# forsaken628/katib

Measured on AMD Instinct MI355X. Metric: darts_cifar10_search_wall_clock_s, lower is better.
Workload: dtype fp32; 1 GPU; model=darts-cnn-cifar10 supernet (b5: C=4, L=2, N=3, stem x1, 6 primitives + none), global_batch=128, per_gpu_batch=128, parallelism=dp1, epochs=2, steps_per_epoch=196, ops=hip, hip_graph=True, sync_bn=False, hessian=concurrent

## Files before the change

katib_amd/csrc/hip/darts_bind.cpp:

```cpp
#include <torch/extension.h>
#include <c10/hip/HIPStream.h>

#include "darts_ops.h"
#include "darts_plane_layout.h"

using namespace katib_hip;
using at::Tensor;
using OptT = c10::optional<Tensor>;

namespace {

hipStream_t cur_stream() { return c10::hip::getCurrentHIPStream().stream(); }

void check_f32(const Tensor& t, const char* name) {
  TORCH_CHECK(t.is_cuda(), name, " must be a GPU tensor");
  TORCH_CHECK(t.scalar_type() == at::kFloat, name, " must be float32");
  TORCH_CHECK(t.is_contiguous(), name, " must be contiguous");
}

constexpr at::ScalarType kZType = kZbf16 ? at::kBFloat16 : at::kFloat;

void check_z(const Tensor& t, const char* name) {
  TORCH_CHECK(t.is_cuda(), name, " must be a GPU tensor");
  TORCH_CHECK(t.scalar_type() == kZType, name, " must be ", kZbf16 ? "bfloat16" : "float32",
              " (the per-op intermediates' storage type of this build)");
  TORCH_CHECK(t.is_contiguous(), name, " must be contiguous");
}

zt* zptr(const Tensor& t) { return reinterpret_cast<zt*>(t.data_ptr()); }

template <typename T>
T* ptr_or_null(const OptT& t) {
  return t.has_value() && t->defined() ? t->data_ptr<T>() : nullptr;
}

BNRef make_bn(const py::tuple& b, int C) {
  BNRef r{};
  TORCH_CHECK(b.size() == 8, "bn tuple has 8 fields");
  OptT sums = b[0].cast<OptT>(), rm = b[1].cast<OptT>(), rv = b[2].cast<OptT>();
  r.rep = b[6].cast<int>();
  r.rstride = b[7].cast<int>();
  TORCH_CHECK(r.rep >= 1 && r.rep <= kRep && r.rstride >= 2 * C, "bn replica layout");
  if (sums.has_value() && sums->defined()) {
    TORCH_CHECK(sums->scalar_type() == at::kDouble && sums->is_contiguous() &&
                    sums->numel() >= (int64_t)(r.rep - 1) * r.rstride + 2 * C,
                "bn sums must be f64 with rep x rstride doubles");
  }
  r.sums = ptr_or_null<double>(sums);
  r.rmean = ptr_or_null<float>(rm);
  r.rvar = ptr_or_null<float>(rv);
  r.inv_count = b[3].cast<float>();
  r.eval = b[4].cast<bool>() ? 1 : 0;
  r.eps = b[5].cast<float>();
  r.C = C;
  TORCH_CHECK(r.eval ? (r.rmean && r.rvar) : (r.sums != nullptr), "bn reference lacks its statistics");
  return r;
}

int64_t storage_doubles_after(const Tensor& t) {
  return (int64_t)(t.storage().nbytes() / sizeof(double)) - t.storage_offset();
}

GradSrc make_gs(const py::tuple& t, int C) {
  GradSrc g{};
  TORCH_CHECK(t.size() == 9, "grad-source tuple has 9 fields");
  Tensor gt = t[0].cast<Tensor>(), zt = t[1].cast<Tensor>();
  check_f32(gt, "g");
  check_z(zt, "z");
  g.g = gt.data_ptr<float>();
  g.z = zptr(zt);
  OptT s1 = t[2].cast<OptT>(), s2 = t[3].cast<OptT>();
  g.S1 = ptr_or_null<double>(s1);
  g.S2 = ptr_or_null<double>(s2);
  g.bn = make_bn(t[4].cast<py::tuple>(), C);
  g.eval = g.bn.eval;
  TORCH_CHECK(g.eval || (g.S1 && g.S2), "training-mode BN backward needs S1/S2 reductions");
  OptT w = t[5].cast<OptT>();
  g.w = ptr_or_null<float>(w);
  g.widx = t[6].cast<int>();
  g.rep = t[7].cast<int>();
  g.rstride = t[8].cast<int>();
  TORCH_CHECK(g.rep >= 1 && g.rep <= kRep, "replicas");
  if (!g.eval) {
    for (int k = 2; k <= 3; ++k) {
      Tensor sv = *t[k].cast<OptT>();
      TORCH_CHECK(sv.scalar_type() == at::kDouble &&
                      storage_doubles_after(sv) >= (int64_t)(g.rep - 1) * g.rstride + C,
                  "S1/S2 replicas exceed their buffer");
    }
  }
  return g;
}

int pick_chunk(int C, int per_channel_floats, int fixed_floats) {
  const int budget = 16384 - fixed_floats;
  int ch = C;
  while (ch > 1 && ch * per_channel_floats > budget) ch = (ch + 1) / 2;
  return std::max(ch, 1);
}

template <typename Bt>
void check_batch(const std::vector<py::tuple>& calls) {
  TORCH_CHECK(!calls.empty() && (int)calls.size() <= Bt::kCap, "batch of 1..", Bt::kCap, " edges");
}

#define SAME_SHAPE(b, fld) TORCH_CHECK(b.e[i].fld == b.e[0].fld, "edges in a batch must share " #fld)

static bool fill_dwpw(const py::tuple& t, DwPwFwdArgs& a, int64_t K, int64_t dil, int64_t S, int64_t pad, int nentries,
                      bool use_mfma) {
  Tensor x = t[0].cast<Tensor>(), dw = t[1].cast<Tensor>(), pw = t[2].cast<Tensor>();
  auto inbn = t[3].cast<c10::optional<py::tuple>>();
  OptT d = t[4].cast<OptT>();
  Tensor z = t[5].cast<Tensor>();
  OptT stats = t[6].cast<OptT>();
  const bool has_d = d.has_value() && d->defined();
  const bool has_inbn = t[3].cast<c10::optional<py::tuple>>().has_value();
  if (has_inbn) check_z(x, "x (previous stage z)");
  else check_f32(x, "x");
  check_f32(dw, "dw"); check_f32(pw, "pw"); check_z(z, "z");
  if (has_d) check_z(*d, "d");
  TORCH_CHECK(x.dim() == 4, "x must be NCHW");
  TORCH_CHECK((K == 3 || K == 5) && (dil == 1 || dil == 2) && (S == 1 || S == 2), "K in {3,5}, dil, S in {1,2}");
  const int N = x.size(0), C = x.size(1), H = x.size(2), W = x.size(3);
  const int Ho = z.size(2), Wo = z.size(3);
  TORCH_CHECK(dw.numel() == C * K * K && pw.numel() == C * C, "weight shapes");
  TORCH_CHECK(z.size(0) == N && z.size(1) == C && (!has_d || d->sizes() == z.sizes()), "output shapes");
  TORCH_CHECK(has_d || !dwpw_split_path(C), "dw-pw stages of 16..64 channels (depthwise + pointwise GEMM) need d");
  TORCH_CHECK(C == 4 || C == 8 || C == 16 || (64 % Wo == 0 && Ho % (64 / Wo) == 0),
              "tile constraint: 64 % Wo == 0 and Ho % (64/Wo) == 0");
  TORCH_CHECK(C <= kMaxC, "C too large");
  TORCH_CHECK(Ho == (H + 2 * pad - dil * (K - 1) - 1) / S + 1, "output height mismatch");
  a.x = x.data_ptr(); a.dw = dw.data_ptr<float>(); a.pw = pw.data_ptr<float>();
  a.d = has_d ? zptr(*d) : nullptr; a.z = zptr(z); a.stats = ptr_or_null<double>(stats);
  if (a.stats) TORCH_CHECK(stats->scalar_type() == at::kDouble && stats->numel() >= kRep * 2 * C, "stats f64 [kRep][2C]");
  a.N = N; a.C = C; a.H = H; a.W = W; a.Ho = Ho; a.Wo = Wo; a.pad = pad;
  const int TR = 64 / Wo;
  const int IR = (TR - 1) * S + (K - 1) * dil + 1, IW = (Wo - 1) * S + (K - 1) * dil + 1;
  a.chunk = pick_chunk(C, IR * IW, C * 64 + 4 * C);
  if (C == 4 || C == 8 || C == 16) {
    int nb = std::max(1, std::min(Ho / 4, 2048 / std::max(N * nentries, 1)));
    auto band_bytes = [&](int b) {
      const int BR = (Ho + b - 1) / b;
      return (size_t)C * ((BR - 1) * S + (K - 1) * dil + 1) * plane_pitch(W + 2 * pad, S) * sizeof(float);
    };
    while (band_bytes(nb) > 65536 && nb < Ho) ++nb;
    a.chunk = nb;
  }
  a.use_mfma = (use_mfma && C % 16 == 0) ? 1 : 0;
  const bool prebn = inbn.has_value();
  if (prebn) a.inbn = make_bn(*inbn, C);
  a.variant = (((K == 5) * 4 + (dil == 2) * 2 + (S == 2)) * 4) + (prebn ? 2 : 0);
  return prebn;
}

static void fill_dwpw_multi(const std::vector<py::tuple>& calls, DwPwMultiBatch& bt, int64_t* kk, int64_t* dd,
                            int64_t* ss, int64_t* pp, bool* pre) {
  TORCH_CHECK(!calls.empty() && (int)calls.size() <= DwPwMultiBatch::kCap, "1..", DwPwMultiBatch::kCap, " entries");
  bt.n = calls.size();
  for (int i = 0; i < bt.n; ++i) {
    const py::tuple& t = calls[i];
    TORCH_CHECK(t.size() == 11, "dwpw_fwd_multi entry: (x, dw, pw, inbn, d, z, stats, K, dil, S, pad)");
    kk[i] = t[7].cast<int64_t>(); dd[i] = t[8].cast<int64_t>(); ss[i] = t[9].cast<int64_t>(); pp[i] = t[10].cast<int64_t>();
    pre[i] = fill_dwpw(t, bt.e[i], kk[i], dd[i], ss[i], pp[i], bt.n, true);
    SAME_SHAPE(bt, N); SAME_SHAPE(bt, C); SAME_SHAPE(bt, Ho); SAME_SHAPE(bt, Wo);
  }
}

void dwpw_fwd_multi(std::vector<py::tuple> calls) {
  DwPwMultiBatch bt{};
  int64_t kk[DwPwMultiBatch::kCap], dd[DwPwMultiBatch::kCap], ss[DwPwMultiBatch::kCap], pp[DwPwMultiBatch::kCap];
  bool pre[DwPwMultiBatch::kCap];
  fill_dwpw_multi(calls, bt, kk, dd, ss, pp, pre);
  if (launch_dwpw_multi(bt, cur_stream())) return;
  for (int i = 0; i < bt.n; ++i) {
    DwPwFwdBatch one{};
    one.n = 1;
    fill_dwpw(calls[i], one.e[0], kk[i], dd[i], ss[i], pp[i], 1, true);
    launch_dwpw_fwd(one, kk[i], dd[i], ss[i], pre[i], cur_stream());
  }
}

void pw_fwd(std::vector<py::tuple> calls, int64_t S) {
  check_batch<PwFwdBatch>(calls);
  PwFwdBatch bt{};
  bt.n = calls.size();
  for (int i = 0; i < bt.n; ++i) {
    const py::tuple& t = calls[i];
    Tensor x = t[0].cast<Tensor>(), pw = t[1].cast<Tensor>(), z = t[2].cast<Tensor>();
    OptT stats = t[3].cast<OptT>();
    const int co_off = t[4].cast<int>(), off = t[5].cast<int>();
    check_f32(x, "x"); check_f32(pw, "pw"); check_z(z, "z");
    const bool nm = x.dim() == 5;
    const int xnodes = nm ? x.size(0) : 1;
    const int N = nm ? x.size(1) : x.size(0), Cin = nm ? x.size(0) * x.size(2) : x.size(1);
    const int H = x.size(nm ? 3 : 2), W = x.size(nm ? 4 : 3);
    const int Cout = pw.size(0), Ho = z.size(2), Wo = z.size(3);
    TORCH_CHECK(pw.size(1) == Cin && co_off + Cout <= z.size(1) && z.size(0) == N, "pw shapes");
    TORCH_CHECK((Ho * Wo) % 64 == 0, "Ho*Wo must be a multiple of 64");
    TORCH_CHECK(Cin <= kMaxC && Cout <= kMaxC, "channels");
    PwFwdArgs& a = bt.e[i];
    a.x = x.data_ptr<float>(); a.pw = pw.data_ptr<float>(); a.z = zptr(z);
    a.stats = ptr_or_null<double>(stats);
    if (a.stats)
      TORCH_CHECK(stats->scalar_type() == at::kDouble && stats->numel() >= kRep * 2 * z.size(1), "stats [kRep][2Ctot]");
    a.N = N; a.Cin = Cin; a.Cout = Cout; a.CoutTotal = z.size(1); a.co_off = co_off;
    a.H = H; a.W = W; a.Ho = Ho; a.Wo = Wo; a.S = S; a.off = off; a.relu = 1; a.xnodes = xnodes;
    SAME_SHAPE(bt, N); SAME_SHAPE(bt, Cin); SAME_SHAPE(bt, Cout); SAME_SHAPE(bt, Ho); SAME_SHAPE(bt, Wo);
  }
  launch_pw_fwd(bt, cur_stream());
}

void pool_fwd_multi(std::vector<py::tuple> calls) {
  check_batch<PoolFwdBatch>(calls);
  PoolFwdBatch bt{};
  bt.n = calls.size();
  for (int i = 0; i < bt.n; ++i) {
    const py::tuple& t = calls[i];
    const int64_t S = t[6].cast<int64_t>();
    TORCH_CHECK(S == 1 || S == 2, "pool stride must be 1 or 2");
    bt.e[i].S = (int)S;
    Tensor x = t[0].cast<Tensor>(), zavg = t[1].cast<Tensor>(), zmax = t[2].cast<Tensor>();
    OptT sa = t[3].cast<OptT>(), sm = t[4].cast<OptT>(), amax = t[5].cast<OptT>();
    check_f32(x, "x"); check_z(zavg, "zavg"); check_z(zmax, "zmax");
    PoolFwdArgs& a = bt.e[i];
    if (amax.has_value() && amax->defined()) {
      TORCH_CHECK(amax->scalar_type() == at::kByte && amax->numel() == zmax.numel(), "amax must be uint8 like zmax");
      a.amax = amax->data_ptr<uint8_t>();
    }
    a.x = x.data_ptr<float>(); a.zavg = zptr(zavg); a.zmax = zptr(zmax);
    a.stats_avg = ptr_or_null<double>(sa); a.stats_max = ptr_or_null<double>(sm);
    if (a.stats_avg) TORCH_CHECK(sa->scalar_type() == at::kDouble && sa->numel() >= kRep * 2 * x.size(1), "stats");
    if (a.stats_max) TORCH_CHECK(sm->scalar_type() == at::kDouble && sm->numel() >= kRep * 2 * x.size(1), "stats");
    a.N = x.size(0); a.C = x.size(1); a.H = x.size(2); a.W = x.size(3); a.Ho = zavg.size(2); a.Wo = zavg.size(3);
    TORCH_CHECK(a.Ho == (a.H - 1) / S + 1 && zmax.sizes() == zavg.sizes(), "pool shapes");
    SAME_SHAPE(bt, N); SAME_SHAPE(bt, C);
  }
  launch_pool_fwd_multi(bt, cur_stream());
}

void combine_fwd(std::vector<py::tuple> calls, OptT gamma, OptT beta, Tensor out, double momentum,
                 bool update_running, bool accumulate) {
  check_f32(out, "out");
  check_batch<CombineFwdBatch>(calls);
  CombineFwdBatch bt{};
  bt.n = calls.size();
  const int C = out.size(1);
  TORCH_CHECK(C <= kMaxC, "C too large");
  TORCH_CHECK((int64_t)2 * bt.n * kMaxOps * C * 4 <= 65536, "combine LDS budget exceeded");
  for (int e = 0; e < bt.n; ++e) {
    const py::tuple& t = calls[e];
    auto zs = t[0].cast<std::vector<Tensor>>();
    auto bns = t[1].cast<std::vector<py::tuple>>();
    auto widx = t[2].cast<std::vector<int64_t>>();
    OptT w = t[3].cast<OptT>();
    const int id_idx = t[4].cast<int>();
    OptT xid = t[5].cast<OptT>();
    auto upd = t[6].cast<std::vector<py::tuple>>();
    TORCH_CHECK(zs.size() == bns.size() && zs.size() == widx.size() && (int)zs.size() <= kMaxOps, "ops");
    CombineFwdArgs& a = bt.e[e];
    a.N = out.size(0); a.C = C; a.HW = out.size(2) * out.size(3);
    a.nops = zs.size();
    for (size_t k = 0; k < zs.size(); ++k) {
      check_z(zs[k], "z");
      TORCH_CHECK(zs[k].sizes() == out.sizes(), "combine input shape");
      a.z[k] = zptr(zs[k]);
      a.bn[k] = make_bn(bns[k], C);
      a.widx[k] = widx[k];
    }
    TORCH_CHECK((int)upd.size() <= kMaxUpd, "too many update-only BN layers");
    a.nupd = upd.size();
    for (size_t k = 0; k < upd.size(); ++k) a.upd[k] = make_bn(upd[k], C);
    a.w = ptr_or_null<float>(w); a.id_idx = id_idx; a.xid = ptr_or_null<float>(xid);
    if (a.xid) {
      check_f32(*xid, "xid");
      TORCH_CHECK(xid->sizes() == out.sizes(), "identity shape");
    }
    a.gamma = ptr_or_null<float>(gamma); a.beta = ptr_or_null<float>(beta);
    a.out = out.data_ptr<float>(); a.momentum = momentum; a.update_running = update_running;
    a.accumulate = accumulate;
  }
  launch_combine_fwd(bt, cur_stream());
}

void combine_bwd_reduce(std::vector<py::tuple> calls) {
  check_batch<CombineBwdBatch>(calls);
  CombineBwdBatch bt{};
  bt.n = calls.size();
  for (int i = 0; i < bt.n; ++i) {
    const py::tuple& t = calls[i];
    Tensor dout = t[0].cast<Tensor>();
    auto zs = t[1].cast<std::vector<Tensor>>();
    auto bns = t[2].cast<std::vector<py::tuple>>();
    OptT xid = t[3].cast<OptT>();
    Tensor red = t[4].cast<Tensor>();
    auto widx = t[5].cast<std::vector<int64_t>>();
    const int id_idx = t[6].cast<int>();
    OptT gw = t[7].cast<OptT>();
    check_f32(dout, "dout");
    TORCH_CHECK(red.scalar_type() == at::kDouble, "red must be f64");
    CombineBwdArgs& a = bt.e[i];
    a.N = dout.size(0); a.C = dout.size(1); a.HW = dout.size(2) * dout.size(3);
    a.nops = zs.size();
    a.rstride = (a.nops + 1) * a.C + 1;
    TORCH_CHECK(a.nops <= kMaxOps && red.numel() >= (int64_t)kRep * a.rstride, "red size [kRep][(nops+1)C+1]");
    for (int k = 0; k < a.nops; ++k) {
      TORCH_CHECK(zs[k].sizes() == dout.sizes(), "z shape");
      check_z(zs[k], "z");
      a.z[k] = zptr(zs[k]);
      a.bn[k] = make_bn(bns[k], a.C);
    }
    a.dout = dout.data_ptr<float>(); a.xid = ptr_or_null<float>(xid); a.red = red.data_ptr<double>();
    a.gw = ptr_or_null<double>(gw); a.id_idx = id_idx;
    if (a.gw) {
      TORCH_CHECK(gw->scalar_type() == at::kDouble && gw->numel() % kRep == 0, "gw must be f64 [kRep][nw]");
      a.gwstride = gw->numel() / kRep;
      TORCH_CHECK((int)widx.size() == a.nops, "widx per op");
      for (int k = 0; k < a.nops; ++k) {
        TORCH_CHECK(widx[k] >= 0 && widx[k] < a.gwstride, "widx out of range");
        a.widx[k] = widx[k];
      }
      TORCH_CHECK(id_idx < a.gwstride, "id_idx out of range");
    }
    SAME_SHAPE(bt, N); SAME_SHAPE(bt, C); SAME_SHAPE(bt, HW);
  }
  launch_combine_bwd_reduce(bt, cur_stream());
}

void check_grad_sink(const OptT& gW, int64_t numel, int64_t gstride) {
  if (!gW.has_value() || !gW->defined()) return;
  TORCH_CHECK(gW->scalar_type() == at::kFloat && gW->is_contiguous() && gW->numel() == numel, "gW shape");
  TORCH_CHECK(gstride == 0 || (gstride >= numel && (int64_t)(gW->storage().nbytes() / sizeof(float)) -
                                                           gW->storage_offset() >= (kRep - 1) * gstride + numel),
              "gW replicas exceed their buffer");
}

void pw_bwd(std::vector<py::tuple> calls, int64_t S, int64_t mode, bool need_dx) {
  check_batch<PwBwdBatch>(calls);
  PwBwdBatch bt{};
  bt.n = calls.size();
  for (int i = 0; i < bt.n; ++i) {
    const py::tuple& t = calls[i];
    py::tuple gs = t[0].cast<py::tuple>();
    Tensor pw = t[1].cast<Tensor>();
    OptT ain = t[2].cast<OptT>();
    Tensor x = t[3].cast<Tensor>();
    OptT dd = t[4].cast<OptT>(), gx = t[5].cast<OptT>(), gW = t[6].cast<OptT>();
    const int co_off = t[7].cast<int>(), off = t[8].cast<int>();
    const int64_t gstride = t[9].cast<int64_t>();
    const bool overwrite = t.size() > 10 && t[10].cast<bool>();
    check_f32(pw, "pw");
    if (mode != 0) check_f32(x, "x");
    PwBwdArgs& a = bt.e[i];
    a.overwrite = overwrite;
    TORCH_CHECK(!overwrite || (mode == 1 && S == 1 && off == 0), "gx overwrite needs the stride-1 full-coverage form");
    const int Cout = pw.size(0), Cin = pw.size(1);
    Tensor g = gs[0].cast<Tensor>();
    a.N = g.size(0); a.CoutTotal = g.size(1); a.Ho = g.size(2); a.Wo = g.size(3);
    a.gs = make_gs(gs, a.CoutTotal);
    a.Cin = Cin; a.Cout = Cout; a.co_off = co_off; a.S = S; a.off = off; a.mode = mode;
    a.need_dx = need_dx;
    const bool nm = mode != 0 && x.dim() == 5;
    a.xnodes = nm ? x.size(0) : 1;
    a.H = x.size(nm ? 3 : 2); a.W = x.size(nm ? 4 : 3);
    if (mode != 0) {
      TORCH_CHECK(x.numel() == (int64_t)a.N * Cin * a.H * a.W && (!nm || x.size(1) == a.N),
                  "pw_bwd: x must be [N][Cin][H][W] or node-major [nodes][N][Cin/nodes][H][W]");
      if (gx.has_value() && gx->defined()) TORCH_CHECK(gx->sizes() == x.sizes(), "pw_bwd: gx must have the shape of x");
    }
    TORCH_CHECK(Cin * Cout <= 8192, "pw_bwd supports Cin*Cout <= 8192");
    TORCH_CHECK((a.Ho * a.Wo) % 64 == 0, "Ho*Wo % 64");
    a.pw = pw.data_ptr<float>(); a.x = mode != 0 ? x.data_ptr<float>() : nullptr;
    if (ain.has_value() && ain->defined()) check_z(*ain, "ain (depthwise output d)");
    a.ain = ain.has_value() && ain->defined() ? zptr(*ain) : nullptr;
    a.dd = ptr_or_null<float>(dd); a.gx = ptr_or_null<float>(gx);
    a.gW = ptr_or_null<float>(gW);
    if (mode == 0) {
      TORCH_CHECK((a.ain || !a.gW) && (!need_dx || a.dd), "mode 0 needs ain for a weight gradient (and dd)");
    } else {
      TORCH_CHECK(!need_dx || a.gx, "mode 1 needs gx");
    }
    check_grad_sink(gW, (int64_t)Cin * Cout, gstride);
    a.gstride = gstride;
    SAME_SHAPE(bt, N); SAME_SHAPE(bt, Cin); SAME_SHAPE(bt, Cout); SAME_SHAPE(bt, Ho); SAME_SHAPE(bt, Wo);
  }
  launch_pw_bwd(bt, cur_stream());
}

void dw_bwd_fill(std::vector<py::tuple>& calls, DwBwdBatch& bt, const int64_t* Ks, const int64_t* dils,
                 const int64_t* Ss, bool& prebn);

void dw_bwd_multi(std::vector<py::tuple> calls) {
  check_batch<DwBwdBatch>(calls);
  DwBwdBatch bt{};
  int64_t Ks[DwBwdBatch::kCap], Ds[DwBwdBatch::kCap], Ss[DwBwdBatch::kCap];
  for (size_t i = 0; i < calls.size(); ++i) {
    TORCH_CHECK(calls[i].size() == 10 || calls[i].size() == 12,
                "dw_bwd_multi entry: (x, inbn, dw, dd, gout, gW, red, gstride, overwrite, K[, dil, S])");
    Ks[i] = calls[i][9].cast<int64_t>();
    Ds[i] = calls[i].size() == 12 ? calls[i][10].cast<int64_t>() : 1;
    Ss[i] = calls[i].size() == 12 ? calls[i][11].cast<int64_t>() : 1;
    TORCH_CHECK((Ks[i] == 3 || Ks[i] == 5) && (Ds[i] == 1 || Ds[i] == 2) && (Ss[i] == 1 || Ss[i] == 2),
                "K in {3, 5}, dil and S in {1, 2}");
  }
  bool prebn = false;
  dw_bwd_fill(calls, bt, Ks, Ds, Ss, prebn);
  for (int i = 0; i < bt.n; ++i) {
    TORCH_CHECK(prebn || bt.e[i].overwrite, "dw_bwd_multi: input-gradient entries must own (overwrite) their output");
    TORCH_CHECK(!prebn || (Ds[i] == 1 && Ss[i] == 1), "dw_bwd_multi: input-BN entries are stride-1 separable stages");
    bt.e[i].variant = dw_bwd_variant((int)Ks[i], (int)Ds[i], (int)Ss[i], prebn);
  }
  for (int i = 0; i < bt.n; ++i)
    for (int j = i + 1; j < bt.n; ++j) TORCH_CHECK(bt.e[i].gout != bt.e[j].gout, "dw_bwd_multi entries share an output");
  if (launch_dw_bwd_multi(bt, cur_stream())) return;
  for (int v = 0; v < 16; ++v) {
    DwBwdBatch one{};
    for (int i = 0; i < bt.n; ++i)
      if (bt.e[i].variant == v) one.e[one.n++] = bt.e[i];
    if (one.n) launch_dw_bwd(one, dw_variant_k(v), dw_variant_dil(v), dw_variant_s(v), prebn, cur_stream());
  }
}

void dw_bwd_fill(std::vector<py::tuple>& calls, DwBwdBatch& bt, const int64_t* Ks, const int64_t* dils,
                 const int64_t* Ss, bool& prebn) {
  bt.n = calls.size();
  bool has_gw = false;
  for (int i = 0; i < bt.n; ++i) {
    const py::tuple& t = calls[i];
    const int64_t K = Ks[i], dil = dils[i], S = Ss[i], pad = (K - 1) / 2 * dil;
    Tensor x = t[0].cast<Tensor>();
    auto inbn = t[1].cast<c10::optional<py::tuple>>();
    Tensor dw = t[2].cast<Tensor>(), dd = t[3].cast<Tensor>(), gout = t[4].cast<Tensor>();
    OptT gW = t[5].cast<OptT>(), red = t[6].cast<OptT>();
    const int64_t gstride = t[7].cast<int64_t>();
    const bool overwrite = t[8].cast<bool>();
    if (inbn.has_value()) check_z(x, "x (stage-1 z)");
    else check_f32(x, "x");
    check_f32(dw, "dw"); check_f32(dd, "dd"); check_f32(gout, "gout");
    DwBwdArgs& a = bt.e[i];
    a.N = x.size(0); a.C = x.size(1); a.H = x.size(2); a.W = x.size(3); a.Ho = dd.size(2); a.Wo = dd.size(3);
    TORCH_CHECK(a.H == a.Ho * S && a.W == a.Wo * S, "dw_bwd needs H == Ho*S");
    TORCH_CHECK(gout.sizes() == x.sizes(), "gout shape");
    TORCH_CHECK(dw.numel() == a.C * K * K && dd.size(1) == a.C, "dw_bwd weight / grad shapes");
    a.x = x.data_ptr(); a.dw = dw.data_ptr<float>(); a.dd = dd.data_ptr<float>();
    a.gout = gout.data_ptr<float>(); a.gW = ptr_or_null<float>(gW); a.red = ptr_or_null<double>(red);
    const bool plane = (a.C == 4 || a.C == 8 || (a.C % 16 == 0 && a.C <= kMaxC)) && a.Wo % 4 == 0 &&
                       (((uintptr_t)a.x | (uintptr_t)a.dd | (uintptr_t)a.gout) & 15) == 0;
    TORCH_CHECK(plane || (64 % a.Wo == 0 && a.Ho % (64 / a.Wo) == 0), "tile constraint");
    check_grad_sink(gW, (int64_t)a.C * K * K, gstride);
    a.gstride = gstride;
    a.overwrite = overwrite;
    if (a.red) TORCH_CHECK(red->scalar_type() == at::kDouble && red->numel() >= kRep * 2 * a.C, "red [kRep][2C]");
    a.pad = pad;
    if (i == 0) {
      prebn = inbn.has_value();
      has_gw = a.gW != nullptr;
    }
    TORCH_CHECK(inbn.has_value() == prebn, "edges in a batch must agree on the input BN");
    TORCH_CHECK((a.gW != nullptr) == has_gw, "edges in a batch must agree on weight-gradient sinks");
    TORCH_CHECK(!(prebn && overwrite), "overwrite applies to the input-gradient (non-BN) form");
    const int TR = 64 / a.Wo, r = (K - 1) / 2 * dil, h = (r + S - 1) / S, OR = TR + 2 * h;
    const int IR = (TR - 1) * S + (K - 1) * dil + 1, IW = (a.Wo - 1) * S + (K - 1) * dil + 1;
    a.chunk = pick_chunk(a.C, OR * a.Wo + IR * IW, 4 * a.C + (a.gW ? a.C * (int)(K * K) : 0));
    if (prebn) a.inbn = make_bn(*inbn, a.C);
    SAME_SHAPE(bt, N); SAME_SHAPE(bt, C); SAME_SHAPE(bt, Ho); SAME_SHAPE(bt, Wo);
  }
}

void pool_bwd_multi(std::vector<py::tuple> calls) {
  check_batch<PoolBwdBatch>(calls);
  PoolBwdBatch bt{};
  bt.n = calls.size();
  for (int i = 0; i < bt.n; ++i) {
    const py::tuple& t = calls[i];
    const int64_t S = t[9].cast<int64_t>();
    TORCH_CHECK(S == 1 || S == 2, "pool stride must be 1 or 2");
    bt.e[i].S = (int)S;
    auto ga = t[0].cast<c10::optional<py::tuple>>(), gm = t[1].cast<c10::optional<py::tuple>>();
    Tensor x = t[2].cast<Tensor>();
    OptT dout_id = t[3].cast<OptT>(), w = t[4].cast<OptT>();
    const int id_idx = t[5].cast<int>();
    Tensor gx = t[6].cast<Tensor>();
    OptT amax = t[7].cast<OptT>();
    check_f32(x, "x"); check_f32(gx, "gx");
    PoolBwdArgs& a = bt.e[i];
    a.N = x.size(0); a.C = x.size(1); a.H = x.size(2); a.W = x.size(3);
    a.Ho = (a.H - 1) / S + 1; a.Wo = (a.W - 1) / S + 1;
    TORCH_CHECK(a.Ho * a.Wo <= 8192, "pool_bwd stages one output plane in LDS (Ho*Wo <= 8192)");
    TORCH_CHECK(gx.sizes() == x.sizes(), "gx shape");
    TORCH_CHECK(!gm.has_value() || (amax.has_value() && amax->defined() && amax->scalar_type() == at::kByte &&
                                    amax->numel() == (int64_t)a.N * a.C * a.Ho * a.Wo),
                "max-pool backward needs the uint8 argmax from pool_fwd");
    if (amax.has_value() && amax->defined()) a.amax = amax->data_ptr<uint8_t>();
    if (ga.has_value()) a.ga = make_gs(*ga, a.C);
    if (gm.has_value()) a.gm = make_gs(*gm, a.C);
    a.x = x.data_ptr<float>(); a.dout_id = ptr_or_null<float>(dout_id); a.w = ptr_or_null<float>(w);
    if (a.dout_id) TORCH_CHECK(dout_id->sizes() == x.sizes(), "identity gradient shape");
    a.id_idx = id_idx; a.gx = gx.data_ptr<float>();
    a.overwrite = t[8].cast<bool>();
    if (t.size() > 10) {
      auto ex = t[10].cast<std::vector<Tensor>>();
      TORCH_CHECK(ex.size() <= 4, "pool_bwd: at most 4 extra gradient parts");
      a.nextra = ex.size();
      for (size_t j = 0; j < ex.size(); ++j) {
        check_f32(ex[j], "extra");
        TORCH_CHECK(ex[j].sizes() == gx.sizes(), "extra gradient part shape");
        TORCH_CHECK(ex[j].data_ptr() != gx.data_ptr(), "extra part aliases gx");
        a.extra[j] = ex[j].data_ptr<float>();
      }
    }
    SAME_SHAPE(bt, N); SAME_SHAPE(bt, C);
  }
  for (int i = 0; i < bt.n; ++i)
    for (int j = i + 1; j < bt.n; ++j) TORCH_CHECK(bt.e[i].gx != bt.e[j].gx, "pool_bwd entries share a gx buffer");
  launch_pool_bwd_multi(bt, cur_stream());
}

void fold_rows(Tensor buf) {
  check_f32(buf, "buf");
  TORCH_CHECK(buf.dim() == 2, "buf must be [rows][n]");
  FoldArgs a{};
  a.buf = buf.data_ptr<float>();
  a.rows = buf.size(0);
  a.n = buf.size(1);
  launch_fold_rows(a, cur_stream());
}

void fold_f64(std::vector<py::tuple> segs) {
  TORCH_CHECK(!segs.empty() && (int)segs.size() <= kMaxSeg, "1..kMaxSeg segments");
  FoldF64Args a{};
  a.nseg = segs.size();
  for (int k = 0; k < a.nseg; ++k) {
    Tensor t = segs[k][0].cast<Tensor>();
    int n = segs[k][1].cast<int>(), rs = segs[k][2].cast<int>();
    TORCH_CHECK(t.is_cuda() && t.scalar_type() == at::kDouble && t.is_contiguous(), "fold segment must be f64");
    TORCH_CHECK(n >= 1 && rs >= n && t.numel() >= (int64_t)(kRep - 1) * rs + n, "fold segment size");
    a.p[k] = t.data_ptr<double>();
    a.n[k] = n;
    a.rstride[k] = rs;
    a.total += n;
  }
  launch_fold_f64(a, cur_stream());
}

}

void register_xgmi(py::module& m);
void register_conv(py::module& m);
void register_transformer(py::module& m);
void register_batchnorm(py::module& m);
void register_mlp(py::module& m);
void register_stem(py::module& m);
void register_enas(py::module& m);
void register_dwconv(py::module& m);
void register_darts_optim(py::module& m);
void register_darts_head(py::module& m);
void register_resnet(py::module& m);
void register_augment(py::module& m);

PYBIND11_MODULE(TORCH_EXTENSION_NAME, m) {
  m.doc() = "katib_amd HIP kernels for gfx950 (DARTS edge ops, implicit-GEMM conv, transformer, xGMI all-reduce)";
  m.def("pw_fwd", &pw_fwd);
  m.def("combine_fwd", &combine_fwd);
  m.def("combine_bwd_reduce", &combine_bwd_reduce);
  m.def("pw_bwd", &pw_bwd);
  m.def("dw_bwd_multi", &dw_bwd_multi, "separable second-stage depthwise backward of mixed kernel size in one launch");
  m.def("dwpw_fwd_multi", &dwpw_fwd_multi, "mixed (K, dil, S) dw-pw entries of one node stage in one launch");
  m.def("pool_fwd_multi", &pool_fwd_multi, "stride-1 and stride-2 pools in one launch");
  m.def("pool_bwd_multi", &pool_bwd_multi, "stride-1 and stride-2 pool backward in one launch");
  m.def("set_max_blocks", &set_max_blocks);
  m.def("stamps_arm", [](int kind, int call, torch::Tensor buf) {
    TORCH_CHECK(!buf.defined() || kind == 0 || (buf.is_cuda() && buf.scalar_type() == torch::kInt64 &&
                                               buf.is_contiguous() && buf.numel() >= 65536 * 8),
                "stamps_arm: int64 CUDA buffer of >= 65536 * 8 entries");
    stamps_arm(kind, call, kind == 0 ? nullptr : reinterpret_cast<unsigned long long*>(buf.data_ptr<int64_t>()));
  }, "diagnostic build: phase-stamp the call-th launch of kind (StampKind) into buf[wg * 8 + phase]");
  m.def("stamps_compiled", &stamps_compiled);
  m.def("fold_rows", &fold_rows);
  m.def("fold_f64", &fold_f64);
  m.attr("REP") = kRep;
  m.attr("ZBF16") = kZbf16;
  m.def("max_blocks", &max_blocks);
  m.def("dwpw_split_path", [](int64_t C) { return dwpw_split_path((int)C); });
  register_xgmi(m);
  register_conv(m);
  register_transformer(m);
  register_batchnorm(m);
  register_enas(m);
  register_dwconv(m);
  register_mlp(m);
  register_stem(m);
  register_darts_optim(m);
  register_darts_head(m);
  register_resnet(m);
  register_augment(m);
}
```

katib_amd/csrc/hip/darts_ops.h:

```cpp
#pragma once
#include <hip/hip_runtime.h>
#include <hip/hip_bf16.h>

namespace katib_hip {

#ifdef KATIB_DARTS_ZBF16
typedef __hip_bfloat16 zt;
constexpr bool kZbf16 = true;
#else
typedef float zt;
constexpr bool kZbf16 = false;
#endif
typedef float zf4 __attribute__((ext_vector_type(4)));

__device__ __forceinline__ float z2f(float v) { return v; }
__device__ __forceinline__ float z2f(__hip_bfloat16 v) { return __bfloat162float(v); }
__device__ __forceinline__ void zput(float* p, float v) { *p = v; }
__device__ __forceinline__ void zput(__hip_bfloat16* p, float v) { *p = __float2bfloat16(v); }
__device__ __forceinline__ zf4 zld4(const float* p) { return *reinterpret_cast<const zf4*>(p); }
__device__ __forceinline__ zf4 zld4(const __hip_bfloat16* p) {
  const uint2 u = *reinterpret_cast<const uint2*>(p);
  return zf4{__uint_as_float(u.x << 16), __uint_as_float(u.x & 0xffff0000u), __uint_as_float(u.y << 16),
             __uint_as_float(u.y & 0xffff0000u)};
}
__device__ __forceinline__ void zst4(float* p, zf4 v) { *reinterpret_cast<zf4*>(p) = v; }
__device__ __forceinline__ void zst4(__hip_bfloat16* p, zf4 v) {
  __hip_bfloat16 b[4] = {__float2bfloat16(v.x), __float2bfloat16(v.y), __float2bfloat16(v.z), __float2bfloat16(v.w)};
  *reinterpret_cast<uint2*>(p) = *reinterpret_cast<const uint2*>(b);
}

__host__ __device__ __forceinline__ size_t plane_off(int n, int c, int N, int C, int nodes, size_t HW) {
  if (nodes <= 1) return ((size_t)n * C + c) * HW;
  const int Cn = C / nodes, k = c / Cn;
  return (((size_t)k * N + n) * Cn + (c - k * Cn)) * HW;
}

constexpr int kMaxOps = 8;
constexpr int kMaxUpd = 4;
constexpr int kMaxC = 256;
constexpr bool dwpw_split_path(int C) { return C % 16 == 0 && C <= 64; }
#ifndef KATIB_HIP_REP
#define KATIB_HIP_REP 32
#endif
constexpr int kRep = KATIB_HIP_REP;

struct BNRef {
  const double* sums;
  float* rmean;
  float* rvar;
  float inv_count;
  float eps;
  int eval;
  int C;
  int rep;
  int rstride;
};

struct GradSrc {
  const float* g;
  const zt* z;
  const double* S1;
  const double* S2;
  BNRef bn;
  const float* w;
  int widx;
  int eval;
  int rep;
  int rstride;
};

struct DwPwFwdArgs {
  const void* x;
  BNRef inbn; const float* dw; const float* pw;
  zt* d; zt* z; double* stats;
  int N, C, H, W, Ho, Wo, pad, chunk, use_mfma;
  int variant;
  int nblk;
  int vout = 0;
};

struct PwFwdArgs {
  const void* x;
  const float* pw; zt* z; double* stats;
  int N, Cin, Cout, CoutTotal, co_off, H, W, Ho, Wo, S, off;
  int relu;
  int xnodes;
};

struct PoolFwdArgs {
  const float* x; zt* zavg; zt* zmax; double* stats_avg; double* stats_max; unsigned char* amax;
  int N, C, H, W, Ho, Wo;
  int S, nblk;
};

struct CombineFwdArgs {
  const zt* z[kMaxOps]; BNRef bn[kMaxOps]; int widx[kMaxOps]; int nops;
  BNRef upd[kMaxUpd]; int nupd;
  const float* w; int id_idx; const float* xid; const float* gamma; const float* beta;
  float* out; int N, C, HW; float momentum; int update_running; int accumulate;
};

struct CombineBwdArgs {
  const float* dout; const zt* z[kMaxOps]; BNRef bn[kMaxOps]; int nops;
  const float* xid; double* red; int N, C, HW;
  double* gw; int widx[kMaxOps]; int id_idx;
  int rstride, gwstride;
};

struct PwBwdArgs {
  GradSrc gs; const float* pw; const zt* ain; const float* x; float* dd; float* gx; float* gW;
  int gstride;
  int N, Cin, Cout, CoutTotal, co_off, H, W, Ho, Wo, S, off, mode, need_dx;
  int overwrite;
  int xnodes;
};

struct DwBwdArgs {
  const void* x;
  BNRef inbn; const float* dw; const float* dd; float* gout; float* gW; double* red;
  int gstride;
  int N, C, H, W, Ho, Wo, pad, chunk;
  int overwrite;
  int variant, nbands, nblk;
  int vin = 0;
  int blk0 = 0;
};
constexpr int dw_bwd_variant(int K, int dil, int S, bool prebn) {
  return (((K == 5) * 4 + (dil == 2) * 2 + (S == 2)) << 1) | (prebn ? 1 : 0);
}
constexpr int dw_variant_k(int v) { return (v >> 3) & 1 ? 5 : 3; }
constexpr int dw_variant_dil(int v) { return (v >> 2) & 1 ? 2 : 1; }
constexpr int dw_variant_s(int v) { return (v >> 1) & 1 ? 2 : 1; }
constexpr bool dw_variant_prebn(int v) { return v & 1; }

struct FoldArgs {
  float* buf; int n; int rows;
};

constexpr int kMaxSeg = 128;
struct FoldF64Args {
  double* p[kMaxSeg]; int n[kMaxSeg]; int rstride[kMaxSeg]; int nseg; int total;
};

struct PoolBwdArgs {
  GradSrc ga; GradSrc gm; const float* x; const float* dout_id; const float* w; int id_idx; float* gx;
  const unsigned char* amax;
  const float* extra[4]; int nextra;
  int overwrite;
  int N, C, H, W, Ho, Wo;
  int S;
};

template <typename A, int M>
struct Batch {
  A e[M];
  int n;
  static constexpr int kCap = M;
};
using DwPwFwdBatch = Batch<DwPwFwdArgs, 16>;
using CombineFwdBatch = Batch<CombineFwdArgs, 4>;
using PwFwdBatch = Batch<PwFwdArgs, 32>;
using PoolFwdBatch = Batch<PoolFwdArgs, 16>;
using CombineBwdBatch = Batch<CombineBwdArgs, 8>;
using PwBwdBatch = Batch<PwBwdArgs, 32>;
using DwBwdBatch = Batch<DwBwdArgs, 40>;
using PoolBwdBatch = Batch<PoolBwdArgs, 16>;
using DwPwMultiBatch = Batch<DwPwFwdArgs, 40>;

constexpr size_t kKernargMax = 24576;
static_assert(sizeof(DwPwFwdBatch) <= kKernargMax && sizeof(CombineFwdBatch) <= kKernargMax &&
                  sizeof(PwFwdBatch) <= kKernargMax && sizeof(PoolFwdBatch) <= kKernargMax &&
                  sizeof(CombineBwdBatch) <= kKernargMax && sizeof(PwBwdBatch) <= kKernargMax &&
                  sizeof(DwBwdBatch) <= kKernargMax && sizeof(PoolBwdBatch) <= kKernargMax &&
                  sizeof(DwPwMultiBatch) <= kKernargMax,
              "kernel argument batches exceed the kernarg budget");

void launch_dwpw_fwd(const DwPwFwdBatch& b, int K, int dil, int S, bool prebn, hipStream_t st);
void launch_dw_bwd(const DwBwdBatch& b, int K, int dil, int S, bool prebn, hipStream_t st);
bool launch_dw_bwd_multi(DwBwdBatch b, hipStream_t st);
void launch_pw_fwd(const PwFwdBatch& b, hipStream_t st);
bool launch_dwpw_multi(DwPwMultiBatch b, hipStream_t st);
void launch_pool_fwd_multi(PoolFwdBatch b, hipStream_t st);
void launch_pool_bwd_multi(const PoolBwdBatch& b, hipStream_t st);
void launch_combine_fwd(const CombineFwdBatch& b, hipStream_t st);
void launch_combine_bwd_reduce(const CombineBwdBatch& b, hipStream_t st);
void launch_pw_bwd(const PwBwdBatch& b, hipStream_t st);
int max_blocks();
void launch_fold_rows(const FoldArgs& a, hipStream_t st);
void launch_fold_f64(const FoldF64Args& a, hipStream_t st);
void set_max_blocks(int n);
void stamps_arm(int kind, int call, unsigned long long* buf);
bool stamps_compiled();

}
```

katib_amd/csrc/hip/darts_ops_dwb.hip:

```cpp
#include "darts_ops_dev.h"

namespace katib_hip {

template <int K, int DIL, int S, bool PREBN>
__global__ void __launch_bounds__(256) dw_bwd_kernel(DwBwdBatch bt) {
  const DwBwdArgs& a = bt.e[blockIdx.y];
  constexpr int P = 64, KK = K * K;
  const int C = a.C, H = a.H, W = a.W, Ho = a.Ho, Wo = a.Wo;
  const int TR = P / Wo;
  const int tiles = Ho / TR;
  const int ntiles = a.N * tiles;
  const int pad = a.pad;
  const int r = (K - 1) / 2 * DIL;
  const int h = (r + S - 1) / S;
  const int OR = TR + 2 * h;
  const int IR = (TR - 1) * S + (K - 1) * DIL + 1;
  const int IW = (Wo - 1) * S + (K - 1) * DIL + 1;
  extern __shared__ __attribute__((aligned(16))) float smem[];
  float* sDD = smem;
  float* sIn = sDD + a.chunk * OR * Wo;
  float* sMean = sIn + a.chunk * IR * IW;
  float* sInv = sMean + C;
  float* sRed = sInv + C;
  float* sGW = sRed + 2 * C;
  const int tid = threadIdx.x, wave = tid >> 6, lane = tid & 63;
  for (int c = tid; c < C; c += 256) {
    if (PREBN) bn_coeffs(a.inbn, c, sMean[c], sInv[c]);
    sRed[c] = 0.f;
    sRed[C + c] = 0.f;
  }
  if (a.gW)
    for (int i = tid; i < C * KK; i += 256) sGW[i] = 0.f;
  __syncthreads();
  const int own_in = TR * S;
  const int nq = own_in * W;
  for (int t = blockIdx.x; t < ntiles; t += gridDim.x) {
    const int n = t / tiles, oy0 = (t % tiles) * TR;
    const int iy0 = oy0 * S - pad;
    const size_t xin = (size_t)n * C * H * W;
    const float* ddn = a.dd + (size_t)n * C * Ho * Wo;
    for (int c0 = 0; c0 < C; c0 += a.chunk) {
      const int cn = min(a.chunk, C - c0);
      #pragma unroll 4
      for (int i = tid; i < cn * OR * Wo; i += 256) {
        int cc = i / (OR * Wo), rr = (i / Wo) % OR, q = i % Wo;
        int oy = oy0 - h + rr;
        sDD[i] = (oy >= 0 && oy < Ho) ? ddn[((size_t)(c0 + cc) * Ho + oy) * Wo + q] : 0.f;
      }
      if (a.gW) {
        #pragma unroll 4
        for (int i = tid; i < cn * IR * IW; i += 256) {
          int cc = i / (IR * IW), rr = (i / IW) % IR, q = i % IW;
          int iy = iy0 + rr, ix = -pad + q, c = c0 + cc;
          float v = 0.f;
          if (iy >= 0 && iy < H && ix >= 0 && ix < W) {
            v = xval<PREBN>(a.x, xin + ((size_t)c * H + iy) * W + ix);
            if (PREBN) v = (v - sMean[c]) * sInv[c];
            v = fmaxf(v, 0.f);
          }
          sIn[i] = v;
        }
      }
      __syncthreads();
      if (a.gW) {
        for (int job = tid; job < cn * KK; job += 256) {
          const int cc = job / KK, tap = job % KK, ky = tap / K, kx = tap % K;
          const float* dd = sDD + (cc * OR + h) * Wo;
          const float* in = sIn + (cc * IR + ky * DIL) * IW + kx * DIL;
          float s = 0.f;
          for (int ty = 0; ty < TR; ++ty)
            for (int tx = 0; tx < Wo; ++tx) s += dd[ty * Wo + tx] * in[ty * S * IW + tx * S];
          sGW[(c0 + cc) * KK + tap] += s;
        }
      }
      const int qspan = (nq < 256 && 256 % nq == 0) ? nq : 256;
      const int G = 256 / qspan;
      for (int q0 = 0; q0 < nq; q0 += qspan) {
        const int q = q0 + tid % qspan;
        const int cg = __builtin_amdgcn_readfirstlane(tid / qspan);
        const int rr = q / W, ix = q - rr * W;
        const int iy = oy0 * S + rr;
        const bool ok = q < nq && iy < H;
        int srow[K], ocol[K];
        float mrow[K], mcol[K];
#pragma unroll
        for (int k = 0; k < K; ++k) {
          int ty = iy + pad - k * DIL;
          int oy = ty >= 0 ? ty / S : -1;
          bool v = ok && ty >= 0 && (ty % S) == 0 && oy < Ho;
          srow[k] = v ? oy - (oy0 - h) : 0;
          mrow[k] = v ? 1.f : 0.f;
          int tx = ix + pad - k * DIL;
          int ox = tx >= 0 ? tx / S : -1;
          bool u = ok && tx >= 0 && (tx % S) == 0 && ox < Wo;
          ocol[k] = u ? ox : 0;
          mcol[k] = u ? 1.f : 0.f;
        }
        for (int cc = cg; cc < cn; cc += G) {
          const int c = c0 + cc;
          const float* wk = a.dw + c * KK;
          const float* dd = sDD + cc * OR * Wo;
          float ga = 0.f;
#pragma unroll
          for (int ky = 0; ky < K; ++ky) {
            float rowacc = 0.f;
#pragma unroll
            for (int kx = 0; kx < K; ++kx) rowacc += mcol[kx] * wk[ky * K + kx] * dd[srow[ky] * Wo + ocol[kx]];
            ga += mrow[ky] * rowacc;
          }
          const size_t xi = ((size_t)(n * C + c) * H + iy) * W + ix;
          if (PREBN) {
            float g = 0.f, gy = 0.f;
            if (ok) {
              float y = (xval<true>(a.x, xi) - sMean[c]) * sInv[c];
              g = y > 0.f ? ga : 0.f;
              gy = g * y;
              a.gout[xi] = g;
            }
            if (a.red) {
              g = wave_sum(g);
              gy = wave_sum(gy);
              if (lane == 0) {
                atomicAdd(sRed + c, g);
                atomicAdd(sRed + C + c, gy);
              }
            }
          } else if (ok) {
            const float gm = xval<false>(a.x, xi) > 0.f ? ga : 0.f;
            if (a.overwrite) a.gout[xi] = gm;
            else if (gm != 0.f) a.gout[xi] += gm;
          }
        }
      }
      __syncthreads();
    }
  }
  if (PREBN && a.red)
    for (int i = tid; i < 2 * C; i += 256) atomicAdd(a.red + rep_slot() * 2 * C + i, (double)sRed[i]);
  if (a.gW)
    for (int i = tid; i < C * KK; i += 256) atomicAdd(a.gW + (size_t)rep_slot() * a.gstride + i, sGW[i]);
}

template <int S, bool V4 = false>
__device__ __forceinline__ void pool_bwd_body(const PoolBwdArgs& a, const int bx) {
  const int C = a.C, H = a.H, W = a.W, Ho = a.Ho, Wo = a.Wo, HWo = Ho * Wo;
  const int nc = bx, c = nc % C;
  const size_t ob = (size_t)nc * HWo;
  extern __shared__ __attribute__((aligned(16))) float smem[];
  float* sGa = smem;
  float* sGm = smem + HWo;
  unsigned char* sArg = (unsigned char*)(smem + 2 * HWo);
  __shared__ float sCo[8];
  KSTAMP(0);
  if (threadIdx.x < 64) {
    const int grp = threadIdx.x >> 4, j = threadIdx.x & 15;
    const GradSrc& gs = grp & 1 ? a.gm : a.ga;
    const bool on = gs.z != nullptr, stats = grp < 2;
    const BNRef& b = gs.bn;
    double s = 0.0, s2 = 0.0;
    if (on && stats && !b.eval) {
      for (int r = j; r < b.rep; r += 16) {
        s += b.sums[(size_t)r * b.rstride + c];
        s2 += b.sums[(size_t)r * b.rstride + b.C + c];
      }
    } else if (on && !stats && !gs.eval) {
      const int rep = gs.rep, rs = gs.rep == 1 ? 0 : gs.rstride;
      const size_t off2 = gs.S2 - gs.S1;
      for (int r = j; r < rep; r += 16) {
        s += gs.S1[(size_t)r * rs + c];
        s2 += gs.S1[(size_t)r * rs + off2 + c];
      }
    }
#pragma unroll
    for (int o = 8; o > 0; o >>= 1) {
      s += __shfl_xor(s, o, 64);
      s2 += __shfl_xor(s2, o, 64);
    }
    if (j == 0) {
      float* o = sCo + 4 * (grp & 1) + (stats ? 0 : 2);
      if (!on) {
        o[0] = 0.f;
        o[1] = stats ? 1.f : 0.f;
      } else if (stats) {
        if (b.eval) {
          o[0] = b.rmean[c];
          o[1] = rsqrtf(b.rvar[c] + b.eps);
        } else {
          const double m = s * (double)b.inv_count;
          double v = s2 * (double)b.inv_count - m * m;
          if (v < 0) v = 0;
          o[0] = (float)m;
          o[1] = rsqrtf((float)v + b.eps);
        }
      } else {
        o[0] = gs.eval ? 0.f : (float)(s * (double)gs.bn.inv_count);
        o[1] = gs.eval ? 0.f : (float)(s2 * (double)gs.bn.inv_count);
      }
    }
  }
  __syncthreads();
  KSTAMP(1);
  const float ma = sCo[0], ia = sCo[1], a1 = a.ga.z ? sCo[2] : 0.f, a2 = a.ga.z ? sCo[3] : 0.f;
  const float mm = sCo[4], im = sCo[5], m1 = a.gm.z ? sCo[6] : 0.f, m2 = a.gm.z ? sCo[7] : 0.f;
  const float wa = a.ga.w ? a.ga.w[a.ga.widx] : 0.f;
  const float wm = a.gm.w ? a.gm.w[a.gm.widx] : 0.f;
  const float wid = (a.w && a.id_idx >= 0) ? a.w[a.id_idx] : 0.f;
  if constexpr (V4) {
    typedef float f4 __attribute__((ext_vector_type(4)));
    const float* gsrc = a.ga.z ? a.ga.g : a.gm.g;
    for (int o4 = threadIdx.x * 4; o4 < HWo; o4 += 1024) {
      const f4 g = *reinterpret_cast<const f4*>(gsrc + ob + o4);
      if (a.ga.z) {
        const f4 z = zld4(a.ga.z + ob + o4);
        const f4 d = wa * ia * (g - a1 - ((z - ma) * ia) * a2);
#pragma unroll
        for (int t = 0; t < 4; ++t) {
          const int o = o4 + t, oy = o / Wo, ox = o - oy * Wo;
          const int y0 = max(oy * S - 1, 0), y1 = min(oy * S + 1, H - 1);
          const int x0 = max(ox * S - 1, 0), x1 = min(ox * S + 1, W - 1);
          sGa[o] = d[t] / (float)((y1 - y0 + 1) * (x1 - x0 + 1));
        }
      } else {
        *reinterpret_cast<f4*>(sGa + o4) = f4{0.f, 0.f, 0.f, 0.f};
      }
      if (a.gm.z) {
        const f4 z = zld4(a.gm.z + ob + o4);
        *reinterpret_cast<f4*>(sGm + o4) = wm * im * (g - m1 - ((z - mm) * im) * m2);
        *reinterpret_cast<unsigned*>(sArg + o4) = *reinterpret_cast<const unsigned*>(a.amax + ob + o4);
      } else {
        *reinterpret_cast<f4*>(sGm + o4) = f4{0.f, 0.f, 0.f, 0.f};
        *reinterpret_cast<unsigned*>(sArg + o4) = 0xffffffffu;
      }
    }
    __syncthreads();
    KSTAMP(2);
    const size_t pb = (size_t)nc * H * W;
    for (int q4 = threadIdx.x * 4; q4 < H * W; q4 += 1024) {
      f4 g = {0.f, 0.f, 0.f, 0.f};
      if (a.dout_id) g = wid * *reinterpret_cast<const f4*>(a.dout_id + pb + q4);
#pragma unroll
      for (int j = 0; j < 4; ++j)
        if (j < a.nextra) g += *reinterpret_cast<const f4*>(a.extra[j] + pb + q4);
      const int iy = q4 / W, ix0 = q4 - iy * W;
      if constexpr (S == 1) {
        float wa[3][6], wm[3][6];
        unsigned char wt[3][6];
#pragma unroll
        for (int r = 0; r < 3; ++r) {
          const int oy = iy - 1 + r;
          const bool rok = oy >= 0 && oy < Ho;
          const int o = (rok ? oy : 0) * Wo + ix0;
          const f4 ga4 = *reinterpret_cast<const f4*>(sGa + o), gm4 = *reinterpret_cast<const f4*>(sGm + o);
          const unsigned t4 = *reinterpret_cast<const unsigned*>(sArg + o);
#pragma unroll
          for (int k = 0; k < 4; ++k) {
            wa[r][k + 1] = rok ? ga4[k] : 0.f;
            wm[r][k + 1] = rok ? gm4[k] : 0.f;
            wt[r][k + 1] = rok ? (unsigned char)(t4 >> (8 * k)) : 255;
          }
          const bool lok = rok && ix0 > 0, hok = rok && ix0 + 4 < Wo;
          wa[r][0] = lok ? sGa[o - 1] : 0.f;
          wm[r][0] = lok ? sGm[o - 1] : 0.f;
          wt[r][0] = lok ? sArg[o - 1] : 255;
          wa[r][5] = hok ? sGa[o + 4] : 0.f;
          wm[r][5] = hok ? sGm[o + 4] : 0.f;
          wt[r][5] = hok ? sArg[o + 4] : 255;
        }
#pragma unroll
        for (int t = 0; t < 4; ++t) {
          float v = 0.f;
#pragma unroll
          for (int r = 0; r < 3; ++r)
#pragma unroll
            for (int cx = 0; cx < 3; ++cx) {
              v += wa[r][t + cx];
              if (wt[r][t + cx] == (2 - r) * 3 + (2 - cx)) v += wm[r][t + cx];
            }
          g[t] += v;
        }
        f4* dst = reinterpret_cast<f4*>(a.gx + pb + q4);
        *dst = a.overwrite ? g : *dst + g;
        continue;
      }
      if constexpr (S == 2) {
        float wa[2][3], wm[2][3];
        unsigned char wt[2][3];
        const int m = iy >> 1, k2 = ix0 >> 1;
#pragma unroll
        for (int r = 0; r < 2; ++r) {
          const int oy = m + r;
          const bool rok = oy < Ho && (r == 0 || (iy & 1));
          const int o = (rok ? oy : m) * Wo + k2;
          typedef float f2 __attribute__((ext_vector_type(2)));
          const f2 ga2 = *reinterpret_cast<const f2*>(sGa + o), gm2 = *reinterpret_cast<const f2*>(sGm + o);
          const unsigned short t2 = *reinterpret_cast<const unsigned short*>(sArg + o);
#pragma unroll
          for (int c = 0; c < 2; ++c) {
            wa[r][c] = rok ? ga2[c] : 0.f;
            wm[r][c] = rok ? gm2[c] : 0.f;
            wt[r][c] = rok ? (unsigned char)(t2 >> (8 * c)) : 255;
          }
          const bool hok = rok && k2 + 2 < Wo;
          wa[r][2] = hok ? sGa[o + 2] : 0.f;
          wm[r][2] = hok ? sGm[o + 2] : 0.f;
          wt[r][2] = hok ? sArg[o + 2] : 255;
        }
#pragma unroll
        for (int t = 0; t < 4; ++t) {
          float v = 0.f;
#pragma unroll
          for (int r = 0; r < 2; ++r)
#pragma unroll
            for (int c = t / 2; c <= (t + 1) / 2; ++c) {
              v += wa[r][c];
              if (wt[r][c] == (iy - 2 * (m + r) + 1) * 3 + (t - 2 * c + 1)) v += wm[r][c];
            }
          g[t] += v;
        }
        f4* dst = reinterpret_cast<f4*>(a.gx + pb + q4);
        *dst = a.overwrite ? g : *dst + g;
        continue;
      }
      const int oy_lo = iy - 1 < 0 ? 0 : (iy - 1 + S - 1) / S, oy_hi = min((iy + 1) / S, Ho - 1);
#pragma unroll
      for (int t = 0; t < 4; ++t) {
        const int ix = ix0 + t;
        const int ox_lo = ix - 1 < 0 ? 0 : (ix - 1 + S - 1) / S, ox_hi = min((ix + 1) / S, Wo - 1);
        float v = 0.f;
        for (int oy = oy_lo; oy <= oy_hi; ++oy)
          for (int ox = ox_lo; ox <= ox_hi; ++ox) {
            const int o = oy * Wo + ox;
            v += sGa[o];
            if (sArg[o] == (iy - oy * S + 1) * 3 + (ix - ox * S + 1)) v += sGm[o];
          }
        g[t] += v;
      }
      f4* dst = reinterpret_cast<f4*>(a.gx + pb + q4);
      *dst = a.overwrite ? g : *dst + g;
    }
    KSTAMP(3);
    return;
  }
  for (int o = threadIdx.x; o < HWo; o += 256) {
    int oy = o / Wo, ox = o % Wo;
    if (a.ga.z) {
      int y0 = max(oy * S - 1, 0), y1 = min(oy * S + 1, H - 1);
      int x0 = max(ox * S - 1, 0), x1 = min(ox * S + 1, W - 1);
      sGa[o] = bn_bwd_val(a.ga, ob + o, ma, ia, wa, a1, a2) / (float)((y1 - y0 + 1) * (x1 - x0 + 1));
    } else {
      sGa[o] = 0.f;
    }
    if (a.gm.z) {
      sGm[o] = bn_bwd_val(a.gm, ob + o, mm, im, wm, m1, m2);
      sArg[o] = a.amax[ob + o];
    } else {
      sGm[o] = 0.f;
      sArg[o] = 255;
    }
  }
  __syncthreads();
  for (int q = threadIdx.x; q < H * W; q += 256) {
    int iy = q / W, ix = q % W;
    float g = 0.f;
    int oy_lo = iy - 1 < 0 ? 0 : (iy - 1 + S - 1) / S, oy_hi = min((iy + 1) / S, Ho - 1);
    int ox_lo = ix - 1 < 0 ? 0 : (ix - 1 + S - 1) / S, ox_hi = min((ix + 1) / S, Wo - 1);
    for (int oy = oy_lo; oy <= oy_hi; ++oy) {
      for (int ox = ox_lo; ox <= ox_hi; ++ox) {
        int o = oy * Wo + ox;
        g += sGa[o];
        int tap = (iy - oy * S + 1) * 3 + (ix - ox * S + 1);
        if (sArg[o] == tap) g += sGm[o];
      }
    }
    if (a.dout_id) g += wid * a.dout_id[(size_t)nc * H * W + q];
#pragma unroll
    for (int j = 0; j < 4; ++j)
      if (j < a.nextra) g += a.extra[j][(size_t)nc * H * W + q];
    if (a.overwrite) a.gx[(size_t)nc * H * W + q] = g;
    else a.gx[(size_t)nc * H * W + q] += g;
  }
}

template <bool V4>
__global__ void __launch_bounds__(256) pool_bwd_multi_kernel(PoolBwdBatch bt) {
  const PoolBwdArgs a = bt.e[blockIdx.y];
  if ((int)blockIdx.x >= a.N * a.C) return;
  if (a.S == 1) pool_bwd_body<1, V4>(a, blockIdx.x);
  else pool_bwd_body<2, V4>(a, blockIdx.x);
}


template <int K, int DIL, int S, bool PREBN, int C>
__device__ __forceinline__ void dw_bwd_plane_body(const DwBwdArgs& a, const int bx, const int nb, const int dbg) {
  constexpr int KK = K * K, PAD = (K - 1) / 2 * DIL, PO = (PAD + S - 1) / S, SH = S == 2 ? 1 : 0;
  const int H = a.H, W = a.W, Ho = a.Ho, Wo = a.Wo;
  const int G = a.C / C, grp = bx % G, nbx = bx / G, c0 = grp * C;
  const int n = nbx / nb, band = nbx - n * nb;
  const int BRi = H / nb, iy0 = band * BRi, nrow = BRi;
  const int oyA = (iy0 - PAD) >> SH;
  const int oyB = (iy0 + nrow - 1 + PAD) >> SH;
  const int ODR = oyB - oyA + 1, ODW = plane_pitch(Wo + 2 * PO, S), PIN = plane_pitch(W, S), NP = nrow * W;
  const bool accum = !PREBN && !a.overwrite;
  extern __shared__ __attribute__((aligned(16))) float smem[];
  float* sWt = smem;
  float* sGW = smem + C * 25;
  float* sDD = smem + dwb_head_floats(C);
  float* sIn = sDD + C * ODR * ODW;
  float* sOld = sIn + C * nrow * PIN;
  __shared__ float sMean[C], sInv[C], sRed[2 * C];
  const int tid = threadIdx.x, lane = tid & 63, wave = tid >> 6;
  KSTAMP(0);
  for (int i = tid; i < C * KK; i += 256) {
    sGW[i] = 0.f;
    sWt[i] = a.dw[c0 * KK + i];
  }
  if (tid < C) {
    if (PREBN) bn_coeffs(a.inbn, c0 + tid, sMean[tid], sInv[tid]);
    sRed[tid] = 0.f;
    sRed[C + tid] = 0.f;
  }
  if (PREBN) __syncthreads();
  KSTAMP(1);
  const float* ddn = a.dd + ((size_t)n * a.C + c0) * Ho * Wo;
  const size_t xn = ((size_t)n * a.C + c0) * H * W;
  const int va = max(oyA, 0), vb = min(oyB, Ho - 1), vrows = vb - va + 1;
  {
    const int q4 = vrows * Wo / 4;
#pragma unroll 4
    for (int i = tid; i < C * q4; i += 256) {
      const int c = i / q4, o = (i - c * q4) * 4, r = o / Wo, ox = o - r * Wo;
      const float4 v = *reinterpret_cast<const float4*>(ddn + ((size_t)c * Ho + va) * Wo + o);
      float* d = sDD + (c * ODR + va - oyA + r) * ODW + PO + ox;
      d[0] = v.x;
      d[1] = v.y;
      d[2] = v.z;
      d[3] = v.w;
    }
    for (int i = tid; i < C * ODR; i += 256) {
      const int c = i / ODR, oy = oyA + i - c * ODR;
      float* d = sDD + i * ODW;
      if (oy < 0 || oy >= Ho) {
        for (int q = 0; q < ODW; ++q) d[q] = 0.f;
      } else {
        for (int q = 0; q < PO; ++q) d[q] = d[PO + Wo + q] = 0.f;
      }
    }
  }
  {
    const int q4 = NP / 4, w4 = W / 4;
#pragma unroll 4
    for (int i = tid; i < C * q4; i += 256) {
      const int c = i / q4, oq = i - c * q4, o = oq * 4, r = oq / w4, lo = (c * nrow + r) * PIN + (oq - r * w4) * 4;
      float4 v = xval4<PREBN>(a.x, xn + ((size_t)c * H + iy0) * W + o);
      if (PREBN) {
        const float m = sMean[c], iv = sInv[c];
        v.x = (v.x - m) * iv;
        v.y = (v.y - m) * iv;
        v.z = (v.z - m) * iv;
        v.w = (v.w - m) * iv;
      }
      v.x = fmaxf(v.x, 0.f);
      v.y = fmaxf(v.y, 0.f);
      v.z = fmaxf(v.z, 0.f);
      v.w = fmaxf(v.w, 0.f);
      *reinterpret_cast<float4*>(sIn + lo) = v;
    }
    if (accum) {
      const float* gsrc = a.gout + ((size_t)n * a.C + c0) * H * W;
#pragma unroll 4
      for (int i = tid; i < C * q4; i += 256) {
        const int c = i / q4, oq = i - c * q4, o = oq * 4, r = oq / w4;
        *reinterpret_cast<float4*>(sOld + (c * nrow + r) * PIN + (oq - r * w4) * 4) =
            *reinterpret_cast<const float4*>(gsrc + ((size_t)c * H + iy0) * W + o);
      }
    }
  }
  __syncthreads();
  KSTAMP(2);
  float st1[C], st2[C];
#pragma unroll
  for (int c = 0; c < C; ++c) st1[c] = st2[c] = 0.f;
  float* gn = a.gout + ((size_t)n * a.C + c0) * H * W;
  const bool tiled = S == 1 && (W & 7) == 0;
  const bool vin = a.vin && (S == 2 || tiled);
  if (S == 1 && vin) {
    typedef float f4 __attribute__((ext_vector_type(4)));
    constexpr int NQ = (4 + 2 * PAD + 3) / 4;
    const int npair = W >> 3, nrb = (nrow + kCellRows - 1) / kCellRows;
    for (int j = 4 * wave + tile_cell(lane); j < ((dbg & 1) ? 0 : C * nrb * npair); j += kBlockCells) {
      const TileItem it = tile_item(j, lane, nrb, npair);
      if (it.row >= nrow) continue;
      const int c = it.c, r = it.row, ix = 4 * it.quad, iy = iy0 + r;
      int srow[K];
#pragma unroll
      for (int k = 0; k < K; ++k) srow[k] = (iy + PAD - k * DIL - oyA) * ODW + ix;
      KEEP_WEIGHT_READS_LOCAL();
      const float* wk = sWt + c * KK;
      const float* dd = sDD + c * ODR * ODW;
      f4 ga = {0.f, 0.f, 0.f, 0.f};
#pragma unroll
      for (int ky = 0; ky < K; ++ky) {
        float v[4 * NQ];
#pragma unroll
        for (int q = 0; q < NQ; ++q) {
          const float4 t = *reinterpret_cast<const float4*>(dd + srow[ky] + 4 * q);
          v[4 * q] = t.x;
          v[4 * q + 1] = t.y;
          v[4 * q + 2] = t.z;
          v[4 * q + 3] = t.w;
        }
#pragma unroll
        for (int kx = 0; kx < K; ++kx) {
          const float w = wk[ky * K + kx];
          const int o = 2 * PAD - kx * DIL;
          ga.x += w * v[o];
          ga.y += w * v[o + 1];
          ga.z += w * v[o + 2];
          ga.w += w * v[o + 3];
        }
      }
      const int li = (c * nrow + r) * PIN + ix;
      const f4 act = *reinterpret_cast<const f4*>(sIn + li);
      const f4 g = {act.x > 0.f ? ga.x : 0.f, act.y > 0.f ? ga.y : 0.f, act.z > 0.f ? ga.z : 0.f,
                    act.w > 0.f ? ga.w : 0.f};
      f4* dst = reinterpret_cast<f4*>(gn + ((size_t)c * H + iy) * W + ix);
      if (PREBN) {
        *dst = g;
        const float t1 = (g.x + g.y) + (g.z + g.w);
        const float t2 = (g.x * act.x + g.y * act.y) + (g.z * act.z + g.w * act.w);
#pragma unroll
        for (int cc = 0; cc < C; ++cc)
          if (cc == c) {
            st1[cc] += t1;
            st2[cc] += t2;
          }
      } else {
        *dst = accum ? *reinterpret_cast<const f4*>(sOld + li) + g : g;
      }
    }
  }
  if constexpr (S == 2) {
    const int hw2 = W / 2, NPc = (nrow / 2) * hw2;
    for (int q = tid; q < ((dbg & 1) || !vin ? 0 : NP); q += 256) {
      const int cls = NPc % 64 == 0 ? __builtin_amdgcn_readfirstlane(q / NPc) : q / NPc;
      const int qq = q - cls * NPc, rr = qq / hw2, xx = qq - rr * hw2;
      const int r = 2 * rr + (cls >> 1), ix = 2 * xx + (cls & 1), iy = iy0 + r;
      const int iyc = iy0 + (cls >> 1), ixc = cls & 1;
      int srow[K], scol[K];
#pragma unroll
      for (int k = 0; k < K; ++k) {
        srow[k] = (((iy + PAD - k * DIL) >> 1) - oyA) * ODW;
        scol[k] = ((ix + PAD - k * DIL) >> 1) + PO;
      }
#pragma unroll
      for (int c = 0; c < C; ++c) {
        KEEP_WEIGHT_READS_LOCAL();
        const float* wk = sWt + c * KK;
        const float* dd = sDD + c * ODR * ODW;
        float ga = 0.f;
#pragma unroll
        for (int ky = 0; ky < K; ++ky) {
          if ((iyc + PAD - ky * DIL) & 1) continue;
#pragma unroll
          for (int kx = 0; kx < K; ++kx) {
            if ((ixc + PAD - kx * DIL) & 1) continue;
            ga += wk[ky * K + kx] * dd[srow[ky] + scol[kx]];
          }
        }
        const int li = (c * nrow + r) * PIN + ix;
        const float act = sIn[li];
        const size_t gi = ((size_t)c * H + iy) * W + ix;
        const float g = act > 0.f ? ga : 0.f;
        if (PREBN) {
          gn[gi] = g;
          st1[c] += g;
          st2[c] += g * act;
        } else {
          gn[gi] = accum ? sOld[li] + g : g;
        }
      }
    }
  }
  for (int p = tid; p < ((dbg & 1) || vin ? 0 : NP); p += 256) {
    const int r = p / W, ix = p - r * W, iy = iy0 + r;
    int srow[K], scol[K];
    float mrow[K], mcol[K];
#pragma unroll
    for (int k = 0; k < K; ++k) {
      const int t = iy + PAD - k * DIL, u = ix + PAD - k * DIL;
      srow[k] = ((t >> SH) - oyA) * ODW;
      scol[k] = (u >> SH) + PO;
      mrow[k] = (S == 1 || (t & 1) == 0) ? 1.f : 0.f;
      mcol[k] = (S == 1 || (u & 1) == 0) ? 1.f : 0.f;
    }
#pragma unroll
    for (int c = 0; c < C; ++c) {
      KEEP_WEIGHT_READS_LOCAL();
        const float* wk = sWt + c * KK;
      const float* dd = sDD + c * ODR * ODW;
      float ga = 0.f;
#pragma unroll
      for (int ky = 0; ky < K; ++ky) {
        float rowacc = 0.f;
#pragma unroll
        for (int kx = 0; kx < K; ++kx) {
          const float v = wk[ky * K + kx] * dd[srow[ky] + scol[kx]];
          rowacc += S == 1 ? v : mcol[kx] * v;
        }
        ga += S == 1 ? rowacc : mrow[ky] * rowacc;
      }
      const int li = (c * nrow + r) * PIN + ix;
      const float act = sIn[li];
      const size_t gi = ((size_t)c * H + iy) * W + ix;
      const float g = act > 0.f ? ga : 0.f;
      if (PREBN) {
        gn[gi] = g;
        st1[c] += g;
        st2[c] += g * act;
      } else {
        gn[gi] = accum ? sOld[li] + g : g;
      }
    }
  }
  if (PREBN && a.red) {
    float st[2 * C];
#pragma unroll
    for (int c = 0; c < C; ++c) st[c] = st1[c], st[C + c] = st2[c];
    const float v = wave_reduce_scatter<2 * C>(st);
    if ((lane & (32 / C - 1)) == 0) atomicAdd(sRed + wave_scatter_index<2 * C>(lane), v);
  }
  KSTAMP(3);
  if (a.gW && !(dbg & 2) && tiled) {
    constexpr int KP = K == 3 ? 4 : 8;
    const int npair = W >> 3, nrb = (nrow + kCellRows - 1) / kCellRows;
    const int xp = wgrad_parts(C * K * nrb, npair), ncell = C * K * nrb * xp;
    const bool wave_job = ((nrb * xp) & 3) == 0;
    for (int u0 = 4 * wave; u0 < ncell; u0 += kBlockCells) {
      const int u = u0 + tile_cell(lane);
      const WgradJob jb = wgrad_job(u, lane, K, nrb, xp);
      float acc[KP];
#pragma unroll
      for (int kx = 0; kx < KP; ++kx) acc[kx] = 0.f;
      if (u < ncell && jb.row < nrow) {
        const float* ddr = sDD + (jb.c * ODR + iy0 + jb.row + PAD - jb.ky * DIL - oyA) * ODW;
        const float* inr = sIn + (jb.c * nrow + jb.row) * PIN;
        for (int ix = 4 * jb.q0; ix < W; ix += 8 * xp) {
          const float4 v = *reinterpret_cast<const float4*>(inr + ix);
          constexpr int NQ = (4 + 2 * PAD + 3) / 4;
          float dseg[4 * NQ];
#pragma unroll
          for (int q = 0; q < NQ; ++q) {
            const float4 t = *reinterpret_cast<const float4*>(ddr + ix + 4 * q);
            dseg[4 * q] = t.x;
            dseg[4 * q + 1] = t.y;
            dseg[4 * q + 2] = t.z;
            dseg[4 * q + 3] = t.w;
          }
#pragma unroll
          for (int kx = 0; kx < K; ++kx) {
            const int o = 2 * PAD - kx * DIL;
            acc[kx] += v.x * dseg[o] + v.y * dseg[o + 1] + v.z * dseg[o + 2] + v.w * dseg[o + 3];
          }
        }
      }
      float* gw = sGW + jb.c * KK + jb.ky * K;
      if (wave_job) {
        const float sum = wave_reduce_scatter<KP>(acc);
        const int kx = wave_scatter_index<KP>(lane);
        if ((lane & (64 / KP - 1)) == 0 && kx < K) atomicAdd(gw + kx, sum);
      } else {
#pragma unroll
        for (int kx = 0; kx < K; ++kx) {
          float v = acc[kx];
          v += __shfl_xor(v, 1, 64);
          v += __shfl_xor(v, 2, 64);
          v += __shfl_xor(v, 12, 64);
          v += __shfl_xor(v, 20, 64);
          if ((lane & 27) == 0 && u < ncell) atomicAdd(gw + kx, v);
        }
      }
    }
  } else if (a.gW && !(dbg & 2)) {
    constexpr int JOBS = C * KK, T = JOBS >= 256 ? 1 : 256 / JOBS;
    for (int j = tid; j < JOBS * T; j += 256) {
      const int job = j / T, part = j - job * T;
      const int c = job / KK, tap = job - c * KK, ky = tap / K, kx = tap - ky * K;
      const float* dd = sDD + c * ODR * ODW;
      const float* in = sIn + c * nrow * PIN;
      float acc = 0.f;
      for (int r = 0; r < nrow; ++r) {
        const int t = iy0 + r + PAD - ky * DIL;
        if (S == 2 && (t & 1)) continue;
        const float* ddr = dd + ((t >> SH) - oyA) * ODW + PO;
        const float* inr = in + r * PIN;
        for (int ix = part * S + ((S == 2) ? ((PAD - kx * DIL) & 1) : 0); ix < W; ix += T * S)
          acc += inr[ix] * ddr[(ix + PAD - kx * DIL) >> SH];
      }
      atomicAdd(sGW + job, acc);
    }
  }
  KSTAMP(4);
  __syncthreads();
  if (PREBN && a.red && tid < 2 * C)
    atomicAdd(a.red + (bx % kRep) * 2 * a.C + (tid < C ? c0 + tid : a.C + c0 + tid - C), (double)sRed[tid]);
  if (a.gW)
    for (int i = tid; i < C * KK; i += 256) atomicAdd(a.gW + (size_t)(bx % kRep) * a.gstride + c0 * KK + i, sGW[i]);
  KSTAMP(5);
}

template <int K, int DIL, int S, bool PREBN, int C>
__global__ void __launch_bounds__(256) dw_bwd_plane_kernel(DwBwdBatch bt, int nb, int dbg) {
  dw_bwd_plane_body<K, DIL, S, PREBN, C>(bt.e[blockIdx.y], blockIdx.x, nb, dbg);
}

#define DWB_CASE(KK, DD, SS, PB) \
  case dw_bwd_variant(KK, DD, SS, PB): dw_bwd_plane_body<KK, DD, SS, PB, C>(a, bx, a.nbands, 0); break;
template <int C>
__global__ void __launch_bounds__(256) dw_bwd_plane_multi_kernel(DwBwdBatch bt) {
  int ei = 0;
  for (int i = 1; i < bt.n; ++i)
    if ((int)blockIdx.x >= bt.e[i].blk0) ei = i;
  const DwBwdArgs a = bt.e[ei];
  const int bx = blockIdx.x - a.blk0;
  switch (a.variant) {
    DWB_CASE(3, 1, 1, true) DWB_CASE(5, 1, 1, true)
    DWB_CASE(3, 1, 1, false) DWB_CASE(3, 1, 2, false) DWB_CASE(5, 1, 1, false) DWB_CASE(5, 1, 2, false)
    DWB_CASE(3, 2, 1, false) DWB_CASE(3, 2, 2, false) DWB_CASE(5, 2, 1, false) DWB_CASE(5, 2, 2, false)
    default: break;
  }
}
#undef DWB_CASE

void launch_pool_bwd_multi(const PoolBwdBatch& b, hipStream_t st) {
  int maxblk = 0;
  size_t lds = 0;
  bool v4 = true;
  auto al = [](const void* p, uintptr_t m) { return p == nullptr || (reinterpret_cast<uintptr_t>(p) & (m - 1)) == 0; };
  for (int i = 0; i < b.n; ++i) {
    const PoolBwdArgs& a = b.e[i];
    maxblk = std::max(maxblk, a.N * a.C);
    lds = std::max(lds, sizeof(float) * 2 * a.Ho * a.Wo + a.Ho * a.Wo + 16);
    v4 = v4 && (a.Ho * a.Wo) % 4 == 0 && (a.H * a.W) % 4 == 0 && a.W % 4 == 0 && al(a.ga.g, 16) && al(a.gm.g, 16) &&
         al(a.ga.z, 4 * sizeof(zt)) && al(a.gm.z, 4 * sizeof(zt)) && al(a.amax, 4) && al(a.dout_id, 16) &&
         al(a.gx, 16) && (!a.ga.z || !a.gm.z || a.ga.g == a.gm.g);
    for (int j = 0; j < a.nextra; ++j) v4 = v4 && al(a.extra[j], 16);
  }
  KSTAMP_ARM(kStampPoolBwd, st)
  if (v4) hipLaunchKernelGGL(pool_bwd_multi_kernel<true>, dim3(maxblk, b.n), dim3(256), lds, st, b);
  else hipLaunchKernelGGL(pool_bwd_multi_kernel<false>, dim3(maxblk, b.n), dim3(256), lds, st, b);
  KSTAMP_DISARM(st)
}

#ifndef KATIB_DWB_BAND_KB
#define KATIB_DWB_BAND_KB 48
#endif
constexpr int kDwbBandKB = KATIB_DWB_BAND_KB;
static size_t dw_plane_floats(const DwBwdArgs& a, int K, int DIL, int S, int nb, bool accum, int C) {
  const int PAD = (K - 1) / 2 * DIL, PO = (PAD + S - 1) / S, sh = S == 2 ? 1 : 0, BRi = a.H / nb;
  auto fdiv = [sh](int v) { return v >= 0 ? v >> sh : -((-v + (1 << sh) - 1) >> sh); };
  const int ODR = fdiv(BRi - 1 + PAD) - fdiv(-PAD) + 2;
  return (size_t)dwb_head_floats(C) + (size_t)C * ODR * plane_pitch(a.Wo + 2 * PO, S) +
         (size_t)C * BRi * plane_pitch(a.W, S) * (accum ? 2 : 1);
}

template <int K, int DIL, int S, int C>
static void launch_dw_bwd_plane_t(const DwBwdBatch& b, bool prebn, hipStream_t st) {
  const DwBwdArgs& a = b.e[0];
  bool accum = false;
  for (int i = 0; i < b.n; ++i) accum |= !prebn && !b.e[i].overwrite;
  int nb = 1;
  const int G = a.C / C;
  while (nb < 8 && a.H % (2 * nb) == 0 &&
         (dw_plane_floats(a, K, DIL, S, nb, accum, C) * 4 > kDwbBandKB * 1024 || a.N * nb * G * b.n < 1024))
    nb *= 2;
  const size_t lds = sizeof(float) * dw_plane_floats(a, K, DIL, S, nb, accum, C);
  dim3 grid(a.N * nb * G, b.n);
  constexpr int dbg = 0;
  if (prebn) hipLaunchKernelGGL((dw_bwd_plane_kernel<K, DIL, S, true, C>), grid, dim3(256), lds, st, b, nb, dbg);
  else hipLaunchKernelGGL((dw_bwd_plane_kernel<K, DIL, S, false, C>), grid, dim3(256), lds, st, b, nb, dbg);
}

static bool aligned16(const DwBwdBatch& b) {
  for (int i = 0; i < b.n; ++i)
    if (((uintptr_t)b.e[i].x | (uintptr_t)b.e[i].dd | (uintptr_t)b.e[i].gout) & 15) return false;
  return true;
}

static bool dw_plane_ok(const DwBwdBatch& b, int K, int DIL, int S) {
  const DwBwdArgs& a = b.e[0];
  return (a.C == 4 || a.C == 8 || (a.C % 16 == 0 && a.C <= kMaxC)) && a.H == a.Ho * S && a.W == a.Wo * S &&
         a.pad == (K - 1) / 2 * DIL && a.Wo % 4 == 0 && aligned16(b);
}

template <int K, int DIL, int S>
static void launch_dw_bwd_t(const DwBwdBatch& b, bool prebn, hipStream_t st) {
  const DwBwdArgs& a = b.e[0];
  if (dw_plane_ok(b, K, DIL, S)) {
    constexpr int grp = 4;
    if (a.C == 4 || grp == 4) return launch_dw_bwd_plane_t<K, DIL, S, 4>(b, prebn, st);
    if (a.C == 8 || grp == 8) return launch_dw_bwd_plane_t<K, DIL, S, 8>(b, prebn, st);
    return launch_dw_bwd_plane_t<K, DIL, S, 16>(b, prebn, st);
  }
  const int TR = 64 / a.Wo;
  const int r = (K - 1) / 2 * DIL, h = (r + S - 1) / S, OR = TR + 2 * h;
  const int IR = (TR - 1) * S + (K - 1) * DIL + 1;
  const int IW = (a.Wo - 1) * S + (K - 1) * DIL + 1;
  size_t lds = sizeof(float) * (a.chunk * OR * a.Wo + a.chunk * IR * IW + 4 * a.C + (a.gW ? a.C * K * K : 0));
  dim3 grid(per_edge_blocks(a.N * (a.Ho / TR), b.n), b.n);
  if (prebn) hipLaunchKernelGGL((dw_bwd_kernel<K, DIL, S, true>), grid, dim3(256), lds, st, b);
  else hipLaunchKernelGGL((dw_bwd_kernel<K, DIL, S, false>), grid, dim3(256), lds, st, b);
}

bool launch_dw_bwd_multi(DwBwdBatch b, hipStream_t st) {
  if (b.n < 1) return true;
  const DwBwdArgs& a0 = b.e[0];
  if (!(a0.C == 4 || a0.C == 8 || (a0.C % 16 == 0 && a0.C <= kMaxC)) || !aligned16(b)) return false;
  constexpr int grp = 4;
  const int C = (a0.C == 4 || grp == 4) ? 4 : 8;
  if (a0.C % C) return false;
  int total = 0;
  size_t lds = 0;
  for (int i = 0; i < b.n; ++i) {
    DwBwdArgs& a = b.e[i];
    const int K = dw_variant_k(a.variant), DIL = dw_variant_dil(a.variant), S = dw_variant_s(a.variant);
    const bool prebn = dw_variant_prebn(a.variant);
    if (a.C != a0.C || a.H != a.Ho * S || a.W != a.Wo * S || a.pad != (K - 1) / 2 * DIL || a.Wo % 4 ||
        (prebn && (DIL != 1 || S != 1)) || (!prebn && !a.overwrite))
      return false;
    int nb = 1;
    const int G = a.C / C;
    constexpr int min_wg = 512;
    while (nb < 8 && a.H % (2 * nb) == 0 &&
           (dw_plane_floats(a, K, DIL, S, nb, false, C) * 4 > kDwbBandKB * 1024 || a.N * nb * G * b.n < min_wg))
      nb *= 2;
    a.nbands = nb;
    a.nblk = a.N * nb * G;
    a.vin = S == 1 ? (vec_mask() >> (C == 4 ? 2 : 3)) & 1 : (vec_mask() >> 4) & 1;
    a.blk0 = total;
    total += a.nblk;
    lds = std::max(lds, sizeof(float) * dw_plane_floats(a, K, DIL, S, nb, false, C));
  }
  KSTAMP_ARM(kStampDwBwd, st)
  if (C == 4) hipLaunchKernelGGL(dw_bwd_plane_multi_kernel<4>, dim3(total), dim3(256), lds, st, b);
  else hipLaunchKernelGGL(dw_bwd_plane_multi_kernel<8>, dim3(total), dim3(256), lds, st, b);
  KSTAMP_DISARM(st)
  return true;
}

void launch_dw_bwd(const DwBwdBatch& b, int K, int dil, int S, bool prebn, hipStream_t st) {
#define DISPATCH(KK, DD, SS) \
  if (K == KK && dil == DD && S == SS) return launch_dw_bwd_t<KK, DD, SS>(b, prebn, st);
  DISPATCH(3, 1, 1) DISPATCH(3, 1, 2) DISPATCH(5, 1, 1) DISPATCH(5, 1, 2)
  DISPATCH(3, 2, 1) DISPATCH(3, 2, 2) DISPATCH(5, 2, 1) DISPATCH(5, 2, 2)
#undef DISPATCH
}

}
```

katib_amd/models/darts_search.py:

```python

from __future__ import annotations

import math
from typing import Dict, List, Optional

import torch
import torch.nn.functional as F

from ..parallel.comm import Comm
from .darts import BNState, DartsLayout, DartsNetwork, accuracy

EVAL_GROUP = 16


def eval_groups(batches, group: int = 0):
    group = max(1, group or EVAL_GROUP)
    buf = []
    for b in batches:
        buf.append(b)
        if len(buf) == group:
            yield (buf[0][0], buf[0][1]) if group == 1 else (torch.cat([x for x, _ in buf]), torch.cat([y for _, y in buf]))
            buf = []
    if buf:
        yield (buf[0][0], buf[0][1]) if len(buf) == 1 else (torch.cat([x for x, _ in buf]), torch.cat([y for _, y in buf]))

DEFAULTS = dict(w_lr=0.025, w_lr_min=0.001, w_momentum=0.9, w_weight_decay=3e-4, w_grad_clip=5.0,
                alpha_lr=3e-4, alpha_weight_decay=1e-3)


class _Leaves:

    def __init__(self, views: Dict[str, torch.Tensor], grad_views: Dict[str, torch.Tensor]):
        self.views = views
        for k, v in views.items():
            v.requires_grad_(True)
            v.grad = grad_views[k]
        self.list = list(views.values())


class DartsSearch:
    debug_skip_hessian_passes = False

    def __init__(self, layout: DartsLayout, device, comm: Optional[Comm] = None, seed: int = 2,
                 settings: Optional[Dict] = None, capture: bool = False, ops=None, sync_bn: bool = False,
                 hessian: str = "concurrent"):
        self.layout = layout
        self.device = torch.device(device)
        self.comm = comm or Comm(device=self.device)
        if self.device.type == "cuda":
            self.comm.enable_xgmi()
        self.s = dict(DEFAULTS)
        if settings:
            self.s.update({k: float(v) for k, v in settings.items() if k in DEFAULTS})
        self.capture = capture and self.device.type == "cuda"
        self.net = DartsNetwork(layout, ops=ops)
        g = torch.Generator().manual_seed(seed)
        dev, f32 = self.device, torch.float32
        nW, nA = layout.n_weights, layout.n_alphas
        W = torch.zeros(nW, dtype=f32)
        layout.init_weights(W, g)
        A = 1e-3 * torch.randn(nA, generator=g)
        self.W = W.to(dev)
        self.A = A.to(dev)
        self.comm.broadcast_(self.W)
        self.comm.broadcast_(self.A)
        self.Wv = torch.zeros_like(self.W)
        self.Av = torch.zeros_like(self.A)
        self.hd = None
        if self.device.type == "cuda" and self.net.ops.backend() == "hip":
            self.hd = self.net.ops.hip_module()
        self.sync_bn = bool(sync_bn) and self.comm.distributed
        self._hsync = None
        if self.sync_bn:
            self.net.sync = self.comm
            if self.hd is not None:
                self._hsync = self.hd.SyncBN(self.comm)
                if not self._hsync.capturable:
                    self.capture = False
            elif self.capture and not self.comm.graph_capturable([]):
                self.capture = False
        R = self.hd.REP if self.hd is not None else 1
        self.gW_rep = torch.zeros(R, nW, device=dev)
        self.gWv_rep = torch.zeros(R, nW, device=dev)
        if self.hd is not None:
            self.hd.register_grad_replicas(self.gW_rep)
            self.hd.register_grad_replicas(self.gWv_rep)
        self.gW = self.gW_rep[0]
        self.gWv = self.gWv_rep[0]
        self.gAv = torch.zeros_like(self.A)
        self.gA = torch.zeros_like(self.A)
        self.gAp = torch.zeros_like(self.A)
        self.alpha_grad = torch.zeros_like(self.A)
        self.mom = torch.zeros_like(self.W)
        self.adam_m = torch.zeros_like(self.A)
        self.adam_v = torch.zeros_like(self.A)
        self.adam_t = torch.zeros((), device=dev)
        self.lr = torch.full((), self.s["w_lr"], device=dev)
        self.eps = torch.zeros((), device=dev)
        self.bn = BNState(layout, dev)
        self.bn_v = BNState(layout, dev)
        self.loss_out = torch.zeros((), device=dev)
        self.logits_out = None
        self.Pw = _Leaves(layout.views(self.W), layout.views(self.gW))
        self.Pv = _Leaves(layout.views(self.Wv), layout.views(self.gWv))
        self.An, self.Ar = layout.alpha_views(self.A)
        self.Aw, self.gAw = self._alpha_leaves(self.A, self.gA)
        self.Avw, _ = self._alpha_leaves(self.Av, self.gAv)
        self.W_detached = layout.views(self.W.detach())
        if hessian not in ("stacked", "concurrent", "sequential"):
            raise ValueError("hessian must be stacked, concurrent or sequential")
        if self.device.type != "cuda" or self.hd is None:
            hessian = "sequential"
        self._hsync_side = None
        if hessian == "concurrent" and self.sync_bn:
            if self._hsync is not None and self._hsync.capturable:
                side = self.comm if self._hsync.ws is not None else self.comm.subgroup()
                self._hsync_side = self.hd.SyncBN(side)
            if self._hsync_side is None or not self._hsync_side.capturable:
                hessian = "sequential"
        self.hessian = hessian
        self.hess_concurrent = hessian == "concurrent"
        if hessian in ("stacked", "concurrent"):
            self.Wp = torch.empty_like(self.W)
            self.Wm = torch.empty_like(self.W)
            self.Wp_views = layout.views(self.Wp)
            self.Wm_views = layout.views(self.Wm)
            self.Aw_p, _ = self._alpha_leaves(self.A, self.gAp)
            self.bn_plus = BNState(layout, dev)
            self.bn_zero = BNState(layout, dev)
            self._one_side = torch.ones((), device=dev)
        if hessian == "concurrent":
            self._side = torch.cuda.Stream(device=dev)
        self.K = self.hd._K if self.hd is not None else None
        self._parts = (torch.zeros(self.K.OPTIM_MAX_PARTS, dtype=torch.float64, device=dev)
                       if self.K is not None else None)
        self._one = None
        self.graphs = None
        self.rendezvous_per_step = None
        self.rendezvous_serial_per_step = None
        self.rendezvous_in_graph = None
        self.static = None
        self._eval_graphs = {}
        self.stack_stats = None

    def _alpha_leaves(self, A, gA):
        rows, K = self.layout.n_alpha_rows, len(self.layout.prims)
        leaves, grads = [], []
        for t in range(2 if self.layout.has_reduce else 1):
            v = A[t * rows * K:(t + 1) * rows * K].view(rows, K)
            g = gA[t * rows * K:(t + 1) * rows * K].view(rows, K)
            v.requires_grad_(True)
            v.grad = g
            leaves.append(v)
            grads.append(g)
        return leaves, grads

    @staticmethod
    def _fixed(leaves):
        return [a.detach() for a in leaves]

    def _arch(self, leaves):
        return leaves[0], (leaves[1] if len(leaves) > 1 else [])

    def _loss(self, x, y, P, an, ar, bn):
        return self.net.forward_loss(x, y, P, an, ar, bn, training=True)

    def _fold(self, rep):
        if self.hd is not None:
            self.hd.fold(rep)

    def _backward(self, loss, inputs):
        if self._one is None or self._one.device != loss.device:
            self._one = torch.ones((), device=loss.device)
        torch.autograd.backward(loss, grad_tensors=self._one, inputs=inputs)

    def _seg_virtual(self, tx, ty):
        if self.K is None:
            self.gW.zero_()
        loss, _ = self._loss(tx, ty, self.Pw.views, *self._arch(self._fixed(self.Aw)), self.bn)
        self._backward(loss, self.Pw.list)
        self._fold(self.gW_rep)

    def _seg_unrolled(self, vx, vy):
        s = self.s
        if self.K is not None:
            self.K.optim_virtual_step(self.Wv, self.W, self.mom, self.gW, self.lr, s["w_momentum"],
                                      s["w_weight_decay"], self.Av, self.A, self.gWv, self.gAv, True)
        else:
            with torch.no_grad():
                self.Wv.copy_(self.mom).mul_(s["w_momentum"]).add_(self.gW).add_(self.W, alpha=s["w_weight_decay"])
                self.Wv.mul_(-self.lr).add_(self.W)
                self.Av.copy_(self.A)
            self.gWv.zero_()
            self.gAv.zero_()
        loss, _ = self._loss(vx, vy, self.Pv.views, *self._arch(self.Avw), self.bn_v)
        self._backward(loss, self.Pv.list + self.Avw)
        self._fold(self.gWv_rep)

    def _seg_hessian(self, tx, ty):
        if self.K is not None and self.hessian in ("stacked", "concurrent"):
            K, args = self.K, (self.eps, self._parts)
            nparts = K.optim_sumsq(self.gWv, self._parts)
            tail = (self.gA, self.gAp, self.gAv, self.alpha_grad, self.lr, self.Wp, self.Wm, self.bn.buf,
                    self.bn_plus.buf, self.bn_zero.buf, self.net.momentum)
            K.optim_hessian_split(3, self.W, self.gWv, *args, nparts, *tail)
            if self.debug_skip_hessian_passes:
                if not getattr(self, "_warned_skip", False):
                    import warnings

                    warnings.warn("DartsSearch.debug_skip_hessian_passes is set: the architecture gradient is wrong")
                    self._warned_skip = True
                K.optim_hessian_split(2, self.W, self.gWv, *args, nparts, *tail)
                return
            if self.hessian == "stacked":
                with self.hd.stacked_passes() as sp:
                    with sp.pass_():
                        loss, _ = self._loss(tx, ty, self.Wp_views, *self._arch(self.Aw_p), self.bn_plus)
                        torch.autograd.backward(loss, grad_tensors=self._one_side, inputs=self.Aw_p)
                    with sp.pass_():
                        loss, _ = self._loss(tx, ty, self.Wm_views, *self._arch(self.Aw), self.bn)
                        self._backward(loss, self.Aw)
                self.stack_stats = sp.stats
                K.optim_hessian_split(2, self.W, self.gWv, *args, nparts, *tail)
                return
            main = torch.cuda.current_stream()
            self._side.wait_stream(main)
            with torch.cuda.stream(self._side), self._scope(self._hsync_side):
                loss, _ = self._loss(tx, ty, self.Wp_views, *self._arch(self.Aw_p), self.bn_plus)
                torch.autograd.backward(loss, grad_tensors=self._one_side, inputs=self.Aw_p)
            loss, _ = self._loss(tx, ty, self.Wm_views, *self._arch(self.Aw), self.bn)
            self._backward(loss, self.Aw)
            main.wait_stream(self._side)
            K.optim_hessian_split(2, self.W, self.gWv, *args, nparts, *tail)
            return
        if self.K is not None:
            K, args = self.K, (self.eps, self._parts)
            nparts = K.optim_sumsq(self.gWv, self._parts)
            tail = (self.gA, self.gAp, self.gAv, self.alpha_grad, self.lr)
            K.optim_hessian(0, self.W, self.gWv, *args, nparts, *tail)
            loss, _ = self._loss(tx, ty, self.W_detached, *self._arch(self.Aw), self.bn)
            loss.backward(inputs=self.Aw)
            K.optim_hessian(1, self.W, self.gWv, *args, nparts, *tail)
            loss, _ = self._loss(tx, ty, self.W_detached, *self._arch(self.Aw), self.bn)
            loss.backward(inputs=self.Aw)
            K.optim_hessian(2, self.W, self.gWv, *args, nparts, *tail)
            return
        with torch.no_grad():
            self.eps.copy_(0.01 / self.gWv.norm())
            self.W.add_(self.gWv * self.eps)
        self.gA.zero_()
        loss, _ = self._loss(tx, ty, self.W_detached, *self._arch(self.Aw), self.bn)
        loss.backward(inputs=self.Aw)
        with torch.no_grad():
            self.gAp.copy_(self.gA)
            self.W.sub_(self.gWv * (2.0 * self.eps))
        self.gA.zero_()
        loss, _ = self._loss(tx, ty, self.W_detached, *self._arch(self.Aw), self.bn)
        loss.backward(inputs=self.Aw)
        with torch.no_grad():
            self.W.add_(self.gWv * self.eps)
            h = (self.gAp - self.gA) / (2.0 * self.eps)
            torch.sub(self.gAv, h * self.lr, out=self.alpha_grad)

    def _seg_alpha_step(self):
        s = self.s
        b1, b2 = 0.5, 0.999
        if self.K is not None:
            self.K.optim_adam(self.A, self.alpha_grad, self.adam_m, self.adam_v, self.adam_t, s["alpha_lr"], b1, b2,
                              s["alpha_weight_decay"], 1e-8, self.gA)
            return
        with torch.no_grad():
            g = self.alpha_grad + s["alpha_weight_decay"] * self.A
            self.adam_t.add_(1.0)
            self.adam_m.mul_(b1).add_(g, alpha=1 - b1)
            self.adam_v.mul_(b2).addcmul_(g, g, value=1 - b2)
            bc1 = 1 - torch.pow(b1, self.adam_t)
            bc2 = 1 - torch.pow(b2, self.adam_t)
            denom = (self.adam_v.sqrt() / bc2.sqrt()).add_(1e-8)
            self.A.sub_(self.adam_m / denom * (s["alpha_lr"] / bc1))

    def _seg_weight(self, tx, ty):
        if self.K is None:
            self.gW.zero_()
            self.gA.zero_()
        loss, logits = self._loss(tx, ty, self.Pw.views, *self._arch(self._fixed(self.Aw)), self.bn)
        self._backward(loss, self.Pw.list)
        self._fold(self.gW_rep)
        if self.hd is not None:
            self.loss_out, self.logits_out = loss.detach(), logits.detach()
            return
        with torch.no_grad():
            self.loss_out.copy_(loss.detach())
            if self.logits_out is None or self.logits_out.shape != logits.shape:
                self.logits_out = torch.empty_like(logits)
            self.logits_out.copy_(logits.detach())

    def _seg_weight_update(self):
        s = self.s
        if self.K is not None:
            nparts = self.K.optim_sumsq(self.gW, self._parts)
            self.K.optim_sgd_clip(self.W, self.gW, self.mom, self.lr, self._parts, nparts, s["w_grad_clip"],
                                  s["w_momentum"], s["w_weight_decay"], True)
            return
        with torch.no_grad():
            total = self.gW.norm()
            coef = torch.clamp(s["w_grad_clip"] / (total + 1e-6), max=1.0)
            self.gW.mul_(coef)
            d = self.gW.add(self.W, alpha=s["w_weight_decay"])
            self.mom.mul_(s["w_momentum"]).add_(d)
            self.W.sub_(self.mom * self.lr)

    def _segments(self):
        c = self.comm
        hd = None
        if self.device.type == "cuda":
            from ..ops import darts as dops

            if dops.backend() == "hip":
                from ..ops import hip_darts as hd
        begin = (lambda: hd.arena_begin(self.device, deferred_zero=self.net.net_function)) if hd else (lambda: None)
        end = hd.arena_end if hd else (lambda: None)
        return [
            (lambda: (begin(), self._seg_virtual(self.static["tx"], self.static["ty"])), [self.gW]),
            (lambda: self._seg_unrolled(self.static["vx"], self.static["vy"]), [self.gWv, self.gAv]),
            (lambda: self._seg_hessian(self.static["tx"], self.static["ty"]), [self.alpha_grad]),
            (lambda: (self._seg_alpha_step(), self._seg_weight(self.static["tx"], self.static["ty"])), [self.gW]),
            (lambda: (self._seg_weight_update(), end()), []),
        ]

    def _scope(self, sync=None):
        if self.hd is not None:
            return self.hd.sync_scope(sync if sync is not None else self._hsync)
        import contextlib

        return contextlib.nullcontext()

    def _run_eager(self):
        with self._scope():
            for fn, colls in self._segments():
                fn()
                for t in colls:
                    self.comm.allreduce_mean_(t)

    def _rendezvous(self) -> int:
        n = self.comm.calls
        for sy in (self._hsync, self._hsync_side):
            if sy is None:
                continue
            if sy.ws is not None:
                n += sy.folds
            elif sy.comm is not self.comm:
                n += sy.comm.calls
        return n

    def _side_folds(self) -> int:
        sy = self._hsync_side
        if sy is None:
            return 0
        return sy.folds if sy.ws is not None else sy.comm.calls

    def _build_graphs(self):
        segs = self._segments()
        whole = self.comm.graph_capturable([t for _, colls in segs for t in colls])
        groups, cur = [], []
        for fn, colls in segs:
            if whole:
                cur.append(lambda fn=fn, colls=colls: (fn(), [self.comm.allreduce_mean_(t) for t in colls]))
            else:
                cur.append(fn)
                if colls and self.comm.distributed:
                    groups.append((cur, colls))
                    cur = []
        if cur:
            groups.append((cur, []))
        s = torch.cuda.Stream()
        s.wait_stream(torch.cuda.current_stream())
        with torch.cuda.stream(s):
            for _ in range(2):
                self._snapshot_state()
                self._run_eager()
                self._restore_state()
        torch.cuda.current_stream().wait_stream(s)
        graphs = []
        n0 = self._rendezvous()
        side0 = self._side_folds()
        for fns, colls in groups:
            g = torch.cuda.CUDAGraph()
            with torch.cuda.graph(g), self._scope():
                for fn in fns:
                    fn()
            graphs.append((g, colls))
        self.graphs = graphs
        self.rendezvous_per_step = self._rendezvous() - n0 + (
            sum(len(c) for _, c in graphs) if self.comm.distributed else 0)
        self.rendezvous_serial_per_step = self.rendezvous_per_step - (self._side_folds() - side0)
        self.rendezvous_in_graph = not any(c for _, c in graphs)

    def _state_tensors(self):
        return [self.W, self.A, self.mom, self.adam_m, self.adam_v, self.adam_t, self.bn.mean, self.bn.var,
                self.bn_v.mean, self.bn_v.var]

    def _snapshot_state(self):
        self._saved = [t.clone() for t in self._state_tensors()]

    def _restore_state(self):
        with torch.no_grad():
            for t, s in zip(self._state_tensors(), self._saved):
                t.copy_(s)
        self._saved = None

    def set_lr(self, lr: float):
        self.lr.fill_(lr)

    def sync_bn_stats(self):
        if self.comm.distributed and not self.sync_bn:
            self.comm.allreduce_mean_(self.bn.mean)
            self.comm.allreduce_mean_(self.bn.var)

    def step(self, tx, ty, vx, vy):
        if self.static is None:
            self.static = {"tx": tx.clone(), "ty": ty.clone(), "vx": vx.clone(), "vy": vy.clone()}
        else:
            self.static["tx"].copy_(tx)
            self.static["ty"].copy_(ty)
            self.static["vx"].copy_(vx)
            self.static["vy"].copy_(vy)
        if self.capture:
            if self.graphs is None:
                self._build_graphs()
            for g, colls in self.graphs:
                g.replay()
                for t in colls:
                    self.comm.allreduce_mean_(t)
        else:
            n0, side0 = self._rendezvous(), self._side_folds()
            self._run_eager()
            self.rendezvous_per_step = self._rendezvous() - n0
            self.rendezvous_serial_per_step = self.rendezvous_per_step - (self._side_folds() - side0)
            self.rendezvous_in_graph = False
        return self.loss_out

    @torch.no_grad()
    def _evaluate(self, x, y):
        loss, logits = self.net.forward_loss(x, y, self.layout.views(self.W), *self._arch(self.Aw), self.bn,
                                             training=False)
        top1, top5 = accuracy(logits, y)
        return loss, top1, top5

    @torch.no_grad()
    def evaluate(self, x, y):
        if not self.capture:
            return self._evaluate(x, y)
        key = (tuple(x.shape), tuple(y.shape), x.dtype, y.dtype)
        ent = self._eval_graphs.get(key)
        if ent is None:
            sx, sy = x.clone(), y.clone()
            side = torch.cuda.Stream()
            side.wait_stream(torch.cuda.current_stream())
            with torch.cuda.stream(side):
                for _ in range(2):
                    self._evaluate(sx, sy)
            torch.cuda.current_stream().wait_stream(side)
            g = torch.cuda.CUDAGraph()
            with torch.cuda.graph(g):
                out = torch.stack(self._evaluate(sx, sy))
            ent = self._eval_graphs[key] = (g, sx, sy, out)
        g, sx, sy, out = ent
        sx.copy_(x)
        sy.copy_(y)
        g.replay()
        r = out.clone()
        return r[0], r[1], r[2]

    def train_metrics(self, y):
        top1, top5 = accuracy(self.logits_out, y)
        return float(self.loss_out), float(top1), float(top5)

    def genotype(self):
        from .darts import Genotype

        sp = self.layout.space
        normal = sp.parse([a.detach() for a in self.An], k=2)
        reduce = sp.parse([a.detach() for a in self.Ar], k=2) if self.Ar else []
        concat = range(2, 2 + self.layout.N)
        return Genotype(normal=normal, normal_concat=concat, reduce=reduce, reduce_concat=concat)
```

katib_amd/ops/hip_darts.py:

```python

from __future__ import annotations

import contextlib
import importlib
import weakref
from collections import defaultdict
from typing import Dict, List, Optional, Sequence, Tuple

import torch

from .. import _hipload

try:
    _K = _hipload.hipkern()
except ImportError as e:
    raise ImportError("katib_amd._hipkern is not built (run __graft_entry__.build()): %s" % e)

F64 = torch.float64
REP = int(_K.REP)
ZDT = torch.bfloat16 if bool(getattr(_K, "ZBF16", False)) else torch.float32


_SYNC = None


class SyncBN:

    def __init__(self, comm):
        self.comm, self.world = comm, comm.world_size
        self.ws = None
        if comm.xgmi is not None:
            from ..parallel import xgmi

            ar = xgmi.create(comm, capacity=1 << 16, blocks=16)
            self.ws = ar.ws if ar is not None else None
        self.rccl_graph = self.ws is None and comm.probe_rccl_capture()
        self.folds = 0

    @property
    def capturable(self) -> bool:
        return self.ws is not None or self.rccl_graph

    @property
    def path(self) -> str:
        return "xgmi-oneshot" if self.ws is not None else ("rccl-graph" if self.rccl_graph else "host")

    def fold(self, segs):
        self.folds += 1
        if self.ws is not None:
            self.ws.fold_sync(list(segs))
            return
        _K.fold_f64([tuple(sg[:3]) for sg in segs])
        self.comm.allreduce_sum_many_([sg[0][:sg[1]] for sg in segs if len(sg) < 4 or sg[3]])


class sync_scope:

    def __init__(self, sync):
        self.sync = sync

    def __enter__(self):
        global _SYNC
        self.prev, _SYNC = _SYNC, self.sync
        return self

    def __exit__(self, *exc):
        global _SYNC
        _SYNC = self.prev
        return False


def _world() -> int:
    return _SYNC.world if _SYNC is not None else 1


def _fold(segs):
    if not segs:
        return
    if _SYNC is not None and any(len(sg) < 4 or sg[3] for sg in segs):
        _SYNC.fold(segs)
    else:
        _K.fold_f64([tuple(sg[:3]) for sg in segs])


def _defer() -> bool:
    return _SYNC is None


_CAP = {"combine_fwd": 4, "dwpw_fwd_multi": 20, "pw_fwd": 16, "pool_fwd_multi": 8, "combine_bwd_reduce": 4,
        "pw_bwd": 16, "dw_bwd_multi": 20, "pool_bwd_multi": 8}
_REPLICATED: List[Tuple[weakref.ref, int]] = []


class _Arena:

    def __init__(self):
        self.buf: Optional[torch.Tensor] = None
        self.keep: List[torch.Tensor] = []
        self.off = 0
        self.used = 0
        self.need = 0
        self.active = False
        self.pending_zero = False


_ARENA = _Arena()


def arena_begin(device, deferred_zero: bool = False):
    a = _ARENA
    if a.need and (a.buf is None or a.buf.numel() < a.need):
        if a.buf is not None:
            a.keep.append(a.buf)
        a.buf = torch.zeros(a.need, dtype=F64, device=device)
        a.pending_zero = False
    elif a.buf is not None:
        if deferred_zero:
            a.pending_zero = True
        else:
            a.buf.zero_()
    a.off, a.used, a.active = 0, 0, True


def arena_end():
    a = _ARENA
    a.need = max(a.need, a.used)
    a.active = False
    if a.pending_zero:
        a.buf.zero_()
        a.pending_zero = False


def zeros64(n: int, device) -> torch.Tensor:
    a = _ARENA
    if a.active:
        if a.pending_zero and a.buf is not None:
            a.buf.zero_()
            a.pending_zero = False
        step = (n + 31) // 32 * 32
        a.used += step
        if a.buf is not None and a.off + step <= a.buf.numel() and a.buf.device == device:
            t = a.buf[a.off:a.off + n]
            a.off += step
            return t
    return torch.zeros(n, dtype=F64, device=device)


def register_grad_replicas(buf: torch.Tensor):
    if buf.dim() != 2 or buf.shape[0] != REP or not buf.is_contiguous() or buf.dtype != torch.float32:
        raise ValueError("replicated gradient buffer must be contiguous fp32 [%d][n]" % REP)
    _REPLICATED.append((weakref.ref(buf), buf.shape[1]))


def fold(buf: torch.Tensor):
    _K.fold_rows(buf)


def _replica_stride(g: torch.Tensor) -> int:
    ptr = g.data_ptr()
    for ref, n in list(_REPLICATED):
        buf = ref()
        if buf is None:
            _REPLICATED.remove((ref, n))
            continue
        base = buf.data_ptr()
        if base <= ptr and ptr + g.numel() * 4 <= base + n * 4:
            return n
    return 0


def _launch(name: str, calls: List, *args):
    cap = _CAP[name]
    fn = getattr(_K, name)
    for i in range(0, len(calls), cap):
        fn(calls[i:i + cap], *args)


def _unfolded(bn):
    return bn[:6] + (REP, bn[7])


NEEDED_GRADS = True
DROP_D = True


def _dwpw_multi(entries):
    _launch("dwpw_fwd_multi", entries)


def _pool_multi(entries):
    _launch("pool_fwd_multi", entries)


class EdgeSpec:

    def __init__(self, prims: Sequence[str], stride: int, pnames: List[str], slots: Dict[str, Tuple[int, ...]]):
        self.prims = list(prims)
        self.stride = stride
        self.pnames = pnames
        self.slots = slots
        self.nbn = sum(len(v) for v in slots.values())
        self.pidx = {n: i for i, n in enumerate(pnames)}


def _bn(stats: Optional[torch.Tensor], rm, rv, count: int, training: bool, eps: float, C: int):
    if training:
        return (stats, rm, rv, 1.0 / (count * _world()), False, eps, 1, 2 * C)
    return (None, rm, rv, 1.0 / count, True, eps, 1, 2 * C)


class _Sinks:

    def __init__(self):
        self.temps = []

    def get(self, p: torch.Tensor, key):
        if not p.requires_grad:
            return None, 0
        g = p.grad if p.is_leaf else None
        if g is not None and g.is_contiguous():
            stride = _replica_stride(g)
            if stride:
                return g, stride
        t = torch.zeros(REP, p.numel(), device=p.device, dtype=torch.float32)
        self.temps.append((key, t, g, p))
        return t[0].view_as(p), p.numel()

    def finish(self, grads: List):
        for key, t, g, p in self.temps:
            s = t.sum(0).view_as(p)
            if g is not None:
                g.add_(s)
            else:
                grads[key] = s


class _Edge:

    def __init__(self, i, x, w, spec: EdgeSpec, bn, params):
        self.i, self.x, self.w, self.spec, self.bn = i, x, w, spec, bn
        self.P = dict(zip(spec.pnames, params))
        self.S = spec.stride
        self.refs = []
        self.zs, self.bns, self.widx = {}, {}, []
        self.saved = {}
        self.id_idx, self.xid = -1, None
        self.upd = []


def _node_forward(xs, ws, specs, bns, params_list, training, momentum, eps, out=None, extra_fold=(), grad=True):
    E = len(specs)
    xs = [t.contiguous() for t in xs]
    N, C = xs[0].shape[:2]
    S0 = specs[0].stride
    Ho = (xs[0].shape[2] - 1) // S0 + 1
    Wo = (xs[0].shape[3] - 1) // S0 + 1
    cnt = N * Ho * Wo
    dev = xs[0].device
    slot = REP * 2 * C
    edges, off = [], 0
    for i in range(E):
        edges.append(_Edge(i, xs[i], ws[i], specs[i], bns[i], params_list[i]))
    nslots = sum(e.spec.nbn for e in edges)
    stats = zeros64(max(nslots, 1) * slot, dev) if training else None
    base = 0
    for e in edges:
        e.slot0 = base
        e.refs = [_bn(stats[(base + i) * slot:(base + i + 1) * slot] if training else None, e.bn[i][0],
                      e.bn[i][1], cnt, training, eps, C) for i in range(e.spec.nbn)]
        base += e.spec.nbn

    def st(e, i):
        return stats[(e.slot0 + i) * slot:(e.slot0 + i + 1) * slot] if training else None

    def new():
        return torch.empty(N, C, Ho, Wo, device=dev, dtype=ZDT)

    keep_d = not DROP_D or bool(_K.dwpw_split_path(C))

    def new_d(pw):
        return new() if keep_d or (grad and pw.requires_grad) else None

    dw_groups = defaultdict(list)
    pool_groups = defaultdict(list)
    fr_calls = []
    stage1, stage2 = [], []
    for e in edges:
        for k, prim in enumerate(e.spec.prims):
            if prim == "none":
                continue
            sl = e.spec.slots.get(prim, ())
            if prim.startswith("separable_convolution"):
                K = int(prim[-1])
                d1, z1 = new_d(e.P[prim + ".0.pw"]), new()
                dw_groups[(K, 1, e.S, K // 2)].append(
                    (e.x, e.P[prim + ".0.dw"], e.P[prim + ".0.pw"], None, d1, z1, st(e, sl[0])))
                e.saved[prim] = [d1, z1]
                stage1.append(e.slot0 + sl[0])
                stage2.append(e.slot0 + sl[1])
            elif prim.startswith("dilated_convolution"):
                K = int(prim[-1])
                d, z = new_d(e.P[prim + ".pw"]), new()
                dw_groups[(K, 2, e.S, (K // 2) * 2)].append(
                    (e.x, e.P[prim + ".dw"], e.P[prim + ".pw"], None, d, z, st(e, sl[0])))
                e.zs[k], e.bns[k] = z, e.refs[sl[0]]
                e.saved[prim] = (d, z)
                stage1.append(e.slot0 + sl[0])
            elif prim in ("avg_pooling_3x3", "max_pooling_3x3"):
                if "pool" not in e.saved:
                    za, zm = new(), new()
                    am = torch.empty(N, C, Ho, Wo, dtype=torch.uint8, device=dev)
                    sa = e.spec.slots.get("avg_pooling_3x3")
                    sm = e.spec.slots.get("max_pooling_3x3")
                    pool_groups[e.S].append((e.x, za, zm, st(e, sa[0]) if sa else None,
                                             st(e, sm[0]) if sm else None, am))
                    e.saved["pool"] = (za, zm, am)
                e.zs[k] = e.saved["pool"][0 if prim == "avg_pooling_3x3" else 1]
                e.bns[k] = e.refs[sl[0]]
                stage1.append(e.slot0 + sl[0])
            elif prim == "skip_connection":
                if e.S == 1:
                    e.id_idx, e.xid = k, e.x
                    continue
                z = new()
                fr_calls.append((e.x, e.P[prim + ".conv1"], z, st(e, sl[0]), 0, 0))
                fr_calls.append((e.x, e.P[prim + ".conv2"], z, st(e, sl[0]), C // 2, 1))
                e.zs[k], e.bns[k] = z, e.refs[sl[0]]
                e.saved[prim] = (z,)
                stage1.append(e.slot0 + sl[0])
            else:
                raise ValueError(prim)
            e.widx.append(k)
    dw1 = [(*c, K, dil, S, pad) for (K, dil, S, pad), calls in dw_groups.items() for c in calls]
    pools = [(*c, S) for S, calls in pool_groups.items() for c in calls]
    _dwpw_multi(dw1)
    _pool_multi(pools)
    if fr_calls:
        _launch("pw_fwd", fr_calls, 2)
    defer = training and _defer()
    if training and stage1 and not defer:
        _fold([(stats[i * slot:(i + 1) * slot], 2 * C, 2 * C) for i in sorted(set(stage1))])
    s2_groups = defaultdict(list)
    for e in edges:
        for k, prim in enumerate(e.spec.prims):
            if prim.startswith("separable_convolution"):
                K = int(prim[-1])
                sl = e.spec.slots[prim]
                d1, z1 = e.saved[prim]
                d2, z2 = new_d(e.P[prim + ".1.pw"]), new()
                inbn = _unfolded(e.refs[sl[0]]) if defer else e.refs[sl[0]]
                s2_groups[K].append((z1, e.P[prim + ".1.dw"], e.P[prim + ".1.pw"], inbn, d2, z2, st(e, sl[1])))
                e.upd.append(e.refs[sl[0]])
                e.zs[k], e.bns[k] = z2, e.refs[sl[1]]
                e.saved[prim] = (d1, z1, d2, z2)
    _dwpw_multi([(*c, K, 1, 1, K // 2) for K, calls in s2_groups.items() for c in calls])
    if training and (stage2 or (defer and stage1) or extra_fold):
        _fold([(stats[i * slot:(i + 1) * slot], 2 * C, 2 * C)
               for i in sorted(set(stage2 + (stage1 if defer else [])))] + list(extra_fold))
    if out is None:
        out = torch.empty(N, C, Ho, Wo, device=dev)
    ccalls = []
    for e in edges:
        e.zl = [e.zs[k] for k in e.widx]
        e.bl = [e.bns[k] for k in e.widx]
        ccalls.append((e.zl, e.bl, e.widx, e.w, e.id_idx, e.xid, e.upd if training else []))
    cap = _CAP["combine_fwd"]
    for i in range(0, E, cap):
        _K.combine_fwd(ccalls[i:i + cap], None, None, out, momentum, training, i > 0)
    return out, edges


def _node_backward(edges, training, C, dout, gx_of, take_first, sinks, pkey, cell_gw=None, live=None,
                   alpha_need=True):
    dout = dout.contiguous()
    dev = dout.device
    if live is None:
        live = [True] * len(edges)
    for e in edges:
        e.gw = None
    entries = [e for e in edges if alpha_need or live[e.i]]
    edges = [e for e in edges if live[e.i]]
    if not entries:
        return

    def sink(e, name):
        return sinks.get(e.P[name], pkey(e, name))

    sizes = []
    for e in entries:
        e.nred = (len(e.zl) + 1) * C + 1
        sizes.append(REP * (e.nred + e.w.numel()))
    buf = zeros64(sum(sizes), dev)
    o = 0
    calls, segs, gsegs = [], [], []
    for e, sz in zip(entries, sizes):
        e.red = buf[o:o + REP * e.nred]
        e.gw = buf[o + REP * e.nred:o + sz]
        o += sz
        calls.append((dout, e.zl, e.bl, e.x if e.id_idx >= 0 else None, e.red, e.widx, e.id_idx, e.gw))
        if live[e.i]:
            segs.append((e.red, e.nred, e.nred))
        gsegs.append((e.gw, e.w.numel(), e.w.numel(), False))
        segs.append(gsegs[-1])
    _launch("combine_bwd_reduce", calls)
    defer = training and _defer()
    nofold = defer and cell_gw is not None
    if nofold:
        cell_gw.extend(gsegs)
    if not defer:
        _fold(segs)

    r_early = REP if defer else 1
    r_late = REP if nofold else 1

    def src(e, k, z, rep=r_late):
        j = e.widx.index(k)
        return (dout, z, e.red[:C], e.red[(1 + j) * C:(2 + j) * C], e.bl[j], e.w, k, rep, e.nred)

    gxs = {e.i: gx_of(e.i) for e in edges}

    dils = [(e, k, p) for e in edges for k, p in enumerate(e.spec.prims) if p.startswith("dilated_convolution")]
    pwd, dd_of = [], {}
    for e, k, prim in dils:
        d, z = e.saved[prim]
        dd = torch.empty(z.shape, device=dev)
        dd_of[(e.i, prim)] = dd
        g, gst = sink(e, prim + ".pw")
        pwd.append((src(e, k, z, r_early), e.P[prim + ".pw"], d, e.x, dd, None, g, 0, 0, gst))
    seps = [(e, k, p) for e in edges for k, p in enumerate(e.spec.prims) if p.startswith("separable_convolution")]
    if not seps and pwd:
        _launch("pw_bwd", pwd, 1, 0, True)
    if not seps and defer and not nofold:
        _fold(segs)
    if seps:
        red1 = zeros64(len(seps) * REP * 2 * C, dev) if training else None
        pw2, dw2 = [], defaultdict(list)
        for n, (e, k, prim) in enumerate(seps):
            K = int(prim[-1])
            d1, z1, d2, z2 = e.saved[prim]
            dd2 = torch.empty(z2.shape, device=dev)
            g, gst = sink(e, prim + ".1.pw")
            pw2.append((src(e, k, z2, r_early), e.P[prim + ".1.pw"], d2, z1, dd2, None, g, 0, 0, gst))
            g1 = torch.empty(z1.shape, device=dev)
            r1 = red1[n * REP * 2 * C:(n + 1) * REP * 2 * C] if training else None
            g, gst = sink(e, prim + ".1.dw")
            dw2[K].append((z1, e.refs[e.spec.slots[prim][0]], e.P[prim + ".1.dw"], dd2, g1, g, r1, gst, False))
            e.saved[prim + "/g1"] = (g1, r1)
        _launch("pw_bwd", pw2 + pwd, 1, 0, True)
        _launch("dw_bwd_multi", [(*c, K) for K, calls in dw2.items() for c in calls])
        if training and not nofold:
            _fold([(red1[n * REP * 2 * C:(n + 1) * REP * 2 * C], 2 * C, 2 * C) for n in range(len(seps))]
                  + (segs if defer else []))
        pw1 = []
        for e, k, prim in seps:
            d1, z1, d2, z2 = e.saved[prim]
            g1, r1 = e.saved[prim + "/g1"]
            b1 = e.refs[e.spec.slots[prim][0]]
            gs1 = (g1, z1, r1[:C] if training else None, r1[C:2 * C] if training else None, b1, None, 0, r_late, 2 * C)
            dd1 = torch.empty(z1.shape, device=dev)
            e.saved[prim + "/dd1"] = dd1
            g, gst = sink(e, prim + ".0.pw")
            pw1.append((gs1, e.P[prim + ".0.pw"], d1, e.x, dd1, None, g, 0, 0, gst))
        _launch("pw_bwd", pw1, 1, 0, True)

    first = {e.i: take_first(e.i) for e in edges}

    def tf(i):
        f = first.get(i, False)
        first[i] = False
        return f

    def pool_srcs(e):
        za, zm, am = e.saved["pool"]
        ga = gm = None
        for k, p in enumerate(e.spec.prims):
            if p == "avg_pooling_3x3":
                ga = src(e, k, za)
            elif p == "max_pooling_3x3":
                gm = src(e, k, zm)
        return ga, gm, am

    convs, parts = [], defaultdict(list)
    for e, k, prim in seps + dils:
        sep = prim.startswith("separable_convolution")
        K = int(prim[-1])
        t = torch.empty_like(e.x)
        parts[e.i].append(t)
        name = prim + (".0.dw" if sep else ".dw")
        g, gst = sink(e, name)
        dd = e.saved[prim + "/dd1"] if sep else dd_of[(e.i, prim)]
        convs.append((e.x, None, e.P[name], dd, t, g, None, gst, True, K, 1 if sep else 2, e.S))
    _launch("dw_bwd_multi", convs)
    sums = []
    for e in edges:
        ga, gm, am = pool_srcs(e) if "pool" in e.saved else (None, None, None)
        ex = parts.get(e.i, [])
        if ga is None and gm is None and e.id_idx < 0 and not ex:
            continue
        sums.append((ga, gm, e.x, dout if e.id_idx >= 0 else None, e.w, e.id_idx, gxs[e.i], am, tf(e.i), e.S, ex))
    _launch("pool_bwd_multi", sums)
    frc = []
    for e in edges:
        if "skip_connection" in e.saved:
            if tf(e.i):
                gxs[e.i].zero_()
            k = e.spec.prims.index("skip_connection")
            (z,) = e.saved["skip_connection"]
            gs = src(e, k, z)
            g, gst = sink(e, "skip_connection.conv1")
            frc.append((gs, e.P["skip_connection.conv1"], None, e.x, None, gxs[e.i], g, 0, 0, gst))
            g, gst = sink(e, "skip_connection.conv2")
            frc.append((gs, e.P["skip_connection.conv2"], None, e.x, None, gxs[e.i], g, C // 2, 1, gst))
    if frc:
        _launch("pw_bwd", frc, 2, 1, True)


class _MixedNode(torch.autograd.Function):
    @staticmethod
    def forward(ctx, meta, *flat):
        specs, bns, training, momentum, eps, nparams, grad = meta
        E = len(specs)
        params, off = [], 2 * E
        for n in nparams:
            params.append(flat[off:off + n])
            off += n
        out, edges = _node_forward(flat[:E], flat[E:2 * E], specs, bns, params, training, momentum, eps, grad=grad)
        ctx.meta = (edges, training, out.shape[1])
        ctx.save_for_backward(*flat)
        return out

    @staticmethod
    def backward(ctx, dout):
        flat = ctx.saved_tensors
        edges, training, C = ctx.meta
        E = len(edges)
        sinks = _Sinks()
        pbase, acc = [], 2 * E
        for e in edges:
            pbase.append(acc)
            acc += len(e.spec.pnames)
        need = ctx.needs_input_grad
        live = [_edge_live(e, need[1 + e.i]) for e in edges]
        gxs = [torch.empty_like(e.x) if lv else None for e, lv in zip(edges, live)]
        first = [True] * E

        def take_first(i):
            f = first[i]
            first[i] = False
            return f

        _node_backward(edges, training, C, dout, lambda i: gxs[i], take_first, sinks,
                       lambda e, name: pbase[e.i] + e.spec.pidx[name], None, live, any(need[1 + E:1 + 2 * E]))
        for i in range(E):
            if first[i] and live[i]:
                gxs[i].zero_()
        grads = [None] * len(flat)
        for i, e in enumerate(edges):
            grads[i] = gxs[i] if need[1 + i] else None
            grads[E + i] = e.gw[:e.w.numel()].to(e.w.dtype) if need[1 + E + i] else None
        sinks.finish(grads)
        return (None, *grads)


def mixed_node(xs: Sequence[torch.Tensor], ws: Sequence[torch.Tensor], specs: Sequence[EdgeSpec],
               bns: Sequence[List[Tuple[torch.Tensor, torch.Tensor]]], params: Sequence[Sequence[torch.Tensor]],
               training: bool, momentum: float = 0.1, eps: float = 1e-5):
    meta = (list(specs), list(bns), training, momentum, eps, [len(p) for p in params], torch.is_grad_enabled())
    flat = list(xs) + list(ws) + [p for ps in params for p in ps]
    return _MixedNode.apply(meta, *flat)


def mixed_edge(x, w, spec: EdgeSpec, bn: List[Tuple[torch.Tensor, torch.Tensor]], params: Sequence[torch.Tensor],
               training: bool, momentum: float = 0.1, eps: float = 1e-5):
    return mixed_node([x], [w], [spec], [bn], [params], training, momentum, eps)


def _dims(x: torch.Tensor):
    if x.dim() == 5:
        return x.shape[1], x.shape[0] * x.shape[2], x.shape[3], x.shape[4]
    return tuple(x.shape)


def _stdconv_forward(x, rm, rv, training, momentum, eps, w1, w2, defer=None):
    x = x.contiguous()
    N, Cin, H, W = _dims(x)
    fr = w2 is not None
    Cout = w1.shape[0] * (2 if fr else 1)
    Ho, Wo = (H // 2, W // 2) if fr else (H, W)
    cnt = N * Ho * Wo
    stats = zeros64(REP * 2 * Cout, x.device) if training else None
    z = torch.empty(N, Cout, Ho, Wo, device=x.device, dtype=ZDT)
    if fr:
        _K.pw_fwd([(x, w1, z, stats, 0, 0), (x, w2, z, stats, Cout // 2, 1)], 2)
    else:
        _K.pw_fwd([(x, w1, z, stats, 0, 0)], 1)
    bn = _bn(stats, rm, rv, cnt, training, eps, Cout)
    late = defer is not None and training and _defer()
    if training and not late:
        _fold([(stats, 2 * Cout, 2 * Cout)])
    if late:
        defer.append((stats, 2 * Cout, 2 * Cout))
    out = torch.empty(z.shape, device=x.device)
    _K.combine_fwd([([z], [_unfolded(bn) if late else bn], [0], None, -1, None, [])], None, None, out, momentum,
                   training, False)
    return out, (x, z, w1, w2, bn, fr, Cout, training)


def _stdconv_backward(state, dout, need_x, sinks, keys, gx=None, first=True):
    x, z, w1, w2, bn, fr, Cout, training = state
    dout = dout.contiguous()
    nred = 2 * Cout + 1
    red = zeros64(REP * nred, x.device)
    late = training and _defer()
    if training:
        _K.combine_bwd_reduce([(dout, [z], [bn], None, red, [0], -1, None)])
        if not late:
            _fold([(red, nred, nred)])
    gs = (dout, z, red[:Cout], red[Cout:2 * Cout], bn, None, 0, REP if late else 1, nred)
    g1, s1 = sinks.get(w1, keys[0])
    given = gx is not None
    if fr:
        if need_x and not given:
            gx = torch.zeros_like(x)
        elif need_x and first:
            gx.zero_()
        g2, s2 = sinks.get(w2, keys[1])
        _K.pw_bwd([(gs, w1, None, x, None, gx, g1, 0, 0, s1), (gs, w2, None, x, None, gx, g2, Cout // 2, 1, s2)],
                  2, 1, need_x)
    else:
        if need_x and not given:
            gx = torch.empty_like(x)
        _K.pw_bwd([(gs, w1, None, x, None, gx, g1, 0, 0, s1, first or not given)], 1, 1, need_x)
    return gx if need_x else None


class _StdConvBN(torch.autograd.Function):
    @staticmethod
    def forward(ctx, x, rm, rv, training, momentum, eps, w1, w2):
        out, state = _stdconv_forward(x, rm, rv, training, momentum, eps, w1, w2)
        ctx.state = state
        ctx.save_for_backward(x, w1, *([w2] if w2 is not None else []))
        return out

    @staticmethod
    def backward(ctx, dout):
        sinks = _Sinks()
        grads = [None, None, None]
        gx = _stdconv_backward(ctx.state, dout, ctx.needs_input_grad[0], sinks, (1, 2))
        ctx.state = None
        sinks.finish(grads)
        return gx, None, None, None, None, None, grads[1], grads[2]


class CellSpec:

    def __init__(self, pre0, pre1, nodes, C):
        self.pre0, self.pre1, self.nodes, self.C = pre0, pre1, nodes, C
        self.names = list(pre0[1]) + list(pre1[1])
        for node in nodes:
            for _, pnames, _, _, _ in node:
                self.names += pnames
        self.index = {n: i for i, n in enumerate(self.names)}


def needed_grads(spec: CellSpec, need0: bool, need1: bool, wreq, alpha: bool) -> List[bool]:
    need = [need0 or any(wreq(n) for n in spec.pre0[1]), need1 or any(wreq(n) for n in spec.pre1[1])]
    for node in spec.nodes:
        need.append(any(alpha or need[src] or any(wreq(n) for n in pnames) for _, pnames, _, src, _ in node))
    return need


def network_needed_grads(spec: "NetSpec", wreq, alpha_n: bool, alpha_r: bool):
    need = [any(wreq(n) for n in spec.stem[:3])]
    i0 = i1 = 0
    cells = []
    for cspec, red in zip(spec.cells, spec.reduce):
        c = needed_grads(cspec, need[i0], need[i1], wreq, alpha_r if red else alpha_n)
        cells.append(c)
        need.append(any(c[2:]))
        i0, i1 = i1, len(need) - 1
    return need[0], cells


def _cell_fwd(spec, s0, s1, wts, P, bn_of, training, momentum, eps, grad=True):
    late = []

    def pre(x, p):
        kind, pnames, bname = p
        rm, rv = bn_of(bname)
        if kind == "fr":
            return _stdconv_forward(x, rm, rv, training, momentum, eps, P[pnames[0]], P[pnames[1]], late)
        return _stdconv_forward(x, rm, rv, training, momentum, eps, P[pnames[0]], None, late)
    t0, st0 = pre(s0, spec.pre0)
    t1, st1 = pre(s1, spec.pre1)
    states = [t0, t1]
    N, C = t0.shape[0], spec.C
    nn_ = len(spec.nodes)
    S = [e[0].stride for e in spec.nodes[0]]
    Ho = (t0.shape[2] - 1) // max(S) + 1 if S else t0.shape[2]
    Wo = (t0.shape[3] - 1) // max(S) + 1 if S else t0.shape[3]
    O = torch.empty(nn_, N, C, Ho, Wo, device=t0.device)
    node_states = []
    for i, node in enumerate(spec.nodes):
        xs = [states[src] for _, _, _, src, _ in node]
        ws = [wts[row] for _, _, _, _, row in node]
        specs = [es for es, _, _, _, _ in node]
        bns = [[bn_of(b) for b in bnames] for _, _, bnames, _, _ in node]
        plist = [[P[n] for n in pnames] for _, pnames, _, _, _ in node]
        out, edges = _node_forward(xs, ws, specs, bns, plist, training, momentum, eps, out=O[i],
                                   extra_fold=late if i == 0 else (), grad=grad)
        states.append(out)
        node_states.append(edges)
    return O, (spec, training, st0, st1, node_states, states, wts, P)


def _edge_live(e, src_need: bool) -> bool:
    return not NEEDED_GRADS or src_need or any(p.requires_grad for p in e.P.values())


def _cell_bwd(state, gO, sinks, pkey, gx0, first0, gx1, first1, need0, need1, alpha_rows=None, alpha_need=True):
    spec, training, st0, st1, node_states, states, wts, P = state
    nn_ = len(spec.nodes)
    if NEEDED_GRADS:
        need = needed_grads(spec, need0, need1, lambda n: P[n].requires_grad, alpha_need)
    else:
        need = [True] * (2 + nn_)
    gS = [None, None] + [gO[i] for i in range(nn_)]
    first = [True, True] + [False] * nn_
    ga_rows = [None] * nn_
    cell_gw = []
    for i in reversed(range(nn_)):
        if not need[2 + i]:
            continue
        node = spec.nodes[i]
        edges = node_states[i]
        srcs = [src for _, _, _, src, _ in node]
        live = [_edge_live(e, need[src]) for e, src in zip(edges, srcs)]
        for src, lv in zip(srcs, live):
            if lv and gS[src] is None:
                gS[src] = torch.empty_like(states[src])

        def take_first(k, srcs=srcs):
            f = first[srcs[k]]
            first[srcs[k]] = False
            return f

        _node_backward(edges, training, spec.C, gS[2 + i], lambda k, srcs=srcs: gS[srcs[k]], take_first, sinks,
                       lambda e, name, node=node: pkey(node[e.i][1][e.spec.pidx[name]]), cell_gw, live, alpha_need)
        if alpha_rows is not None:
            for e, (_, _, _, _, row) in zip(edges, node):
                if e.gw is not None:
                    alpha_rows.append((e.gw, e.w.numel(), wts[row], row))
        elif alpha_need:
            ga_rows[i] = [e.gw[:wts.shape[1]] for e in edges]
    gs = [None, None]
    for j, (st, needx, gx, fst, pre) in enumerate(((st0, need0, gx0, first0, spec.pre0),
                                                   (st1, need1, gx1, first1, spec.pre1))):
        if not need[j]:
            continue
        if first[j]:
            gS[j] = torch.zeros_like(states[j])
        gs[j] = _stdconv_backward(st, gS[j], needx, sinks, tuple(pkey(n) for n in pre[1]) + (None,), gx, fst)
    gw = None
    if alpha_rows is None and alpha_need:
        if cell_gw:
            _K.fold_f64(cell_gw)
        gw = torch.cat([g for rows in ga_rows for g in rows]).view(wts.shape).to(torch.float32)
    return gs[0], gs[1], gw


class _Cell(torch.autograd.Function):

    @staticmethod
    def forward(ctx, meta, s0, s1, wts, *params):
        spec, bn_of, training, momentum, eps, grad = meta
        P = dict(zip(spec.names, params))
        O, state = _cell_fwd(spec, s0, s1, wts, P, bn_of, training, momentum, eps, grad)
        nn_, N, C, Ho, Wo = O.shape
        y = O.permute(1, 0, 2, 3, 4).reshape(N, nn_ * C, Ho, Wo)
        ctx.cell = state
        ctx.save_for_backward(s0, s1, wts, *params)
        return y

    @staticmethod
    def backward(ctx, dy):
        state = ctx.cell
        ctx.cell = None
        spec = state[0]
        saved = ctx.saved_tensors
        params = saved[3:]
        nn_ = len(spec.nodes)
        N, C = dy.shape[0], spec.C
        Ho, Wo = dy.shape[2], dy.shape[3]
        gO = dy.reshape(N, nn_, C * Ho * Wo).transpose(0, 1).contiguous().view(nn_, N, C, Ho, Wo)
        sinks = _Sinks()
        need = ctx.needs_input_grad
        grads = [None] * (4 + len(params))
        gs0, gs1, gw = _cell_bwd(state, gO, sinks, lambda n: 4 + spec.index[n], None, True, None, True, need[1],
                                 need[2], None, need[3])
        grads[1], grads[2] = gs0, gs1
        if need[3]:
            grads[3] = gw
        sinks.finish(grads)
        return tuple(grads)


def cell_forward(spec: CellSpec, s0, s1, wts, params: Sequence[torch.Tensor], bn_of, training: bool,
                 momentum: float = 0.1, eps: float = 1e-5):
    return _Cell.apply((spec, bn_of, training, momentum, eps, torch.is_grad_enabled()), s0, s1, wts, *params)


def relu_conv_bn(x, w, rm, rv, training, momentum=0.1, eps=1e-5):
    return _StdConvBN.apply(x, rm, rv, training, momentum, eps, w, None)


def factorized_reduce_bn(x, w1, w2, rm, rv, training, momentum=0.1, eps=1e-5):
    return _StdConvBN.apply(x, rm, rv, training, momentum, eps, w1, w2)


def supported(x: torch.Tensor, stride: int) -> bool:
    if not x.is_cuda or x.dtype != torch.float32 or x.dim() != 4:
        return False
    N, C, H, W = x.shape
    Ho, Wo = (H - 1) // stride + 1, (W - 1) // stride + 1
    return (C <= 256 and C * C <= 4096 and Wo <= 64 and 64 % Wo == 0 and Ho % (64 // Wo) == 0
            and H == Ho * stride and W == Wo * stride)


class _StemConv(torch.autograd.Function):

    @staticmethod
    def forward(ctx, x, w):
        x, w = x.contiguous(), w.contiguous()
        N, _, H, W = x.shape
        y = torch.empty(N, w.shape[0], H, W, device=x.device, dtype=x.dtype)
        _K.stem_conv_fwd(x, w, y)
        ctx.save_for_backward(x, w)
        return y

    @staticmethod
    def backward(ctx, dy):
        x, w = ctx.saved_tensors
        dy = dy.contiguous()
        gx = gw = None
        if ctx.needs_input_grad[1]:
            chunks = stem_chunks(x, w.shape[0])
            partial = torch.empty(chunks, w.numel(), device=x.device, dtype=torch.float32)
            gw = torch.empty_like(w)
            _K.stem_conv_wgrad(x, dy, partial, gw)
        if ctx.needs_input_grad[0]:
            gx = torch.nn.grad.conv2d_input(x.shape, w, dy, padding=1)
        return gx, gw


def _stem_fwd(x, w, gamma, beta, rm, rv, momentum, eps):
    x, w = x.contiguous(), w.contiguous()
    N, _, H, W = x.shape
    C = w.shape[0]
    stats = zeros64(REP * 2 * C, x.device)
    z = torch.empty(N, C, H, W, device=x.device, dtype=x.dtype)
    _K.stem_conv_fwd_stats(x, w, z, stats)
    _fold([(stats, 2 * C, 2 * C)])
    bn = _bn(stats, rm, rv, N * H * W, True, eps, C)
    out = torch.empty_like(z)
    zs = z if ZDT == z.dtype else z.to(ZDT)
    _K.combine_fwd([([zs], [bn], [0], None, -1, None, [])], gamma, beta, out, momentum, True, False)
    return out, (x, w, gamma, beta, z, zs, bn, eps, stats)


def _stem_bwd(state, dout, sinks, keys, need):
    x, w, gamma, beta, z, zs, bn, eps, stats = state
    dout = dout.contiguous()
    C = w.shape[0]
    nred = 2 * C + 1
    red = zeros64(REP * nred, x.device)
    _K.combine_bwd_reduce([(dout, [zs], [bn], None, red, [0], -1, None)])
    _fold([(red, nred, nred)])
    gg, _ = sinks.get(gamma, keys[1]) if need[2] else (None, 0)
    gb, _ = sinks.get(beta, keys[2]) if need[3] else (None, 0)
    gw = gx = None
    if need[1] or need[2] or need[3]:
        chunks = stem_chunks(x, C)
        partial = torch.empty(chunks, w.numel(), device=x.device, dtype=torch.float32)
        if need[1]:
            gdst, _ = sinks.get(w, keys[0])
            _K.stem_conv_wgrad_bn(x, dout, z, red, stats, gamma, eps, gg, gb, partial, gdst, _world(), True)
        else:
            _K.stem_conv_wgrad_bn(x, dout, z, red, stats, gamma, eps, gg, gb, partial, torch.empty_like(w), _world())
    if need[0]:
        m = stats[:C] / z[:, 0].numel()
        var = (stats[C:2 * C] / z[:, 0].numel() - m * m).clamp_min(0)
        istd = torch.rsqrt(var.float() + eps).view(1, C, 1, 1)
        zhat = (z - m.float().view(1, C, 1, 1)) * istd
        m1 = (red[:C] / z[:, 0].numel()).float().view(1, C, 1, 1)
        m2 = (red[C:2 * C] / z[:, 0].numel()).float().view(1, C, 1, 1)
        dz = gamma.view(1, C, 1, 1) * istd * (dout - m1 - zhat * m2)
        gx = torch.nn.grad.conv2d_input(x.shape, w, dz, padding=1)
    return gx, gw


class _StemConvBN(torch.autograd.Function):

    @staticmethod
    def forward(ctx, x, w, gamma, beta, rm, rv, momentum, eps):
        out, state = _stem_fwd(x, w, gamma, beta, rm, rv, momentum, eps)
        ctx.stem = state
        return out

    @staticmethod
    def backward(ctx, dout):
        state = ctx.stem
        ctx.stem = None
        need = ctx.needs_input_grad
        grads = [None] * 8
        sinks = _Sinks()
        gx, _ = _stem_bwd(state, dout, sinks, (1, 2, 3), need[:4])
        grads[0] = gx
        sinks.finish(grads)
        return tuple(grads)


def stem_conv_bn(x, w, gamma, beta, rm, rv, momentum=0.1, eps=1e-5):
    return _StemConvBN.apply(x, w, gamma, beta, rm, rv, momentum, eps)


@torch.no_grad()
def stem_bn_eval(z, gamma, beta, rm, rv, eps=1e-5):
    z = z.contiguous()
    N, C, H, W = z.shape
    out = torch.empty(z.shape, device=z.device)
    zs = z if z.dtype == ZDT else z.to(ZDT)
    _K.combine_fwd([([zs], [_bn(None, rm, rv, N * H * W, False, eps, C)], [0], None, -1, None, [])], gamma, beta, out,
                   0.0, False, False)
    return out


def stem_chunks(x: torch.Tensor, cout: int) -> int:
    pixels = x.shape[0] * x.shape[2] * x.shape[3]
    return max(1, min(pixels // 1024, max(16, 1024 // cout)))


def stem_supported(x: torch.Tensor, w: torch.Tensor) -> bool:
    return (x.is_cuda and x.dtype == torch.float32 and w.dtype == torch.float32 and x.dim() == 4
            and x.shape[1] in (1, 3) and tuple(w.shape[1:]) == (x.shape[1], 3, 3) and w.shape[0] <= 64
            and x.numel() < (1 << 31) // 64)


def stem_conv(x: torch.Tensor, w: torch.Tensor) -> torch.Tensor:
    return _StemConv.apply(x, w)


class _Head(torch.autograd.Function):

    @staticmethod
    def forward(ctx, x, w, b, y):
        x = x.contiguous()
        N, C = x.shape[:2]
        K = w.shape[0]
        dev = x.device
        pooled = torch.empty(N, C, device=dev)
        logits = torch.empty(N, K, device=dev)
        dl = torch.empty(N, K, device=dev)
        loss_n = torch.empty(N, device=dev)
        loss = torch.empty((), device=dev)
        _K.head_fwd(x, w, b, y, pooled, logits, dl, loss_n)
        _K.head_loss(loss_n, loss)
        ctx.save_for_backward(dl, pooled, w, b)
        ctx.xshape = x.shape
        ctx.mark_non_differentiable(logits)
        ctx.set_materialize_grads(False)
        return loss, logits

    @staticmethod
    def backward(ctx, gloss, _glogits):
        dl, pooled, w, b = ctx.saved_tensors
        grads = [None, None, None, None]
        if gloss is None:
            return tuple(grads)
        need = ctx.needs_input_grad
        dev = dl.device
        x_like = torch.empty((), device=dev).expand(ctx.xshape)
        dx = torch.empty(ctx.xshape, device=dev) if need[0] else None
        sinks = _Sinks()
        gw, sw = sinks.get(w, 1) if need[1] else (None, 0)
        gb, sb = sinks.get(b, 2) if need[2] else (None, 0)
        _K.head_bwd(x_like, dl, pooled, w, gloss.reshape(()).contiguous().float(), dx, gw, sw, gb, sb)
        grads[0] = dx
        sinks.finish(grads)
        return tuple(grads)


def head_supported(x: torch.Tensor, w: torch.Tensor, y: torch.Tensor) -> bool:
    return (x.is_cuda and x.dim() == 4 and x.dtype == torch.float32 and w.dtype == torch.float32
            and w.dim() == 2 and w.shape[1] == x.shape[1] and x.shape[1] <= 1024 and w.shape[0] <= 64
            and y.dtype == torch.int64 and y.dim() == 1 and y.shape[0] == x.shape[0])


def head_loss(x: torch.Tensor, w: torch.Tensor, b: torch.Tensor, y: torch.Tensor):
    return _Head.apply(x, w, b, y.contiguous())


class NetSpec:

    def __init__(self, stem, cells, reduce, head):
        self.stem, self.cells, self.reduce, self.head = stem, list(cells), list(reduce), head
        names = list(stem[:3])
        for c in self.cells:
            names += c.names
        names += list(head)
        self.names = names
        self.index = {n: i for i, n in enumerate(names)}


ALPHA_GRAD_MAX = 128


def _alpha_grad(entries):
    groups = defaultdict(list)
    for ent in entries:
        groups[ent[3].data_ptr()].append(ent)
    chunk = []
    for rows in groups.values():
        if len(rows) > ALPHA_GRAD_MAX:
            raise ValueError("alpha_grad: %d entries share one destination row, the kernel takes at most %d"
                             % (len(rows), ALPHA_GRAD_MAX))
        if chunk and len(chunk) + len(rows) > 64:
            _K.alpha_grad(chunk, True)
            chunk = []
        chunk += rows
    if chunk:
        _K.alpha_grad(chunk, True)


class _Network(torch.autograd.Function):

    @staticmethod
    def forward(ctx, meta, x, y, an, ar, *params):
        spec, bn_of, training, momentum, eps, grad = meta
        P = dict(zip(spec.names, params))
        dev = x.device
        mats, outs = [an], [torch.empty_like(an)]
        if ar is not None:
            mats.append(ar)
            outs.append(torch.empty_like(ar))
        zero = None
        a = _ARENA
        if training and a.pending_zero and a.buf is not None and a.buf.device == dev:
            zero, a.pending_zero = a.buf, False
        _K.alpha_softmax(mats, outs, zero)
        wn, wr = outs[0], (outs[1] if ar is not None else None)
        conv, gamma, beta, bname = spec.stem
        rm, rv = bn_of(bname)
        if training:
            s, st_stem = _stem_fwd(x, P[conv], P[gamma], P[beta], rm, rv, momentum, eps)
        else:
            s, st_stem = stem_bn_eval(stem_conv(x, P[conv]), P[gamma], P[beta], rm, rv, eps), None
        tensors = [s]
        cells = []
        i0 = i1 = 0
        for cspec, red in zip(spec.cells, spec.reduce):
            O, st = _cell_fwd(cspec, tensors[i0], tensors[i1], wr if red else wn, P, bn_of, training, momentum, eps,
                              grad)
            tensors.append(O)
            cells.append((st, i0, i1, len(tensors) - 1, red))
            i0, i1 = i1, len(tensors) - 1
        feat = tensors[i1]
        hw, hb = spec.head
        N, C = _dims(feat)[:2]
        K = P[hw].shape[0]
        pooled = torch.empty(N, C, device=dev)
        logits = torch.empty(N, K, device=dev)
        dl = torch.empty(N, K, device=dev)
        loss_n = torch.empty(N, device=dev)
        loss = torch.empty((), device=dev)
        _K.head_fwd(feat, P[hw], P[hb], y, pooled, logits, dl, loss_n)
        _K.head_loss(loss_n, loss)
        ctx.net = (spec, P, training, st_stem, cells, tensors, i1, dl, pooled, an, ar)
        ctx.mark_non_differentiable(logits)
        ctx.set_materialize_grads(False)
        return loss, logits

    @staticmethod
    def backward(ctx, gloss, _glogits):
        spec, P, training, st_stem, cells, tensors, last, dl, pooled, an, ar = ctx.net
        ctx.net = None
        grads = [None] * (5 + len(spec.names))
        if gloss is None:
            return tuple(grads)
        need = ctx.needs_input_grad
        sinks = _Sinks()

        def key(n):
            return 5 + spec.index[n]
        alpha = {False: bool(need[3]), True: ar is not None and bool(need[4])}
        if NEEDED_GRADS:
            stem_need, plans = network_needed_grads(spec, lambda n: P[n].requires_grad, alpha[False], alpha[True])
            needT = [stem_need] + [any(c[2:]) for c in plans]
        else:
            needT = [True] * len(tensors)
        g, first = {}, {}
        if needT[last]:
            g[last], first[last] = torch.empty_like(tensors[last]), False
        hw, hb = spec.head
        gw, sw = sinks.get(P[hw], key(hw)) if need[key(hw)] else (None, 0)
        gb, sb = sinks.get(P[hb], key(hb)) if need[key(hb)] else (None, 0)
        if needT[last] or gw is not None or gb is not None:
            _K.head_bwd(tensors[last], dl, pooled, P[hw], gloss.reshape(()).contiguous().float(), g.get(last), gw, sw,
                        gb, sb)
        rows = []
        for st, i0, i1, io, red in reversed(cells):
            if not needT[io]:
                continue
            for i in (i0, i1):
                if needT[i] and i not in g:
                    g[i], first[i] = torch.empty_like(tensors[i]), True
            f0 = first.get(i0, False)
            f1 = first.get(i1, False) and i1 != i0
            cell_rows = []
            _cell_bwd(st, g[io], sinks, key, g.get(i0), f0, g.get(i1), f1, needT[i0], needT[i1], cell_rows, alpha[red])
            for i in (i0, i1):
                if needT[i]:
                    first[i] = False
            rows += [(r, red) for r in cell_rows]
        dst = {}
        for red, leaf, idx in ((False, an, 3), (True, ar, 4)):
            if leaf is None or not need[idx]:
                continue
            if leaf.is_leaf and leaf.grad is not None and leaf.grad.is_contiguous() and leaf.grad.dtype == torch.float32:
                dst[red] = leaf.grad
            else:
                dst[red] = grads[idx] = torch.zeros_like(leaf)
        ents = [(gw_, rs, wrow, dst[red][row]) for (gw_, rs, wrow, row), red in rows if red in dst]
        if ents:
            _alpha_grad(ents)
        conv, gamma, beta, _ = spec.stem
        flags = (False, need[key(conv)], need[key(gamma)], need[key(beta)])
        if training and st_stem is not None and 0 in g and (any(flags) or not NEEDED_GRADS):
            _stem_bwd(st_stem, g[0], sinks, (key(conv), key(gamma), key(beta)), flags)
        sinks.finish(grads)
        return tuple(grads)


_MERGE_CAP = {"pw_fwd": 32, "combine_bwd_reduce": 8, "pw_bwd": 32, "dw_bwd_multi": 40, "dwpw_fwd_multi": 40,
              "pool_fwd_multi": 16, "pool_bwd_multi": 16, "fold_f64": 128, "alpha_grad": 128, "__sync_fold__": 64}
_QUERIES = {"max_blocks", "stamps_compiled", "REP", "ZBF16", "OPTIM_MAX_PARTS", "dwpw_split_path"}


class _Recorder:

    def __init__(self, real, tape, sync=False):
        self._real, self._tape, self._sync = real, tape, sync

    def __getattr__(self, name):
        attr = getattr(self._real, name)
        if self._sync:
            if name != "fold":
                return attr
            name = "__sync_fold__"
        elif name in _QUERIES or not callable(attr):
            return attr

        def rec(*args, **kw):
            self._tape.append((name, args, kw))
            return None

        return rec


def _same(x, y) -> bool:
    if torch.is_tensor(x) or torch.is_tensor(y):
        return x is y
    if isinstance(x, (list, tuple)) and isinstance(y, (list, tuple)):
        return len(x) == len(y) and all(_same(a, b) for a, b in zip(x, y))
    return x == y


class stacked_passes:

    def __init__(self):
        self.tapes: List[list] = []
        self.stats = {"launches": 0, "merged": 0}

    def __enter__(self):
        return self

    @contextlib.contextmanager
    def pass_(self):
        global _K, _SYNC
        tape: list = []
        self.tapes.append(tape)
        real_k, real_sync = _K, _SYNC
        _K = _Recorder(real_k, tape)
        if real_sync is not None:
            _SYNC = _Recorder(real_sync, tape, sync=True)
        try:
            yield
        finally:
            _K, _SYNC = real_k, real_sync

    def _call(self, name, args, kw):
        self.stats["launches"] += 1
        if name == "__sync_fold__":
            _SYNC.fold(*args, **kw)
        else:
            getattr(_K, name)(*args, **kw)

    def __exit__(self, et, ev, tb):
        if et is not None:
            return False
        tapes = self.tapes
        if not tapes:
            return False
        if len(tapes) != 2 or len(tapes[0]) != len(tapes[1]) or any(a[0] != b[0] for a, b in zip(*tapes)):
            for t in tapes:
                for name, args, kw in t:
                    self._call(name, args, kw)
            return False
        self._replay_merged(tapes)
        return False

    def _replay_merged(self, tapes):
        for (name, aa, ka), (_, ab, kb) in zip(*tapes):
            cap = _MERGE_CAP.get(name)
            if (cap and aa and ab and isinstance(aa[0], list) and isinstance(ab[0], list)
                    and len(aa[0]) + len(ab[0]) <= cap and len(aa) == len(ab) and _same(aa[1:], ab[1:])
                    and _same(sorted(ka.items()), sorted(kb.items()))):
                self.stats["merged"] += 1
                self._call(name, (list(aa[0]) + list(ab[0]),) + tuple(aa[1:]), ka)
            else:
                self._call(name, aa, ka)
                self._call(name, ab, kb)


def network_loss(spec: NetSpec, x, y, params: Sequence[torch.Tensor], an, ar, bn_of, training: bool,
                 momentum: float = 0.1, eps: float = 1e-5):
    return _Network.apply((spec, bn_of, training, momentum, eps, torch.is_grad_enabled()), x, y, an, ar, *params)
```

katib_amd/parallel/comm.py:

```python

from __future__ import annotations

import datetime
import os
from typing import Optional

import torch
import torch.distributed as dist


class Comm:
    def __init__(self, rank: int = 0, world_size: int = 1, local_rank: int = 0, backend: Optional[str] = None,
                 device: Optional[torch.device] = None, group=None):
        self.rank, self.world_size, self.local_rank = rank, world_size, local_rank
        self.backend = backend
        self.device = device or torch.device("cpu")
        self.group = group
        self.xgmi = None
        self._rccl_capture = None
        self.calls = 0
        self.xgmi_status = None

    @staticmethod
    def from_env(device_type: Optional[str] = None, backend: Optional[str] = None) -> "Comm":
        ws = int(os.environ.get("WORLD_SIZE", "1"))
        rank = int(os.environ.get("RANK", "0"))
        lrank = int(os.environ.get("LOCAL_RANK", str(rank)))
        lws = int(os.environ.get("LOCAL_WORLD_SIZE", str(ws)))
        if device_type is None:
            device_type = "cuda" if torch.cuda.is_available() else "cpu"
        shared = False
        if device_type == "cuda":
            ndev = max(1, torch.cuda.device_count())
            idx = lrank % ndev
            shared = lws > ndev
            torch.cuda.set_device(idx)
            device = torch.device("cuda", idx)
        else:
            device = torch.device("cpu")
        want = backend
        backend = None
        if ws > 1:
            backend = want or os.environ.get("KATIB_AMD_DIST_BACKEND") or (
                "nccl" if device_type == "cuda" and not shared else "gloo")
            if backend == "nccl" and (shared or device_type != "cuda"):
                backend = "gloo"
            if not dist.is_initialized():
                os.environ.setdefault("MASTER_ADDR", "127.0.0.1")
                kw = {}
                if backend == "nccl":
                    kw["device_id"] = device
                dist.init_process_group(backend, rank=rank, world_size=ws,
                                        timeout=datetime.timedelta(seconds=600), **kw)
        return Comm(rank, ws, lrank, backend, device)

    @property
    def distributed(self) -> bool:
        return self.world_size > 1

    def enable_xgmi(self) -> bool:
        if self.xgmi is None and self.world_size > 1 and self.device.type == "cuda":
            from . import xgmi

            self.xgmi = xgmi.create(self)
            if self.xgmi is not None:
                self.xgmi_status = "passed" if self.distinct_devices() == self.world_size else "passed (same device)"
            elif os.environ.get("KATIB_AMD_XGMI", "1") == "0":
                self.xgmi_status = "disabled"
            elif int(os.environ.get("LOCAL_WORLD_SIZE", str(self.world_size))) != self.world_size \
                    or self.world_size > 8:
                self.xgmi_status = "not applicable (ranks span nodes or > 8)"
            else:
                self.xgmi_status = "failed"
        return self.xgmi is not None

    def device_identity(self) -> str:
        import socket

        if self.device.type != "cuda":
            return "%s/cpu" % socket.gethostname()
        p = torch.cuda.get_device_properties(self.device)
        ident = str(getattr(p, "uuid", "") or "")
        pci = tuple(getattr(p, k, -1) for k in ("pci_domain_id", "pci_bus_id", "pci_device_id"))
        if not ident or ident.strip("0-") == "":
            ident = "pci%s" % (pci,)
        return "%s/%s" % (socket.gethostname(), ident)

    def distinct_devices(self) -> int:
        if getattr(self, "_distinct", None) is None:
            if self.world_size <= 1:
                self._distinct = 1
            else:
                ids = [None] * self.world_size
                dist.all_gather_object(ids, self.device_identity(), group=self.group)
                self._distinct = len(set(ids))
        return self._distinct

    def subgroup(self) -> "Comm":
        if self.world_size <= 1:
            return Comm(self.rank, 1, self.local_rank, self.backend, self.device)
        g = dist.new_group(backend=self.backend)
        c = Comm(self.rank, self.world_size, self.local_rank, self.backend, self.device, group=g)
        t = torch.zeros(1, device=self.device if self.backend == "nccl" else "cpu")
        dist.all_reduce(t, group=g)
        return c

    def probe_rccl_capture(self) -> bool:
        if self._rccl_capture is not None:
            return self._rccl_capture
        ok = (self.world_size > 1 or dist.is_initialized()) and self.backend == "nccl" and \
            self.device.type == "cuda" and os.environ.get("KATIB_AMD_RCCL_CAPTURE", "1") != "0"
        if not ok or self.backend != "nccl":
            self._rccl_capture = False
            return False
        g = None
        x = torch.zeros(64, device=self.device, dtype=torch.float64)
        try:
            dist.all_reduce(x, group=self.group)
            torch.cuda.synchronize(self.device)
            g = torch.cuda.CUDAGraph()
            with torch.cuda.graph(g):
                dist.all_reduce(x, group=self.group)
        except Exception:
            ok, g = False, None
        ok = self._agree(ok)
        if ok:
            try:
                for _ in range(2):
                    x.fill_(float(self.rank + 1))
                    g.replay()
                torch.cuda.synchronize(self.device)
                ok = bool((x == self.world_size * (self.world_size + 1) / 2.0).all())
            except Exception:
                ok = False
            ok = self._agree(ok)
        self._rccl_capture = ok
        return ok

    def _agree(self, ok: bool) -> bool:
        t = torch.tensor([1 if ok else 0], dtype=torch.int32, device=self.device)
        dist.all_reduce(t, op=dist.ReduceOp.MIN, group=self.group)
        return bool(int(t.item()))

    @property
    def rccl_capturable(self) -> bool:
        return bool(self._rccl_capture)

    def graph_capturable(self, tensors) -> bool:
        if self.world_size == 1:
            return True
        if self.xgmi is not None and all(self.xgmi.fits(t) for t in tensors):
            return True
        return self.probe_rccl_capture()

    def _coll(self, fn, t: torch.Tensor, *a, **kw) -> torch.Tensor:
        self.calls += 1
        if self.group is not None:
            kw["group"] = self.group
        if self.backend == "gloo" and t.is_cuda:
            h = t.cpu()
            fn(h, *a, **kw)
            t.copy_(h)
        else:
            fn(t, *a, **kw)
        return t

    def allreduce_mean_(self, t: torch.Tensor) -> torch.Tensor:
        if self.world_size > 1:
            if self.xgmi is not None and self.xgmi.fits(t):
                self.calls += 1
                self.xgmi.allreduce_(t, average=True)
            elif self.backend == "nccl":
                self._coll(dist.all_reduce, t, op=dist.ReduceOp.AVG)
            else:
                self._coll(dist.all_reduce, t)
                t.div_(self.world_size)
        return t

    def allreduce_sum_(self, t: torch.Tensor) -> torch.Tensor:
        if self.world_size > 1:
            if self.xgmi is not None and self.xgmi.fits(t):
                self.calls += 1
                self.xgmi.allreduce_(t)
            else:
                self._coll(dist.all_reduce, t)
        return t

    def allreduce_sum_many_(self, ts) -> None:
        ts = list(ts)
        if self.world_size <= 1 or not ts:
            return
        if self.backend == "nccl" and len(ts) > 1:
            from torch.distributed.distributed_c10d import _coalescing_manager

            self.calls += 1
            with _coalescing_manager(group=self.group, device=self.device):
                for t in ts:
                    dist.all_reduce(t, group=self.group)
            return
        for t in ts:
            self.allreduce_sum_(t)

    def allreduce_max(self, x: float) -> float:
        if self.world_size <= 1:
            return x
        t = torch.tensor([x], dtype=torch.float64, device=self.device)
        self._coll(dist.all_reduce, t, op=dist.ReduceOp.MAX)
        return float(t.item())

    def broadcast_(self, t: torch.Tensor, src: int = 0) -> torch.Tensor:
        if self.world_size > 1:
            self._coll(dist.broadcast, t, src)
        return t

    def barrier(self):
        if self.world_size > 1:
            if self.backend == "nccl":
                dist.barrier(group=self.group, device_ids=[self.device.index])
            else:
                dist.barrier(group=self.group)

    def destroy(self):
        if self.world_size > 1 and dist.is_initialized():
            dist.destroy_process_group()
```

katib_amd/utils/graphcheck.py:

```python

from __future__ import annotations

import ctypes

import torch

_HIP = None
POISON_WORD = 0x7FC07FC0


def _hip():
    global _HIP
    if _HIP is None:
        _HIP = ctypes.CDLL("libamdhip64.so")
    return _HIP


def poison_graph_pool(graph: "torch.cuda.CUDAGraph") -> int:
    pool = tuple(graph.pool())
    torch.cuda.synchronize()
    n = 0
    for seg in torch.cuda.memory._snapshot()["segments"]:
        if tuple(seg.get("segment_pool_id", (0, 0))) != pool:
            continue
        err = _hip().hipMemsetD32(ctypes.c_void_p(seg["address"]), ctypes.c_int(POISON_WORD),
                                  ctypes.c_size_t(seg["total_size"] // 4))
        if err != 0:
            raise RuntimeError("hipMemsetD32 failed: %d" % err)
        n += seg["total_size"]
    torch.cuda.synchronize()
    return n
```

katib_amd/workloads/common.py:

```python

from __future__ import annotations

import os
import time
from typing import Callable, Dict, Optional, Tuple

import torch


def device() -> torch.device:
    if torch.cuda.is_available():
        local = int(os.environ.get("LOCAL_RANK", "0"))
        torch.cuda.set_device(local % max(1, torch.cuda.device_count()))
        return torch.device("cuda", torch.cuda.current_device())
    return torch.device("cpu")


def process_start_time() -> float:
    try:
        with open("/proc/self/stat") as f:
            start_ticks = int(f.read().rsplit(")", 1)[1].split()[19])
        with open("/proc/stat") as f:
            btime = next(int(ln.split()[1]) for ln in f if ln.startswith("btime"))
        return btime + start_ticks / os.sysconf("SC_CLK_TCK")
    except (OSError, ValueError, StopIteration, IndexError):
        return float("nan")


def phase(name: str, t: Optional[float] = None):
    if os.environ.get("KATIB_AMD_TRIAL_PHASES") == "1":
        print("katib-phase %s %.6f" % (name, time.time() if t is None else t), flush=True)


def report(**metrics):
    print(" ".join("%s=%s" % (k, _fmt(v)) for k, v in metrics.items()), flush=True)


def _fmt(v):
    if isinstance(v, float):
        return "%.6g" % v
    return str(v)


def teacher_vectors(n: int, dim: int = 784, classes: int = 10, seed: int = 0, dev=None, noise: float = 0.5,
                    label_noise: float = 0.05):
    g = torch.Generator().manual_seed(seed)
    T = torch.randn(dim, classes, generator=g) / dim ** 0.5
    if dev is not None and torch.device(dev).type == "cuda":
        gd = torch.Generator(device=dev).manual_seed(seed + 7919)
        x = torch.randn(n, dim, generator=gd, device=dev)
        y = (x @ T.to(dev) + noise * torch.randn(n, classes, generator=gd, device=dev) / dim ** 0.5).argmax(1)
        flip = torch.rand(n, generator=gd, device=dev) < label_noise
        return x, torch.where(flip, torch.randint(0, classes, (n,), generator=gd, device=dev), y)
    x = torch.randn(n, dim, generator=g)
    y = (x @ T + noise * torch.randn(n, classes, generator=g) / dim ** 0.5).argmax(1)
    flip = torch.rand(n, generator=g) < label_noise
    y = torch.where(flip, torch.randint(0, classes, (n,), generator=g), y)
    return x.to(dev), y.to(dev)


def pattern_images(n: int, shape=(3, 32, 32), classes: int = 10, seed: int = 0, dev=None, noise: float = 1.5,
                   dtype=torch.float32, modes: int = 3, shift: int = 4, label_noise: float = 0.1):
    g = torch.Generator().manual_seed(seed)
    C, H, W = shape
    up = lambda t: torch.nn.functional.interpolate(t, size=(H, W), mode="bilinear", align_corners=False)
    bank = up(torch.randn(6, C, H // 4, W // 4, generator=g))
    own = up(torch.randn(classes * modes, C, H // 8, W // 8, generator=g))
    mix = torch.randint(0, bank.shape[0], (classes * modes,), generator=g)
    protos = bank[mix] + 0.6 * own
    y = torch.randint(0, classes, (n,), generator=g)
    out = torch.empty(n, C, H, W, dtype=dtype, device=dev)
    on_gpu = dev is not None and torch.device(dev).type == "cuda"
    gs = torch.Generator(device=dev).manual_seed(seed + 7919) if on_gpu else g
    sdev = dev if on_gpu else None
    protos_s, y_s = (protos.to(dev), y.to(dev)) if on_gpu else (protos, y)
    chunk = 16384 if on_gpu else 4096
    for i in range(0, n, chunk):
        yi = y_s[i:i + chunk]
        m = len(yi)
        pid = yi * modes + torch.randint(0, modes, (m,), generator=gs, device=sdev)
        xi = protos_s[pid] * (0.5 + torch.rand(m, 1, 1, 1, generator=gs, device=sdev))
        if shift:
            dy = torch.randint(-shift, shift + 1, (m,), generator=gs, device=sdev)
            dx = torch.randint(-shift, shift + 1, (m,), generator=gs, device=sdev)
            rows = (torch.arange(H, device=sdev).view(1, H) - dy.view(m, 1)) % H
            cols = (torch.arange(W, device=sdev).view(1, W) - dx.view(m, 1)) % W
            xi = xi[torch.arange(m, device=sdev).view(m, 1, 1, 1), torch.arange(C, device=sdev).view(1, C, 1, 1),
                    rows.view(m, 1, H, 1), cols.view(m, 1, 1, W)]
        xi = xi + noise * torch.randn(m, C, H, W, generator=gs, device=sdev)
        out[i:i + chunk] = xi.to(device=dev, dtype=dtype)
    flip = torch.rand(n, generator=g) < label_noise
    y = torch.where(flip, torch.randint(0, classes, (n,), generator=g), y)
    return out, y.to(dev)


def markov_tokens(n_tokens: int, vocab: int = 50257, seed: int = 0, dev=None, fanout: int = 8):
    g = torch.Generator().manual_seed(seed)
    succ = torch.randint(0, vocab, (vocab, fanout), generator=g)
    chains = 1024
    steps = (n_tokens + chains - 1) // chains
    toks = torch.empty(chains, steps, dtype=torch.long)
    state = torch.randint(0, vocab, (chains,), generator=g)
    for i in range(steps):
        toks[:, i] = state
        state = succ[state, torch.randint(0, fanout, (chains,), generator=g)]
    return toks.reshape(-1)[:n_tokens].to(dev)


def global_avg_pool(x: torch.Tensor) -> torch.Tensor:
    return torch.nn.functional.avg_pool2d(x, (x.shape[2], x.shape[3])).flatten(1)


class CapturedStep:

    def __init__(self, fn: Callable[[], torch.Tensor], enabled: bool = True, warmup: int = 3,
                 no_miopen: bool = False):
        if no_miopen:
            inner = fn

            def fn():
                with torch.backends.cudnn.flags(enabled=False):
                    return inner()
        self.fn = fn
        self.enabled = enabled and torch.cuda.is_available()
        self.warmup = warmup
        self.graph = None
        self.out = None
        self.calls = 0

    def __call__(self):
        if not self.enabled:
            return self.fn()
        if self.graph is None:
            if self.calls < self.warmup:
                s = torch.cuda.Stream()
                s.wait_stream(torch.cuda.current_stream())
                with torch.cuda.stream(s):
                    out = self.fn()
                torch.cuda.current_stream().wait_stream(s)
                self.calls += 1
                return out
            self.graph = torch.cuda.CUDAGraph()
            with torch.cuda.graph(self.graph):
                self.out = self.fn()
        self.graph.replay()
        return self.out


class Timer:
    def __init__(self):
        self.t0 = time.time()

    def elapsed(self) -> float:
        if torch.cuda.is_available():
            torch.cuda.synchronize()
        return time.time() - self.t0
```

Baseline: 2.002 s.

## Share pool backward across edges reading the same source state

Restructures the pool backward kernel so that one launch handles up to four edges that read the same source state and stride. Their BN-backward coefficients and gradient sources are combined into a single pass over the shared saved pool outputs and argmax. Python groups the live edges by (source, stride) and launches the shared entries once every member edge has been processed. Separately, graph capture is wrapped so that Python GC is disabled during capture. The cost is a more complex kernel with more per-thread registers and branching on the source count.

```diff
diff --git a/katib_amd/csrc/hip/darts_bind.cpp b/katib_amd/csrc/hip/darts_bind.cpp
--- a/katib_amd/csrc/hip/darts_bind.cpp
+++ b/katib_amd/csrc/hip/darts_bind.cpp
@@ -466,46 +466,107 @@
   }
 }
 
+static PoolGradPart make_pool_part(const py::tuple& t, int C, bool eval) {
+  PoolGradPart g{};
+  TORCH_CHECK(t.size() == 7, "pool grad part has 7 fields");
+  OptT s1 = t[0].cast<OptT>(), s2 = t[1].cast<OptT>(), rvar = t[6].cast<OptT>();
+  Tensor w = t[2].cast<Tensor>();
+  check_f32(w, "w");
+  g.w = w.data_ptr<float>();
+  g.widx = t[3].cast<int>();
+  TORCH_CHECK(g.widx >= 0 && g.widx < w.numel(), "pool_bwd: weight index out of range");
+  g.rep = t[4].cast<int>();
+  g.rstride = t[5].cast<int>();
+  TORCH_CHECK(g.rep >= 1 && g.rep <= kRep, "replicas");
+  if (eval) {
+    TORCH_CHECK(rvar.has_value() && rvar->defined(), "eval-mode pool backward needs the edge's running variance");
+    check_f32(*rvar, "rvar");
+    TORCH_CHECK(rvar->numel() == C, "rvar [C]");
+    g.rvar = rvar->data_ptr<float>();
+    return g;
+  }
+  TORCH_CHECK(s1.has_value() && s1->defined() && s2.has_value() && s2->defined(),
+              "training-mode BN backward needs S1/S2 reductions");
+  for (const OptT* sv : {&s1, &s2})
+    TORCH_CHECK((*sv)->scalar_type() == at::kDouble && (*sv)->is_cuda() &&
+                    storage_doubles_after(**sv) >= (int64_t)(g.rep - 1) * g.rstride + C,
+                "S1/S2 replicas exceed their buffer");
+  g.S1 = s1->data_ptr<double>();
+  g.S2 = s2->data_ptr<double>();
+  return g;
+}
+
 void pool_bwd_multi(std::vector<py::tuple> calls) {
   check_batch<PoolBwdBatch>(calls);
   PoolBwdBatch bt{};
   bt.n = calls.size();
   for (int i = 0; i < bt.n; ++i) {
     const py::tuple& t = calls[i];
-    const int64_t S = t[9].cast<int64_t>();
+    TORCH_CHECK(t.size() == 10, "pool_bwd entry has 10 fields");
+    const int64_t S = t[8].cast<int64_t>();
     TORCH_CHECK(S == 1 || S == 2, "pool stride must be 1 or 2");
-    bt.e[i].S = (int)S;
-    auto ga = t[0].cast<c10::optional<py::tuple>>(), gm = t[1].cast<c10::optional<py::tuple>>();
-    Tensor x = t[2].cast<Tensor>();
-    OptT dout_id = t[3].cast<OptT>(), w = t[4].cast<OptT>();
-    const int id_idx = t[5].cast<int>();
-    Tensor gx = t[6].cast<Tensor>();
-    OptT amax = t[7].cast<OptT>();
+    OptT za = t[0].cast<OptT>(), zm = t[1].cast<OptT>(), amax = t[4].cast<OptT>();
+    auto bna = t[2].cast<c10::optional<py::tuple>>(), bnm = t[3].cast<c10::optional<py::tuple>>();
+    Tensor x = t[5].cast<Tensor>(), gx = t[6].cast<Tensor>();
     check_f32(x, "x"); check_f32(gx, "gx");
+    TORCH_CHECK(x.dim() == 4, "x must be NCHW");
     PoolBwdArgs& a = bt.e[i];
+    a.S = (int)S;
     a.N = x.size(0); a.C = x.size(1); a.H = x.size(2); a.W = x.size(3);
     a.Ho = (a.H - 1) / S + 1; a.Wo = (a.W - 1) / S + 1;
     TORCH_CHECK(a.Ho * a.Wo <= 8192, "pool_bwd stages one output plane in LDS (Ho*Wo <= 8192)");
     TORCH_CHECK(gx.sizes() == x.sizes(), "gx shape");
-    TORCH_CHECK(!gm.has_value() || (amax.has_value() && amax->defined() && amax->scalar_type() == at::kByte &&
-                                    amax->numel() == (int64_t)a.N * a.C * a.Ho * a.Wo),
-                "max-pool backward needs the uint8 argmax from pool_fwd");
-    if (amax.has_value() && amax->defined()) a.amax = amax->data_ptr<uint8_t>();
-    if (ga.has_value()) a.ga = make_gs(*ga, a.C);
-    if (gm.has_value()) a.gm = make_gs(*gm, a.C);
-    a.x = x.data_ptr<float>(); a.dout_id = ptr_or_null<float>(dout_id); a.w = ptr_or_null<float>(w);
-    if (a.dout_id) TORCH_CHECK(dout_id->sizes() == x.sizes(), "identity gradient shape");
-    a.id_idx = id_idx; a.gx = gx.data_ptr<float>();
-    a.overwrite = t[8].cast<bool>();
-    if (t.size() > 10) {
-      auto ex = t[10].cast<std::vector<Tensor>>();
-      TORCH_CHECK(ex.size() <= 4, "pool_bwd: at most 4 extra gradient parts");
-      a.nextra = ex.size();
+    const int64_t onumel = (int64_t)a.N * a.C * a.Ho * a.Wo;
+    const bool has_a = za.has_value() && za->defined(), has_m = zm.has_value() && zm->defined();
+    if (has_a) {
+      check_z(*za, "zavg");
+      TORCH_CHECK(za->numel() == onumel && bna.has_value(), "avg-pool backward needs zavg [N][C][Ho][Wo] and its BN");
+      a.za = zptr(*za);
+      a.bna = make_bn(*bna, a.C);
+    }
+    if (has_m) {
+      check_z(*zm, "zmax");
+      TORCH_CHECK(zm->numel() == onumel && bnm.has_value(), "max-pool backward needs zmax [N][C][Ho][Wo] and its BN");
+      TORCH_CHECK(amax.has_value() && amax->defined() && amax->is_cuda() && amax->scalar_type() == at::kByte &&
+                      amax->is_contiguous() && amax->numel() == onumel,
+                  "max-pool backward needs the uint8 argmax from pool_fwd");
+      a.zm = zptr(*zm);
+      a.bnm = make_bn(*bnm, a.C);
+      a.amax = amax->data_ptr<uint8_t>();
+    }
+    a.gx = gx.data_ptr<float>();
+    a.overwrite = t[7].cast<bool>();
+    auto srcs = t[9].cast<std::vector<py::tuple>>();
+    TORCH_CHECK(!srcs.empty() && (int)srcs.size() <= kMaxShare, "pool_bwd: 1..", kMaxShare, " sources per entry");
+    a.nsrc = srcs.size();
+    for (int e = 0; e < a.nsrc; ++e) {
+      const py::tuple& u = srcs[e];
+      TORCH_CHECK(u.size() == 6, "pool_bwd source has 6 fields");
+      PoolBwdSrc& sr = a.src[e];
+      Tensor dout = u[0].cast<Tensor>();
+      check_f32(dout, "dout");
+      TORCH_CHECK(dout.numel() == onumel, "dout must be [N][C][Ho][Wo]");
+      sr.dout = dout.data_ptr<float>();
+      auto pa = u[1].cast<c10::optional<py::tuple>>(), pm = u[2].cast<c10::optional<py::tuple>>();
+      TORCH_CHECK((!pa.has_value() || has_a) && (!pm.has_value() || has_m), "pool_bwd: a source's pool lacks its z");
+      if (pa.has_value()) sr.a = make_pool_part(*pa, a.C, a.bna.eval);
+      if (pm.has_value()) sr.m = make_pool_part(*pm, a.C, a.bnm.eval);
+      OptT w_id = u[3].cast<OptT>();
+      sr.id_idx = u[4].cast<int>();
+      if (w_id.has_value() && w_id->defined() && sr.id_idx >= 0) {
+        check_f32(*w_id, "w");
+        TORCH_CHECK(S == 1, "the identity skip is stride 1");
+        TORCH_CHECK(sr.id_idx < w_id->numel(), "id_idx out of range");
+        sr.w_id = w_id->data_ptr<float>();
+      }
+      auto ex = u[5].cast<std::vector<Tensor>>();
+      TORCH_CHECK(ex.size() <= 4, "pool_bwd: at most 4 extra gradient parts per source");
+      sr.nextra = ex.size();
       for (size_t j = 0; j < ex.size(); ++j) {
         check_f32(ex[j], "extra");
         TORCH_CHECK(ex[j].sizes() == gx.sizes(), "extra gradient part shape");
         TORCH_CHECK(ex[j].data_ptr() != gx.data_ptr(), "extra part aliases gx");
-        a.extra[j] = ex[j].data_ptr<float>();
+        sr.extra[j] = ex[j].data_ptr<float>();
       }
     }
     SAME_SHAPE(bt, N); SAME_SHAPE(bt, C);
@@ -578,6 +639,7 @@
   m.def("fold_rows", &fold_rows);
   m.def("fold_f64", &fold_f64);
   m.attr("REP") = kRep;
+  m.attr("POOL_SHARE") = kMaxShare;
   m.attr("ZBF16") = kZbf16;
   m.def("max_blocks", &max_blocks);
   m.def("dwpw_split_path", [](int64_t C) { return dwpw_split_path((int)C); });
diff --git a/katib_amd/csrc/hip/darts_ops.h b/katib_amd/csrc/hip/darts_ops.h
--- a/katib_amd/csrc/hip/darts_ops.h
+++ b/katib_amd/csrc/hip/darts_ops.h
@@ -142,10 +142,27 @@
   double* p[kMaxSeg]; int n[kMaxSeg]; int rstride[kMaxSeg]; int nseg; int total;
 };
 
+constexpr int kMaxShare = 4;
+struct PoolGradPart {
+  const double* S1;
+  const double* S2;
+  const float* w;
+  const float* rvar;
+  int widx, rep, rstride;
+};
+struct PoolBwdSrc {
+  const float* dout;
+  PoolGradPart a, m;
+  const float* w_id;
+  int id_idx;
+  const float* extra[4]; int nextra;
+};
 struct PoolBwdArgs {
-  GradSrc ga; GradSrc gm; const float* x; const float* dout_id; const float* w; int id_idx; float* gx;
+  const zt* za; const zt* zm;
+  BNRef bna, bnm;
   const unsigned char* amax;
-  const float* extra[4]; int nextra;
+  float* gx;
+  PoolBwdSrc src[kMaxShare]; int nsrc;
   int overwrite;
   int N, C, H, W, Ho, Wo;
   int S;
diff --git a/katib_amd/csrc/hip/darts_ops_dwb.hip b/katib_amd/csrc/hip/darts_ops_dwb.hip
--- a/katib_amd/csrc/hip/darts_ops_dwb.hip
+++ b/katib_amd/csrc/hip/darts_ops_dwb.hip
@@ -141,8 +141,14 @@
     for (int i = tid; i < C * KK; i += 256) atomicAdd(a.gW + (size_t)rep_slot() * a.gstride + i, sGW[i]);
 }
 
+__device__ __forceinline__ float wave_uniform(float v) {
+  return __int_as_float(__builtin_amdgcn_readfirstlane(__float_as_int(v)));
+}
+
+typedef const PoolBwdSrc __attribute__((address_space(4))) * PoolSrcPtr;
+
 template <int S, bool V4 = false>
-__device__ __forceinline__ void pool_bwd_body(const PoolBwdArgs& a, const int bx) {
+__device__ __forceinline__ void pool_bwd_body(const PoolBwdArgs& a, PoolSrcPtr src, const int bx) {
   const int C = a.C, H = a.H, W = a.W, Ho = a.Ho, Wo = a.Wo, HWo = Ho * Wo;
   const int nc = bx, c = nc % C;
   const size_t ob = (size_t)nc * HWo;
@@ -150,25 +156,44 @@
   float* sGa = smem;
   float* sGm = smem + HWo;
   unsigned char* sArg = (unsigned char*)(smem + 2 * HWo);
-  __shared__ float sCo[8];
+  __shared__ float sCo[4 + 4 * kMaxShare];
   KSTAMP(0);
-  if (threadIdx.x < 64) {
+  if (threadIdx.x < 16 * (2 + 2 * kMaxShare)) {
     const int grp = threadIdx.x >> 4, j = threadIdx.x & 15;
-    const GradSrc& gs = grp & 1 ? a.gm : a.ga;
-    const bool on = gs.z != nullptr, stats = grp < 2;
-    const BNRef& b = gs.bn;
+    const bool stats = grp < 2;
+    const BNRef& b = grp & 1 ? a.bnm : a.bna;
+    const bool on = (grp & 1 ? a.zm != nullptr : a.za != nullptr);
+    const double* p1 = nullptr;
+    size_t off2 = 0;
+    int rep = 0, rs = 0;
+#pragma unroll
+    for (int e = 0; e < kMaxShare; ++e) {
+      if (e < a.nsrc && (grp >> 1) == e + 1) {
+        const float* gw = grp & 1 ? src[e].m.w : src[e].a.w;
+        const double* g1 = grp & 1 ? src[e].m.S1 : src[e].a.S1;
+        const double* g2 = grp & 1 ? src[e].m.S2 : src[e].a.S2;
+        const int grep = grp & 1 ? src[e].m.rep : src[e].a.rep;
+        const int grs = grp & 1 ? src[e].m.rstride : src[e].a.rstride;
+        if (gw && g1) {
+          p1 = g1;
+          off2 = g2 - g1;
+          rep = grep;
+          rs = grep == 1 ? 0 : grs;
+        }
+      }
+    }
     double s = 0.0, s2 = 0.0;
-    if (on && stats && !b.eval) {
-      for (int r = j; r < b.rep; r += 16) {
-        s += b.sums[(size_t)r * b.rstride + c];
-        s2 += b.sums[(size_t)r * b.rstride + b.C + c];
-      }
-    } else if (on && !stats && !gs.eval) {
-      const int rep = gs.rep, rs = gs.rep == 1 ? 0 : gs.rstride;
-      const size_t off2 = gs.S2 - gs.S1;
+    if (stats) {
+      if (on && !b.eval) {
+        for (int r = j; r < b.rep; r += 16) {
+          s += b.sums[(size_t)r * b.rstride + c];
+          s2 += b.sums[(size_t)r * b.rstride + b.C + c];
+        }
+      }
+    } else if (p1) {
       for (int r = j; r < rep; r += 16) {
-        s += gs.S1[(size_t)r * rs + c];
-        s2 += gs.S1[(size_t)r * rs + off2 + c];
+        s += p1[(size_t)r * rs + c];
+        s2 += p1[(size_t)r * rs + off2 + c];
       }
     }
 #pragma unroll
@@ -177,14 +202,11 @@
       s2 += __shfl_xor(s2, o, 64);
     }
     if (j == 0) {
-      float* o = sCo + 4 * (grp & 1) + (stats ? 0 : 2);
-      if (!on) {
-        o[0] = 0.f;
-        o[1] = stats ? 1.f : 0.f;
-      } else if (stats) {
-        if (b.eval) {
-          o[0] = b.rmean[c];
-          o[1] = rsqrtf(b.rvar[c] + b.eps);
+      float* o = sCo + 2 * grp;
+      if (stats) {
+        if (!on || b.eval) {
+          o[0] = 0.f;
+          o[1] = 1.f;
         } else {
           const double m = s * (double)b.inv_count;
           double v = s2 * (double)b.inv_count - m * m;
@@ -193,54 +215,83 @@
           o[1] = rsqrtf((float)v + b.eps);
         }
       } else {
-        o[0] = gs.eval ? 0.f : (float)(s * (double)gs.bn.inv_count);
-        o[1] = gs.eval ? 0.f : (float)(s2 * (double)gs.bn.inv_count);
+        o[0] = (float)(s * (double)b.inv_count);
+        o[1] = (float)(s2 * (double)b.inv_count);
       }
     }
   }
   __syncthreads();
   KSTAMP(1);
-  const float ma = sCo[0], ia = sCo[1], a1 = a.ga.z ? sCo[2] : 0.f, a2 = a.ga.z ? sCo[3] : 0.f;
-  const float mm = sCo[4], im = sCo[5], m1 = a.gm.z ? sCo[6] : 0.f, m2 = a.gm.z ? sCo[7] : 0.f;
-  const float wa = a.ga.w ? a.ga.w[a.ga.widx] : 0.f;
-  const float wm = a.gm.w ? a.gm.w[a.gm.widx] : 0.f;
-  const float wid = (a.w && a.id_idx >= 0) ? a.w[a.id_idx] : 0.f;
+  const float ma = wave_uniform(sCo[0]), ia = wave_uniform(sCo[1]), mm = wave_uniform(sCo[2]), im = wave_uniform(sCo[3]);
+  float ca[kMaxShare], a1[kMaxShare], a2[kMaxShare], cm[kMaxShare], m1[kMaxShare], m2[kMaxShare], wid[kMaxShare];
+#pragma unroll
+  for (int e = 0; e < kMaxShare; ++e) {
+    ca[e] = cm[e] = wid[e] = 0.f;
+    a1[e] = wave_uniform(sCo[4 + 4 * e]);
+    a2[e] = wave_uniform(sCo[5 + 4 * e]);
+    m1[e] = wave_uniform(sCo[6 + 4 * e]);
+    m2[e] = wave_uniform(sCo[7 + 4 * e]);
+    if (e < a.nsrc) {
+      if (a.za && src[e].a.w)
+        ca[e] = src[e].a.w[src[e].a.widx] * (a.bna.eval ? rsqrtf(src[e].a.rvar[c] + a.bna.eps) : ia);
+      if (a.zm && src[e].m.w)
+        cm[e] = src[e].m.w[src[e].m.widx] * (a.bnm.eval ? rsqrtf(src[e].m.rvar[c] + a.bnm.eps) : im);
+      if (src[e].w_id) wid[e] = src[e].w_id[src[e].id_idx];
+    }
+  }
   if constexpr (V4) {
     typedef float f4 __attribute__((ext_vector_type(4)));
-    const float* gsrc = a.ga.z ? a.ga.g : a.gm.g;
     for (int o4 = threadIdx.x * 4; o4 < HWo; o4 += 1024) {
-      const f4 g = *reinterpret_cast<const f4*>(gsrc + ob + o4);
-      if (a.ga.z) {
-        const f4 z = zld4(a.ga.z + ob + o4);
-        const f4 d = wa * ia * (g - a1 - ((z - ma) * ia) * a2);
-#pragma unroll
-        for (int t = 0; t < 4; ++t) {
-          const int o = o4 + t, oy = o / Wo, ox = o - oy * Wo;
-          const int y0 = max(oy * S - 1, 0), y1 = min(oy * S + 1, H - 1);
-          const int x0 = max(ox * S - 1, 0), x1 = min(ox * S + 1, W - 1);
-          sGa[o] = d[t] / (float)((y1 - y0 + 1) * (x1 - x0 + 1));
-        }
-      } else {
-        *reinterpret_cast<f4*>(sGa + o4) = f4{0.f, 0.f, 0.f, 0.f};
-      }
-      if (a.gm.z) {
-        const f4 z = zld4(a.gm.z + ob + o4);
-        *reinterpret_cast<f4*>(sGm + o4) = wm * im * (g - m1 - ((z - mm) * im) * m2);
-        *reinterpret_cast<unsigned*>(sArg + o4) = *reinterpret_cast<const unsigned*>(a.amax + ob + o4);
-      } else {
-        *reinterpret_cast<f4*>(sGm + o4) = f4{0.f, 0.f, 0.f, 0.f};
-        *reinterpret_cast<unsigned*>(sArg + o4) = 0xffffffffu;
-      }
+      f4 za4 = {0.f, 0.f, 0.f, 0.f}, zm4 = {0.f, 0.f, 0.f, 0.f}, gd[kMaxShare];
+      unsigned am4 = 0xffffffffu;
+      if (a.za) za4 = zld4(a.za + ob + o4);
+      if (a.zm) {
+        zm4 = zld4(a.zm + ob + o4);
+        am4 = *reinterpret_cast<const unsigned*>(a.amax + ob + o4);
+      }
+#pragma unroll
+      for (int e = 0; e < kMaxShare; ++e) {
+        gd[e] = f4{0.f, 0.f, 0.f, 0.f};
+        if (e < a.nsrc && ((a.za && src[e].a.w) || (a.zm && src[e].m.w)))
+          gd[e] = *reinterpret_cast<const f4*>(src[e].dout + ob + o4);
+      }
+      const f4 zha = (za4 - ma) * ia, zhm = (zm4 - mm) * im;
+      f4 da = {0.f, 0.f, 0.f, 0.f}, dm = {0.f, 0.f, 0.f, 0.f};
+#pragma unroll
+      for (int e = 0; e < kMaxShare; ++e) {
+        da += ca[e] * (gd[e] - a1[e] - zha * a2[e]);
+        dm += cm[e] * (gd[e] - m1[e] - zhm * m2[e]);
+      }
+#pragma unroll
+      for (int t = 0; t < 4; ++t) {
+        const int o = o4 + t, oy = o / Wo, ox = o - oy * Wo;
+        const int y0 = max(oy * S - 1, 0), y1 = min(oy * S + 1, H - 1);
+        const int x0 = max(ox * S - 1, 0), x1 = min(ox * S + 1, W - 1);
+        sGa[o] = da[t] / (float)((y1 - y0 + 1) * (x1 - x0 + 1));
+      }
+      *reinterpret_cast<f4*>(sGm + o4) = dm;
+      *reinterpret_cast<unsigned*>(sArg + o4) = am4;
     }
     __syncthreads();
     KSTAMP(2);
     const size_t pb = (size_t)nc * H * W;
     for (int q4 = threadIdx.x * 4; q4 < H * W; q4 += 1024) {
       f4 g = {0.f, 0.f, 0.f, 0.f};
-      if (a.dout_id) g = wid * *reinterpret_cast<const f4*>(a.dout_id + pb + q4);
-#pragma unroll
-      for (int j = 0; j < 4; ++j)
-        if (j < a.nextra) g += *reinterpret_cast<const f4*>(a.extra[j] + pb + q4);
+#pragma unroll
+      for (int e = 0; e < kMaxShare; ++e) {
+        if (e < a.nsrc) {
+          f4 dv = {0.f, 0.f, 0.f, 0.f}, xv[4];
+          if (src[e].w_id) dv = *reinterpret_cast<const f4*>(src[e].dout + pb + q4);
+#pragma unroll
+          for (int j = 0; j < 4; ++j) {
+            xv[j] = f4{0.f, 0.f, 0.f, 0.f};
+            if (j < src[e].nextra) xv[j] = *reinterpret_cast<const f4*>(src[e].extra[j] + pb + q4);
+          }
+          g += wid[e] * dv;
+#pragma unroll
+          for (int j = 0; j < 4; ++j) g += xv[j];
+        }
+      }
       const int iy = q4 / W, ix0 = q4 - iy * W;
       if constexpr (S == 1) {
         float wa[3][6], wm[3][6];
@@ -343,20 +394,22 @@
   }
   for (int o = threadIdx.x; o < HWo; o += 256) {
     int oy = o / Wo, ox = o % Wo;
-    if (a.ga.z) {
-      int y0 = max(oy * S - 1, 0), y1 = min(oy * S + 1, H - 1);
-      int x0 = max(ox * S - 1, 0), x1 = min(ox * S + 1, W - 1);
-      sGa[o] = bn_bwd_val(a.ga, ob + o, ma, ia, wa, a1, a2) / (float)((y1 - y0 + 1) * (x1 - x0 + 1));
-    } else {
-      sGa[o] = 0.f;
-    }
-    if (a.gm.z) {
-      sGm[o] = bn_bwd_val(a.gm, ob + o, mm, im, wm, m1, m2);
-      sArg[o] = a.amax[ob + o];
-    } else {
-      sGm[o] = 0.f;
-      sArg[o] = 255;
-    }
+    const float zha = a.za ? (z2f(a.za[ob + o]) - ma) * ia : 0.f;
+    const float zhm = a.zm ? (z2f(a.zm[ob + o]) - mm) * im : 0.f;
+    float da = 0.f, dm = 0.f;
+#pragma unroll
+    for (int e = 0; e < kMaxShare; ++e) {
+      if (e < a.nsrc && ((a.za && src[e].a.w) || (a.zm && src[e].m.w))) {
+        const float g = src[e].dout[ob + o];
+        if (a.za && src[e].a.w) da += ca[e] * (g - a1[e] - zha * a2[e]);
+        if (a.zm && src[e].m.w) dm += cm[e] * (g - m1[e] - zhm * m2[e]);
+      }
+    }
+    int y0 = max(oy * S - 1, 0), y1 = min(oy * S + 1, H - 1);
+    int x0 = max(ox * S - 1, 0), x1 = min(ox * S + 1, W - 1);
+    sGa[o] = da / (float)((y1 - y0 + 1) * (x1 - x0 + 1));
+    sGm[o] = dm;
+    sArg[o] = a.zm ? a.amax[ob + o] : 255;
   }
   __syncthreads();
   for (int q = threadIdx.x; q < H * W; q += 256) {
@@ -372,10 +425,15 @@
         if (sArg[o] == tap) g += sGm[o];
       }
     }
-    if (a.dout_id) g += wid * a.dout_id[(size_t)nc * H * W + q];
-#pragma unroll
-    for (int j = 0; j < 4; ++j)
-      if (j < a.nextra) g += a.extra[j][(size_t)nc * H * W + q];
+#pragma unroll
+    for (int e = 0; e < kMaxShare; ++e) {
+      if (e < a.nsrc) {
+        if (src[e].w_id) g += wid[e] * src[e].dout[(size_t)nc * H * W + q];
+#pragma unroll
+        for (int j = 0; j < 4; ++j)
+          if (j < src[e].nextra) g += src[e].extra[j][(size_t)nc * H * W + q];
+      }
+    }
     if (a.overwrite) a.gx[(size_t)nc * H * W + q] = g;
     else a.gx[(size_t)nc * H * W + q] += g;
   }
@@ -385,8 +443,10 @@
 __global__ void __launch_bounds__(256) pool_bwd_multi_kernel(PoolBwdBatch bt) {
   const PoolBwdArgs a = bt.e[blockIdx.y];
   if ((int)blockIdx.x >= a.N * a.C) return;
-  if (a.S == 1) pool_bwd_body<1, V4>(a, blockIdx.x);
-  else pool_bwd_body<2, V4>(a, blockIdx.x);
+  typedef const PoolBwdBatch __attribute__((address_space(4))) * BatchPtr;
+  PoolSrcPtr src = ((BatchPtr)__builtin_amdgcn_kernarg_segment_ptr())->e[blockIdx.y].src;
+  if (a.S == 1) pool_bwd_body<1, V4>(a, src, blockIdx.x);
+  else pool_bwd_body<2, V4>(a, src, blockIdx.x);
 }
 
 
@@ -740,10 +800,12 @@
     const PoolBwdArgs& a = b.e[i];
     maxblk = std::max(maxblk, a.N * a.C);
     lds = std::max(lds, sizeof(float) * 2 * a.Ho * a.Wo + a.Ho * a.Wo + 16);
-    v4 = v4 && (a.Ho * a.Wo) % 4 == 0 && (a.H * a.W) % 4 == 0 && a.W % 4 == 0 && al(a.ga.g, 16) && al(a.gm.g, 16) &&
-         al(a.ga.z, 4 * sizeof(zt)) && al(a.gm.z, 4 * sizeof(zt)) && al(a.amax, 4) && al(a.dout_id, 16) &&
-         al(a.gx, 16) && (!a.ga.z || !a.gm.z || a.ga.g == a.gm.g);
-    for (int j = 0; j < a.nextra; ++j) v4 = v4 && al(a.extra[j], 16);
+    v4 = v4 && (a.Ho * a.Wo) % 4 == 0 && (a.H * a.W) % 4 == 0 && a.W % 4 == 0 && al(a.za, 4 * sizeof(zt)) &&
+         al(a.zm, 4 * sizeof(zt)) && al(a.amax, 4) && al(a.gx, 16);
+    for (int e = 0; e < a.nsrc; ++e) {
+      v4 = v4 && al(a.src[e].dout, 16);
+      for (int j = 0; j < a.src[e].nextra; ++j) v4 = v4 && al(a.src[e].extra[j], 16);
+    }
   }
   KSTAMP_ARM(kStampPoolBwd, st)
   if (v4) hipLaunchKernelGGL(pool_bwd_multi_kernel<true>, dim3(maxblk, b.n), dim3(256), lds, st, b);
diff --git a/katib_amd/models/darts_search.py b/katib_amd/models/darts_search.py
--- a/katib_amd/models/darts_search.py
+++ b/katib_amd/models/darts_search.py
@@ -8,6 +8,7 @@
 import torch.nn.functional as F
 
 from ..parallel.comm import Comm
+from ..utils.graphcheck import capture
 from .darts import BNState, DartsLayout, DartsNetwork, accuracy
 
 EVAL_GROUP = 16
@@ -386,7 +387,7 @@
         side0 = self._side_folds()
         for fns, colls in groups:
             g = torch.cuda.CUDAGraph()
-            with torch.cuda.graph(g), self._scope():
+            with capture(g), self._scope():
                 for fn in fns:
                     fn()
             graphs.append((g, colls))
@@ -462,7 +463,7 @@
                     self._evaluate(sx, sy)
             torch.cuda.current_stream().wait_stream(side)
             g = torch.cuda.CUDAGraph()
-            with torch.cuda.graph(g):
+            with capture(g):
                 out = torch.stack(self._evaluate(sx, sy))
             ent = self._eval_graphs[key] = (g, sx, sy, out)
         g, sx, sy, out = ent
diff --git a/katib_amd/ops/hip_darts.py b/katib_amd/ops/hip_darts.py
--- a/katib_amd/ops/hip_darts.py
+++ b/katib_amd/ops/hip_darts.py
@@ -248,7 +248,8 @@
         self.upd = []
 
 
-def _node_forward(xs, ws, specs, bns, params_list, training, momentum, eps, out=None, extra_fold=(), grad=True):
+def _node_forward(xs, ws, specs, bns, params_list, training, momentum, eps, out=None, extra_fold=(), grad=True,
+                  pool_cache=None, pool_keys=None):
     E = len(specs)
     xs = [t.contiguous() for t in xs]
     N, C = xs[0].shape[:2]
@@ -285,6 +286,7 @@
     pool_groups = defaultdict(list)
     fr_calls = []
     stage1, stage2 = [], []
+    pool_fold = []
     for e in edges:
         for k, prim in enumerate(e.spec.prims):
             if prim == "none":
@@ -306,6 +308,22 @@
                 e.zs[k], e.bns[k] = z, e.refs[sl[0]]
                 e.saved[prim] = (d, z)
                 stage1.append(e.slot0 + sl[0])
+            elif prim in ("avg_pooling_3x3", "max_pooling_3x3") and pool_cache is not None:
+                key = pool_keys[e.i]
+                if key not in pool_cache:
+                    za, zm = new(), new()
+                    am = torch.empty(N, C, Ho, Wo, dtype=torch.uint8, device=dev)
+                    pst = zeros64(2 * slot, dev) if training else None
+                    sa, sm = (pst[:slot], pst[slot:]) if training else (None, None)
+                    pool_groups[e.S].append((e.x, za, zm, sa, sm, am))
+                    pool_cache[key] = (za, zm, am, sa, sm)
+                    if training:
+                        pool_fold += [(sa, 2 * C, 2 * C), (sm, 2 * C, 2 * C)]
+                za, zm, am, sa, sm = pool_cache[key]
+                e.saved["pool"] = (za, zm, am)
+                avg = prim == "avg_pooling_3x3"
+                e.zs[k] = za if avg else zm
+                e.bns[k] = _bn(sa if avg else sm, e.bn[sl[0]][0], e.bn[sl[0]][1], cnt, training, eps, C)
             elif prim in ("avg_pooling_3x3", "max_pooling_3x3"):
                 if "pool" not in e.saved:
                     za, zm = new(), new()
@@ -338,8 +356,8 @@
     if fr_calls:
         _launch("pw_fwd", fr_calls, 2)
     defer = training and _defer()
-    if training and stage1 and not defer:
-        _fold([(stats[i * slot:(i + 1) * slot], 2 * C, 2 * C) for i in sorted(set(stage1))])
+    if training and (stage1 or pool_fold) and not defer:
+        _fold([(stats[i * slot:(i + 1) * slot], 2 * C, 2 * C) for i in sorted(set(stage1))] + pool_fold)
     s2_groups = defaultdict(list)
     for e in edges:
         for k, prim in enumerate(e.spec.prims):
@@ -354,9 +372,10 @@
                 e.zs[k], e.bns[k] = z2, e.refs[sl[1]]
                 e.saved[prim] = (d1, z1, d2, z2)
     _dwpw_multi([(*c, K, 1, 1, K // 2) for K, calls in s2_groups.items() for c in calls])
-    if training and (stage2 or (defer and stage1) or extra_fold):
+    late_pool = pool_fold if defer else []
+    if training and (stage2 or (defer and stage1) or late_pool or extra_fold):
         _fold([(stats[i * slot:(i + 1) * slot], 2 * C, 2 * C)
-               for i in sorted(set(stage2 + (stage1 if defer else [])))] + list(extra_fold))
+               for i in sorted(set(stage2 + (stage1 if defer else [])))] + late_pool + list(extra_fold))
     if out is None:
         out = torch.empty(N, C, Ho, Wo, device=dev)
     ccalls = []
@@ -371,7 +390,7 @@
 
 
 def _node_backward(edges, training, C, dout, gx_of, take_first, sinks, pkey, cell_gw=None, live=None,
-                   alpha_need=True):
+                   alpha_need=True, pool_out=None):
     dout = dout.contiguous()
     dev = dout.device
     if live is None:
@@ -463,23 +482,6 @@
             pw1.append((gs1, e.P[prim + ".0.pw"], d1, e.x, dd1, None, g, 0, 0, gst))
         _launch("pw_bwd", pw1, 1, 0, True)
 
-    first = {e.i: take_first(e.i) for e in edges}
-
-    def tf(i):
-        f = first.get(i, False)
-        first[i] = False
-        return f
-
-    def pool_srcs(e):
-        za, zm, am = e.saved["pool"]
-        ga = gm = None
-        for k, p in enumerate(e.spec.prims):
-            if p == "avg_pooling_3x3":
-                ga = src(e, k, za)
-            elif p == "max_pooling_3x3":
-                gm = src(e, k, zm)
-        return ga, gm, am
-
     convs, parts = [], defaultdict(list)
     for e, k, prim in seps + dils:
         sep = prim.startswith("separable_convolution")
@@ -491,28 +493,80 @@
         dd = e.saved[prim + "/dd1"] if sep else dd_of[(e.i, prim)]
         convs.append((e.x, None, e.P[name], dd, t, g, None, gst, True, K, 1 if sep else 2, e.S))
     _launch("dw_bwd_multi", convs)
+
+    def fr_pair(e):
+        if "skip_connection" not in e.saved:
+            return None
+        k = e.spec.prims.index("skip_connection")
+        (z,) = e.saved["skip_connection"]
+        gs = src(e, k, z)
+        g1, gst1 = sink(e, "skip_connection.conv1")
+        g2, gst2 = sink(e, "skip_connection.conv2")
+        return ((gs, e.P["skip_connection.conv1"], None, e.x, None, gxs[e.i], g1, 0, 0, gst1),
+                (gs, e.P["skip_connection.conv2"], None, e.x, None, gxs[e.i], g2, C // 2, 1, gst2))
+
+    if pool_out is not None:
+        for e in edges:
+            pool_out.append((e, _pool_source(e, dout, r_late, C, parts.get(e.i, [])), fr_pair(e)))
+        return
+    first = {e.i: take_first(e.i) for e in edges}
+
+    def tf(i):
+        f = first.get(i, False)
+        first[i] = False
+        return f
+
     sums = []
     for e in edges:
-        ga, gm, am = pool_srcs(e) if "pool" in e.saved else (None, None, None)
-        ex = parts.get(e.i, [])
-        if ga is None and gm is None and e.id_idx < 0 and not ex:
+        s = _pool_source(e, dout, r_late, C, parts.get(e.i, []))
+        if s is None:
             continue
-        sums.append((ga, gm, e.x, dout if e.id_idx >= 0 else None, e.w, e.id_idx, gxs[e.i], am, tf(e.i), e.S, ex))
+        sums += _pool_entries([(e, s)], gxs[e.i], tf(e.i))
     _launch("pool_bwd_multi", sums)
     frc = []
     for e in edges:
-        if "skip_connection" in e.saved:
+        pair = fr_pair(e)
+        if pair is not None:
             if tf(e.i):
                 gxs[e.i].zero_()
-            k = e.spec.prims.index("skip_connection")
-            (z,) = e.saved["skip_connection"]
-            gs = src(e, k, z)
-            g, gst = sink(e, "skip_connection.conv1")
-            frc.append((gs, e.P["skip_connection.conv1"], None, e.x, None, gxs[e.i], g, 0, 0, gst))
-            g, gst = sink(e, "skip_connection.conv2")
-            frc.append((gs, e.P["skip_connection.conv2"], None, e.x, None, gxs[e.i], g, C // 2, 1, gst))
+            frc += pair
     if frc:
         _launch("pw_bwd", frc, 2, 1, True)
+
+
+POOL_SHARE = int(_K.POOL_SHARE)
+
+
+def _pool_bn(e, prim):
+    return e.bl[e.widx.index(e.spec.prims.index(prim))]
+
+
+def _pool_source(e, dout, rep, C, extras):
+    part = {}
+    if "pool" in e.saved:
+        for k, p in enumerate(e.spec.prims):
+            if p in ("avg_pooling_3x3", "max_pooling_3x3"):
+                j = e.widx.index(k)
+                part[p] = (e.red[:C], e.red[(1 + j) * C:(2 + j) * C], e.w, k, rep, e.nred, e.bl[j][2])
+    if not part and e.id_idx < 0 and not extras:
+        return None
+    return (dout, part.get("avg_pooling_3x3"), part.get("max_pooling_3x3"), e.w if e.id_idx >= 0 else None,
+            e.id_idx, list(extras))
+
+
+def _pool_entries(group, gx, overwrite):
+    out = []
+    for i in range(0, len(group), POOL_SHARE):
+        chunk = group[i:i + POOL_SHARE]
+        za = zm = am = bna = bnm = None
+        for e, s in chunk:
+            if s[1] is not None and za is None:
+                za, bna = e.saved["pool"][0], _pool_bn(e, "avg_pooling_3x3")
+            if s[2] is not None and zm is None:
+                zm, am, bnm = e.saved["pool"][1], e.saved["pool"][2], _pool_bn(e, "max_pooling_3x3")
+        e0 = chunk[0][0]
+        out.append((za, zm, bna, bnm, am, e0.x, gx, overwrite and i == 0, e0.S, [s for _, s in chunk]))
+    return out
 
 
 class _MixedNode(torch.autograd.Function):
@@ -670,6 +724,23 @@
     return need
 
 
+def live_edges(spec: CellSpec, need: Sequence[bool], wreq) -> List[List[bool]]:
+    return [[bool(need[2 + i]) and (not NEEDED_GRADS or bool(need[src]) or any(wreq(n) for n in pnames))
+             for _, pnames, _, src, _ in node] for i, node in enumerate(spec.nodes)]
+
+
+def pool_groups(spec: CellSpec, live: Optional[Sequence[Sequence[bool]]] = None) -> Dict[Tuple[int, int], List[Tuple[int, int]]]:
+    groups: Dict[Tuple[int, int], List[Tuple[int, int]]] = {}
+    for i, node in enumerate(spec.nodes):
+        for k, (es, _, _, src, _) in enumerate(node):
+            if live is not None and not live[i][k]:
+                continue
+            if all(p == "none" for p in es.prims):
+                continue
+            groups.setdefault((src, es.stride), []).append((i, k))
+    return groups
+
+
 def network_needed_grads(spec: "NetSpec", wreq, alpha_n: bool, alpha_r: bool):
     need = [any(wreq(n) for n in spec.stem[:3])]
     i0 = i1 = 0
@@ -701,6 +772,7 @@
     Wo = (t0.shape[3] - 1) // max(S) + 1 if S else t0.shape[3]
     O = torch.empty(nn_, N, C, Ho, Wo, device=t0.device)
     node_states = []
+    pool_cache = {}
     for i, node in enumerate(spec.nodes):
         xs = [states[src] for _, _, _, src, _ in node]
         ws = [wts[row] for _, _, _, _, row in node]
@@ -708,7 +780,8 @@
         bns = [[bn_of(b) for b in bnames] for _, _, bnames, _, _ in node]
         plist = [[P[n] for n in pnames] for _, pnames, _, _, _ in node]
         out, edges = _node_forward(xs, ws, specs, bns, plist, training, momentum, eps, out=O[i],
-                                   extra_fold=late if i == 0 else (), grad=grad)
+                                   extra_fold=late if i == 0 else (), grad=grad, pool_cache=pool_cache,
+                                   pool_keys=[(src, es.stride) for es, _, _, src, _ in node])
         states.append(out)
         node_states.append(edges)
     return O, (spec, training, st0, st1, node_states, states, wts, P)
@@ -729,24 +802,52 @@
     first = [True, True] + [False] * nn_
     ga_rows = [None] * nn_
     cell_gw = []
+    lives = live_edges(spec, need, lambda n: P[n].requires_grad)
+    groups = pool_groups(spec, lives)
+    ready = defaultdict(list)
+    for key, members in groups.items():
+        ready[min(i for i, _ in members)].append(key)
+    recs = {}
+
+    def form_states(keys):
+        rounds, frs = defaultdict(list), defaultdict(list)
+        depth = defaultdict(int)
+        for key in keys:
+            src = key[0]
+            got = [recs.pop(m) for m in groups[key]]
+            srcs_ = [(e, s) for e, s, _ in got if s is not None]
+            if srcs_:
+                for ent in _pool_entries(srcs_, gS[src], first[src]):
+                    rounds[depth[src]].append(ent)
+                    depth[src] += 1
+                first[src] = False
+            frs[src] += [fr for _, _, fr in got if fr is not None]
+        for r in sorted(rounds):
+            _launch("pool_bwd_multi", rounds[r])
+        for src, pairs in frs.items():
+            if pairs and first[src]:
+                gS[src].zero_()
+                first[src] = False
+        for r in range(max((len(v) for v in frs.values()), default=0)):
+            _launch("pw_bwd", [c for pairs in frs.values() if r < len(pairs) for c in pairs[r]], 2, 1, True)
+
     for i in reversed(range(nn_)):
         if not need[2 + i]:
             continue
         node = spec.nodes[i]
         edges = node_states[i]
         srcs = [src for _, _, _, src, _ in node]
-        live = [_edge_live(e, need[src]) for e, src in zip(edges, srcs)]
+        live = lives[i]
         for src, lv in zip(srcs, live):
             if lv and gS[src] is None:
                 gS[src] = torch.empty_like(states[src])
 
-        def take_first(k, srcs=srcs):
-            f = first[srcs[k]]
-            first[srcs[k]] = False
-            return f
-
-        _node_backward(edges, training, spec.C, gS[2 + i], lambda k, srcs=srcs: gS[srcs[k]], take_first, sinks,
-                       lambda e, name, node=node: pkey(node[e.i][1][e.spec.pidx[name]]), cell_gw, live, alpha_need)
+        out = []
+        _node_backward(edges, training, spec.C, gS[2 + i], lambda k, srcs=srcs: gS[srcs[k]], None, sinks,
+                       lambda e, name, node=node: pkey(node[e.i][1][e.spec.pidx[name]]), cell_gw, live, alpha_need, out)
+        for e, s, fr in out:
+            recs[(i, e.i)] = (e, s, fr)
+        form_states(ready.get(i, []))
         if alpha_rows is not None:
             for e, (_, _, _, _, row) in zip(edges, node):
                 if e.gw is not None:
diff --git a/katib_amd/parallel/comm.py b/katib_amd/parallel/comm.py
--- a/katib_amd/parallel/comm.py
+++ b/katib_amd/parallel/comm.py
@@ -7,6 +7,8 @@
 
 import torch
 import torch.distributed as dist
+
+from ..utils.graphcheck import capture
 
 
 class Comm:
@@ -119,7 +121,7 @@
             dist.all_reduce(x, group=self.group)
             torch.cuda.synchronize(self.device)
             g = torch.cuda.CUDAGraph()
-            with torch.cuda.graph(g):
+            with capture(g):
                 dist.all_reduce(x, group=self.group)
         except Exception:
             ok, g = False, None
diff --git a/katib_amd/utils/graphcheck.py b/katib_amd/utils/graphcheck.py
--- a/katib_amd/utils/graphcheck.py
+++ b/katib_amd/utils/graphcheck.py
@@ -1,7 +1,9 @@
 
 from __future__ import annotations
 
+import contextlib
 import ctypes
+import gc
 
 import torch
 
@@ -30,3 +32,16 @@
         n += seg["total_size"]
     torch.cuda.synchronize()
     return n
+
+
+@contextlib.contextmanager
+def capture(graph: "torch.cuda.CUDAGraph", **kwargs):
+    gc.collect()
+    was_on = gc.isenabled()
+    gc.disable()
+    try:
+        with torch.cuda.graph(graph, **kwargs):
+            yield graph
+    finally:
+        if was_on:
+            gc.enable()
diff --git a/katib_amd/workloads/common.py b/katib_amd/workloads/common.py
--- a/katib_amd/workloads/common.py
+++ b/katib_amd/workloads/common.py
@@ -6,6 +6,8 @@
 from typing import Callable, Dict, Optional, Tuple
 
 import torch
+
+from ..utils.graphcheck import capture
 
 
 def device() -> torch.device:
@@ -141,7 +143,7 @@
                 self.calls += 1
                 return out
             self.graph = torch.cuda.CUDAGraph()
-            with torch.cuda.graph(self.graph):
+            with capture(self.graph):
                 self.out = self.fn()
         self.graph.replay()
         return self.out
```

New measurement: 1.938 s, median of 6. 3.2% less time.
